# Sirui-Xu/InterDiff

Measured on AMD Instinct MI355X. Metric: denoising frame-steps/sec (denoising-steps/sec x B x T frames), higher is better.
Workload: dtype f32 (every contraction of the denoiser -- feed-forward block, QKV projection, self-attention, row-block contractions and the two token GEMMs: every fp32 operand as two f16 planes, 3 f16 MFMAs per product, fp32 accumulate; SMPL and everything else fp32 MFMA / VALU)

## Files before the change

include/interdiff_hip.h:

```cpp
#ifndef INTERDIFF_HIP_H
#define INTERDIFF_HIP_H

#include <stddef.h>
#include <stdint.h>

#ifdef __cplusplus
extern "C" {
#endif

#define IDF_OK            0
#define IDF_E_INVAL      -22
#define IDF_E_NOMEM      -12
#define IDF_E_LAUNCH     -5

int         interdiff_abi_version(void);
const char *interdiff_build_info(void);

int interdiff_rotation_6d_to_matrix   (const float *d6, float *m,  int64_t n, void *stream);
int interdiff_matrix_to_rotation_6d   (const float *m,  float *d6, int64_t n, void *stream);
int interdiff_matrix_to_axis_angle    (const float *m,  float *aa, int64_t n, void *stream);
int interdiff_axis_angle_to_matrix    (const float *aa, float *m,  int64_t n, void *stream);
int interdiff_axis_angle_to_quaternion(const float *aa, float *q,  int64_t n, void *stream);
int interdiff_rotation_6d_to_axis_angle(const float *d6, float *aa, int64_t n, void *stream);

typedef struct {
    int32_t V, J, n_betas, KB, S;
    const float   *blend;
    const float   *jt;
    const float   *js;
    const int32_t *parents;
    const int32_t *skin_idx;
    const float   *skin_w;
} idf_smpl_model;

size_t interdiff_smpl_workspace_bytes(const idf_smpl_model *m, int64_t N);
int interdiff_smpl_forward(const idf_smpl_model *m, const float *pose, const float *betas,
                           const float *trans, int64_t N, float *verts, float *jtr,
                           float *v_posed, void *ws, size_t ws_bytes, void *stream);

int interdiff_vertex_normals(const float *verts, int64_t N, int32_t V, const int32_t *faces,
                             const int32_t *adj_ptr, const int32_t *adj_face,
                             const int32_t *adj_corner, float *normals, void *stream);
int interdiff_nn_argmin(const float *q, int32_t Pq, const float *r, int32_t Pr, int64_t N,
                        int32_t *idx, void *stream);
int interdiff_point2point_signed(const float *x, int32_t P1, const float *y, int32_t P2, int64_t N,
                                 const float *x_normals, const float *y_normals,
                                 float *y2x_signed, float *x2y_signed, int32_t *yidx, int32_t *xidx,
                                 float *y2x, float *x2y, void *stream);

#define IDF_MDM_LAYERS 8
#define IDF_MDM_D      256
#define IDF_MDM_FF     1024
#define IDF_MDM_HEADS  4
#define IDF_MDM_NQ     10
#define IDF_MDM_MEM    10
#define IDF_MDM_MEM_MAX 16
#define IDF_FFN_SLICES 5

typedef struct {
    int64_t is_qan;
    int64_t sa_in_w, sa_in_b, sa_out_w, sa_out_b;
    int64_t qc, wk;
    int64_t ca_q_w, ca_q_b;
    int64_t ca_kv_w, ca_kv_b;
    int64_t ca_out_w, ca_out_b;
    int64_t ff1_w, ff1_b, ff2_w, ff2_b;
    int64_t ffn_pack;
    int64_t ffn_b1p;
    int64_t sa_in_pack;
    int64_t sa_out_frag;
    int64_t ln_w[3], ln_b[3];
    int64_t ffn_pack_h2;
    int64_t sa_in_pack_h2;
    int64_t qc_h2;
    int64_t rb_h2_ok;
    int64_t sa_out_frag_h2;
    int64_t qkv_bounds_ok;
} idf_mdm_layer;

typedef struct {
    int32_t C;
    int32_t n_steps;
    const float *arena;
    int64_t in_w, in_b;
    int64_t out_w, out_b;
    int64_t temb_table;
    int64_t pe;
    int32_t max_T, has_encoder;
    idf_mdm_layer layer[IDF_MDM_LAYERS];
    idf_mdm_layer enc_layer[IDF_MDM_LAYERS];
    int32_t tune[8];
    int64_t out_w_h2, in_w_h2;
    int64_t tail_h2_ok;
    int32_t mem_len;
    int32_t rb_tokens;
} idf_mdm_weights;

int interdiff_gemm_f32(const float *A, int32_t lda, const float *W, const float *bias, const float *resid, float *C,
                       int32_t ldc, int32_t M, int32_t N, int32_t K, int32_t epi, int32_t cfg, void *stream);

int interdiff_mdm_ffn(const idf_mdm_weights *w, int32_t layer, int32_t encoder, const float *x2, int32_t M, float *parts, void *stream);
size_t interdiff_mdm_memctx_floats_for(int32_t B, int32_t mem_len);

size_t interdiff_mdm_memctx_floats(int32_t B);
size_t interdiff_mdm_workspace_bytes(int32_t B, int32_t T);
int interdiff_mdm_prepare_memory(const idf_mdm_weights *w, const float *cond, int32_t B,
                                 float *memctx, void *ws, size_t ws_bytes, void *stream);
int interdiff_mdm_forward(const idf_mdm_weights *w, const float *memctx, const float *x,
                          const int64_t *ts, int32_t B, int32_t T, float *x0,
                          void *ws, size_t ws_bytes, void *stream);

typedef struct {
    int64_t w[3], b[3];
    int32_t c[4];
} idf_pn_mlp;

typedef struct {
    const float *arena;
    idf_pn_mlp sa1[2];
    idf_pn_mlp sa2[2];
    int64_t lin_w, lin_b;
} idf_pointnet2;

int interdiff_pointnet2_encode(const idf_pointnet2 *pn, const float *obj_points, int32_t B, int32_t P, float *out,
                               void *stream);
size_t interdiff_mdm_encode_workspace_bytes(int32_t B, int32_t Tp);
int interdiff_mdm_encode(const idf_mdm_weights *w, const float *pc, const float *x_past, int32_t B, int32_t Tp,
                         float *cond, void *ws, size_t ws_bytes, void *stream);

int interdiff_inpaint(float *x0, const float *gt, const uint8_t *mask, int64_t n, void *stream);
int interdiff_posterior_step(float *x, const float *x0, const float *noise, int64_t n,
                             float c1, float c2, float sigma, uint64_t seed, uint64_t step_index,
                             void *stream);
int interdiff_randn(float *out, int64_t n, uint64_t seed, uint64_t step_index, void *stream);
int interdiff_posterior_step_at(float *x, const float *x0, const float *noise, int64_t n,
                                float c1, float c2, float sigma, uint64_t seed, uint64_t step_index,
                                uint64_t elem0, void *stream);
int interdiff_randn_at(float *out, int64_t n, uint64_t seed, uint64_t step_index, uint64_t elem0, void *stream);
int interdiff_posterior_step_dev(float *x, const float *x0, const float *gt, const uint8_t *mask, int64_t n,
                                 const float *table, int64_t *state, int64_t *ts, int32_t B, void *stream);
int interdiff_sampler_advance(int64_t *state, int64_t *ts, int32_t B, void *stream);
int interdiff_posterior_step_dev_map(float *x, const float *x0, const float *gt, const uint8_t *mask, int64_t n,
                                     const float *table, const int64_t *tmap, int64_t *state, int64_t *ts, int32_t B, void *stream);
int interdiff_sampler_advance_map(int64_t *state, int64_t *ts, const int64_t *tmap, int32_t B, void *stream);
int interdiff_mdm_forward_step(const idf_mdm_weights *w, const float *memctx, float *x, int64_t *ts, int32_t B, int32_t T,
                               const float *gt, const uint8_t *mask, const float *table, int64_t *state,
                               void *ws, size_t ws_bytes, void *stream);
#define IDF_STEP_EMBED_READY 1
#define IDF_STEP_EMBED_NEXT 2
int interdiff_mdm_forward_step_ex(const idf_mdm_weights *w, const float *memctx, float *x, int64_t *ts, int32_t B, int32_t T,
                                  const float *gt, const uint8_t *mask, const float *table, int64_t *state, void *ws,
                                  size_t ws_bytes, int32_t flags, void *stream);
int interdiff_mdm_forward_step_map(const idf_mdm_weights *w, const float *memctx, float *x, int64_t *ts, int32_t B, int32_t T,
                                   const float *gt, const uint8_t *mask, const float *table, const int64_t *tmap, int64_t *state,
                                   void *ws, size_t ws_bytes, int32_t flags, void *stream);
int interdiff_mdm_step_chaining(const idf_mdm_weights *w);
int interdiff_exclusive_cu_report(char *buf, int32_t cap);
int interdiff_debug_deny_exclusive(const char *patterns);

typedef struct {
    int32_t T, past_len, P, n_pre;
    const float *arena;
    int64_t dct_pad;
    int64_t dct;
    int64_t idct;
    int64_t hand_bonus;
    int64_t layer[12];
    int32_t cin[12], cout[12];
} idf_objproj;

int interdiff_objprojector_sample(const idf_objproj *op, const float *obj_angles,
                                  const float *obj_trans, const float *markers,
                                  const int32_t *contact, int32_t B, float *out, void *stream);
size_t interdiff_objprojector_forward_workspace_bytes(int32_t B);
int interdiff_objprojector_forward(const idf_objproj *op, const float *obj_angles, const float *obj_trans, const float *markers,
                                   const int32_t *contact, int32_t B, int32_t initialize, float *out, void *ws, size_t ws_bytes, void *stream);

typedef struct {
    const idf_smpl_model *smpl;
    const idf_objproj    *objproj;
    const int32_t *faces;
    const int32_t *adj_ptr, *adj_face, *adj_corner;
    const int32_t *markers_idx;
    int32_t n_markers, n_points, past_len;
    int32_t tune;
    const int32_t *vorder, *faces_scan, *markers_scan, *adj_pair_scan;
    const int32_t *adj_pair;
    const int32_t *vrank;
} idf_correction_ctx;

size_t interdiff_correction_workspace_bytes(const idf_correction_ctx *c, int32_t B, int32_t T);
int interdiff_correction(const idf_correction_ctx *c, float *x0, const float *gt,
                         const float *hand_pose, const float *beta, const float *obj_points,
                         int32_t B, int32_t T, float blend_t ,
                         uint8_t *condition, int32_t *contact, float *distance, float *loss,
                         void *ws, size_t ws_bytes, void *stream);
int interdiff_correction_dev(const idf_correction_ctx *c, float *x0, const float *gt, const float *hand_pose,
                             const float *beta, const float *obj_points, int32_t B, int32_t T, const float *table,
                             const int64_t *state, void *ws, size_t ws_bytes, void *stream);

#define IDF_CONTACT_STATS 12
size_t interdiff_contact_nn_workspace_bytes(const idf_correction_ctx *c, int32_t B, int32_t T);
int interdiff_contact_nn(const idf_correction_ctx *c, const float *verts, const float *obj_points, const float *objR,
                         const float *objT, int32_t B, int32_t T, float *o2h, int32_t *idx, uint64_t *stats,
                         void *ws, size_t ws_bytes, void *stream);

size_t interdiff_metrics_workspace_bytes(const idf_correction_ctx *c, int32_t B, int32_t T);
int interdiff_metrics(const idf_correction_ctx *c, const float *obj_pred, const float *jtr,
                      const float *body_trans, const float *obj_gt, const float *jtr_gt,
                      const float *body_trans_gt, const float *verts, const float *obj_points,
                      int32_t B, int32_t T, int32_t J, float *out6 ,
                      void *ws, size_t ws_bytes, void *stream);

typedef struct {
    int32_t T, past_len, J, n_pre;
    const float *arena;
    int64_t dct_pad;
    int64_t dct;
    int64_t idct;
    int64_t layer[12];
    int32_t cin[12], cout[12];
} idf_skel_objproj;

int interdiff_skeleton_objprojector_sample(const idf_skel_objproj *op, const float *obj_angles,
                                           const float *obj_trans, const float *human_points, int32_t B,
                                           float *quat_out, float *trans_out, void *stream);
int interdiff_skeleton_correction(const idf_skel_objproj *op, const float *x, const float *gt,
                                  const float *zero_pose_obj, int32_t B, int32_t T, float blend_t,
                                  float *out, void *stream);
int interdiff_skeleton_metrics(const float *body_pred, const float *body_gt, const float *obj_pred,
                               const float *obj_gt, const float *pose_pred, const float *pose_gt,
                               int32_t T, int32_t B, int32_t from_frame, float *out4, void *stream);

int interdiff_skeleton_finetune_param_table(const idf_skel_objproj *op, int32_t *table, int32_t *n_param, int32_t *n_bn);
size_t interdiff_skeleton_finetune_workspace_bytes(const idf_skel_objproj *op, int32_t B);
int interdiff_skeleton_finetune_grads(const idf_skel_objproj *op, const float *params, const float *bn, const float *obj_angles,
                                      const float *obj_trans, const float *human_points, const float *pose_gt, int32_t B, int32_t T,
                                      const float *weights8, float *out9, float *grads, void *ws, size_t ws_bytes, void *stream);
int interdiff_skeleton_finetune_step(const idf_skel_objproj *op, float *arena, float *params, const float *bn, const float *grads,
                                     float *exp_avg, float *exp_avg_sq, int32_t step, double lr, double beta1, double beta2, double eps,
                                     double weight_decay, void *stream);

typedef struct idf_skel_head {
    int32_t n_body, n_points;
    int32_t n_tiles, reserved;
    int64_t out_w, out_b;
    int64_t shape_w, shape_b;
} idf_skel_head;
int interdiff_skeleton_mdm_forward(const idf_mdm_weights *w, const idf_skel_head *head, const float *memctx, const float *x,
                                   const int64_t *ts, const float *zero_pose_obj, int32_t B, int32_t T, float *x0,
                                   void *ws, size_t ws_bytes, void *stream);
int interdiff_skeleton_mdm_forward_step(const idf_mdm_weights *w, const idf_skel_head *head, const float *memctx, float *x,
                                        int64_t *ts, const float *zero_pose_obj, int32_t B, int32_t T, const float *gt,
                                        const uint8_t *mask, const float *table, int64_t *state, void *ws, size_t ws_bytes,
                                        void *stream);
int interdiff_skeleton_mdm_forward_step_map(const idf_mdm_weights *w, const idf_skel_head *head, const float *memctx, float *x,
                                            int64_t *ts, const float *zero_pose_obj, int32_t B, int32_t T, const float *gt,
                                            const uint8_t *mask, const float *table, const int64_t *tmap, int64_t *state, void *ws,
                                            size_t ws_bytes, void *stream);
size_t interdiff_skeleton_mdm_encode_workspace_bytes(int32_t B, int32_t Tp);
int interdiff_skeleton_mdm_encode(const idf_mdm_weights *w, const idf_skel_head *head, const float *zero_pose_obj,
                                  const float *x_past, int32_t B, int32_t Tp, float *cond, void *ws, size_t ws_bytes,
                                  void *stream);

#define IDF_OPT_NP 483
#define IDF_OPT_NLOSS 6
typedef struct {
    const idf_correction_ctx *geo;
    const float   *blendT;
    const int32_t *jv_ptr;
    const int32_t *jv_vtx;
    const float   *jv_w;
    int32_t K3P, _pad;
} idf_opt_ctx;

typedef struct {
    int32_t B, T, P, max_iters;
    const float *betas;
    const float *obj_points;
    float *param, *init, *grad, *m, *v, *best;
    float *pose, *tr;
    float *verts, *vposed, *verts_gt, *gv;
    float *jtr;
    float *pts, *y2x;
    float *y2x_signed;
    int32_t *yidx;
    int32_t *near;
    float *dvposed;
    float *dA;
    float *dfeat;
    float *gtr;
    float *lossf;
    float *loss;
    float *loss_hist;
    float *best_loss;
    int32_t *flag;
    uint8_t *foot_static;
    int32_t *foot_cnt;
    int32_t *ctl;
    void *smpl_ws; size_t smpl_ws_bytes;
    int32_t *porder; float *psort, *pbox;
} idf_opt_state;

int interdiff_optimize_init(const idf_opt_ctx *c, const idf_opt_state *st, const float *pose, const float *trans,
                            const float *obj_angles, const float *obj_trans, int32_t first_iter, void *stream);
int interdiff_optimize_loss_grad(const idf_opt_ctx *c, const idf_opt_state *st, void *stream);
int interdiff_optimize_step(const idf_opt_ctx *c, const idf_opt_state *st, void *stream);
int interdiff_optimize_finish(const idf_opt_ctx *c, const idf_opt_state *st, float *pose, float *trans, float *obj_angles,
                              float *obj_trans, void *stream);
int interdiff_debug_joint_map_vjp(const float *R, const float *g_out, float *g_in, int32_t n);
int interdiff_debug_lds_sentinel(uint32_t *out, int32_t n_wg, int32_t spin, void *stream);
int interdiff_debug_f16_aggressor(const float *src, size_t n_floats, float *sink, int32_t iters, int32_t grid, int32_t with_loads, void *stream);

enum { IDF_LOSS_VAL = 0, IDF_LOSS_TEST = 1 };
int interdiff_q_sample(float *x_t, const float *x0, const float *noise, const int64_t *ts, const float *sqrt_ac, const float *sqrt_1mac,
                       int32_t n_steps, const float *gt, const uint8_t *mask, int32_t B, int64_t per_clip, uint64_t seed, uint64_t elem0,
                       void *stream);
int interdiff_denoising_losses(const float *pred, const float *target, int32_t B, int32_t T, int32_t past_len, float *out, void *stream);
size_t interdiff_sample_losses_workspace_bytes(int32_t K, int32_t B);
int interdiff_sample_losses(const float *samples, const float *gt, const float *hand_pose, int32_t K, int32_t B, int32_t T, int32_t past_len,
                            int32_t variant, float *out_terms, float *out_per_clip, void *ws, size_t ws_bytes, void *stream);

size_t interdiff_skeleton_sample_losses_workspace_bytes(int32_t K, int32_t B);
int interdiff_skeleton_sample_losses(const float *pred, const float *gt, int32_t K, int32_t B, int32_t C, int32_t T, int32_t past_len,
                                     int32_t n_body, int32_t n_points, float *out_terms, float *out_per_clip, void *ws, size_t ws_bytes,
                                     void *stream);
int interdiff_skeleton_denoising_losses(const float *pred, const float *target, int32_t B, int32_t T, int32_t past_len, int32_t n_body,
                                        int32_t n_points, float *out, void *stream);

size_t interdiff_correction_losses_workspace_bytes(int32_t T, int32_t B, int32_t V, int32_t P);
int interdiff_correction_losses(const float *obj_pred, const float *obj_gt, const float *obj_points, int32_t point_stride, const float *human_verts,
                                int32_t T, int32_t B, int32_t V, int32_t P, int32_t rot_width, int32_t past_len, float *out_terms, float *out_frames,
                                void *ws, size_t ws_bytes, void *stream);

size_t interdiff_contact_labels_workspace_bytes(int64_t N, int32_t V, int32_t F, int32_t P);
int interdiff_contact_labels(const float *verts, int64_t N, int32_t V, const int32_t *faces, int32_t F, const float *points, int32_t P,
                             int64_t point_frame_stride, const float *objR, const float *objT, float thres, uint8_t *obj_label ,
                             uint8_t *human_label , float *signed_dist , void *ws, size_t ws_bytes, void *stream);
int interdiff_debug_point_triangle(const float *tri, const float *p, float *out, int32_t n);

#define IDF_RENDER_SUBPIX 16
#define IDF_RENDER_GUARD 32768
#define IDF_RENDER_MAX_DIM 2048
#define IDF_RENDER_ZONE (1 << 28)
#define IDF_RENDER_REC_INTS 20
#define IDF_RENDER_TILE 16
#define IDF_RENDER_MAX_MESHES 8
enum { IDF_RMESH_SCENE_SPACE = 1, IDF_RMESH_VERTEX_RGB = 2 };
typedef struct {
    float off[3], cam_t[3];
    float cam_cos, cam_sin, znear, focal;
    float light[9];
    float light_gain, ambient;
    float bg[3];
    float reserved;
} idf_render_scene;
typedef struct {
    const float *verts, *normals;
    const int32_t *faces;
    const float *rgb, *R, *t;
    int32_t V, F, frames, flags;
} idf_render_mesh;
size_t interdiff_render_frames_workspace_bytes(int64_t n_images, int64_t n_triangles, int32_t H, int32_t W);
int interdiff_render_frames(const idf_render_scene *scene, const idf_render_mesh *meshes, int32_t n_meshes, int64_t N, int32_t views, int32_t H,
                            int32_t W, uint8_t *out_rgb, int32_t *out_id, int32_t *out_depth, int32_t *out_setup, int64_t *dropped, float *stage_ms,
                            void *ws, size_t ws_bytes, void *stream);
int interdiff_debug_render_setup_vertex(const idf_render_scene *scene, int32_t view, int32_t scene_space, int32_t H, int32_t W, const float *pos,
                                        const float *nrm, const float *rgb, float *out_f, int32_t *out_i, int32_t n);
int interdiff_debug_render_pixel(const int32_t *rec, const int32_t *ij, int32_t *out, int32_t n);

enum {
    IDF_K_EMBED = 0, IDF_K_GEMM_QKV, IDF_K_SELF_ATTN, IDF_K_GEMM_OUTPROJ, IDF_K_ROWBLOCK_QAN,
    IDF_K_ROWBLOCK_STD, IDF_K_FFN_FUSED, IDF_K_RESERVED7, IDF_K_GEMM_HEADS, IDF_K_MEM_PREP,
    IDF_K_INPAINT, IDF_K_POSTERIOR, IDF_K_CORR_PREPARE, IDF_K_SMPL_POSE, IDF_K_SMPL_BLEND_SKIN,
    IDF_K_CORR_CONTACT, IDF_K_CORR_REDUCE, IDF_K_OBJPROJ, IDF_K_CORR_BLEND, IDF_K_OTHER,
    IDF_K_COUNT
};
int interdiff_profile_begin(int32_t capacity);
int interdiff_profile_end(double *ms_per_kind, int64_t *count_per_kind);

enum {
    IDF_TUNE_FFN = 3, IDF_TUNE_FFN_MATH = 4, IDF_TUNE_COUNT = 8
};

#ifdef __cplusplus
}
#endif
#endif
```

interdiff_amd/_lib.py:

```python
import ctypes as C
import os
import torch

_HERE = os.path.dirname(os.path.abspath(__file__))
LIB_PATH = os.environ.get('INTERDIFF_HIP_LIB') or os.path.join(_HERE, 'csrc', 'libinterdiff_hip.so')
ABI_VERSION = 17

vp, i32, i64, f32, u64, sz = C.c_void_p, C.c_int32, C.c_int64, C.c_float, C.c_uint64, C.c_size_t

MDM_LAYERS = 8
FFN_SLICES = 5
STEP_EMBED_READY, STEP_EMBED_NEXT = 1, 2
LOSS_VAL, LOSS_TEST = 0, 1
TUNE = dict(ffn=3, ffn_math=4)


class SmplModel(C.Structure):
    _fields_ = [('V', i32), ('J', i32), ('n_betas', i32), ('KB', i32), ('S', i32),
                ('blend', vp), ('jt', vp), ('js', vp), ('parents', vp), ('skin_idx', vp), ('skin_w', vp)]


class MdmLayer(C.Structure):
    _fields_ = [('is_qan', i64),
                ('sa_in_w', i64), ('sa_in_b', i64), ('sa_out_w', i64), ('sa_out_b', i64),
                ('qc', i64), ('wk', i64),
                ('ca_q_w', i64), ('ca_q_b', i64), ('ca_kv_w', i64), ('ca_kv_b', i64),
                ('ca_out_w', i64), ('ca_out_b', i64),
                ('ff1_w', i64), ('ff1_b', i64), ('ff2_w', i64), ('ff2_b', i64), ('ffn_pack', i64), ('ffn_b1p', i64), ('sa_in_pack', i64), ('sa_out_frag', i64),
                ('ln_w', i64 * 3), ('ln_b', i64 * 3), ('ffn_pack_h2', i64), ('sa_in_pack_h2', i64), ('qc_h2', i64), ('rb_h2_ok', i64), ('sa_out_frag_h2', i64), ('qkv_bounds_ok', i64)]


class MdmWeights(C.Structure):
    _fields_ = [('C', i32), ('n_steps', i32), ('arena', vp),
                ('in_w', i64), ('in_b', i64), ('out_w', i64), ('out_b', i64),
                ('temb_table', i64), ('pe', i64), ('max_T', i32), ('has_encoder', i32),
                ('layer', MdmLayer * MDM_LAYERS), ('enc_layer', MdmLayer * MDM_LAYERS), ('tune', i32 * 8), ('out_w_h2', i64), ('in_w_h2', i64), ('tail_h2_ok', i64), ('mem_len', i32), ('rb_tokens', i32)]


class PnMlp(C.Structure):
    _fields_ = [('w', i64 * 3), ('b', i64 * 3), ('c', i32 * 4)]


class PointNet2(C.Structure):
    _fields_ = [('arena', vp), ('sa1', PnMlp * 2), ('sa2', PnMlp * 2), ('lin_w', i64), ('lin_b', i64)]


class ObjProj(C.Structure):
    _fields_ = [('T', i32), ('past_len', i32), ('P', i32), ('n_pre', i32), ('arena', vp),
                ('dct_pad', i64), ('dct', i64), ('idct', i64), ('hand_bonus', i64),
                ('layer', i64 * 12), ('cin', i32 * 12), ('cout', i32 * 12)]


class SkelObjProj(C.Structure):
    _fields_ = [('T', i32), ('past_len', i32), ('J', i32), ('n_pre', i32), ('arena', vp),
                ('dct_pad', i64), ('dct', i64), ('idct', i64),
                ('layer', i64 * 12), ('cin', i32 * 12), ('cout', i32 * 12)]


class SkelHead(C.Structure):
    _fields_ = [('n_body', i32), ('n_points', i32), ('n_tiles', i32), ('reserved', i32),
                ('out_w', i64), ('out_b', i64), ('shape_w', i64), ('shape_b', i64)]


class CorrectionCtx(C.Structure):
    _fields_ = [('smpl', C.POINTER(SmplModel)), ('objproj', C.POINTER(ObjProj)),
                ('faces', vp), ('adj_ptr', vp), ('adj_face', vp), ('adj_corner', vp), ('markers_idx', vp),
                ('n_markers', i32), ('n_points', i32), ('past_len', i32), ('tune', i32),
                ('vorder', vp), ('faces_scan', vp), ('markers_scan', vp), ('adj_pair_scan', vp), ('adj_pair', vp), ('vrank', vp)]


class OptCtx(C.Structure):
    _fields_ = [('geo', C.POINTER(CorrectionCtx)), ('blendT', vp), ('jv_ptr', vp), ('jv_vtx', vp), ('jv_w', vp), ('K3P', i32), ('_pad', i32)]


OPT_NP, OPT_NLOSS = 483, 6
_OPT_PTRS = ('betas', 'obj_points', 'param', 'init', 'grad', 'm', 'v', 'best', 'pose', 'tr', 'verts', 'vposed', 'verts_gt', 'gv',
             'jtr', 'pts', 'y2x', 'y2x_signed', 'yidx', 'near', 'dvposed', 'dA', 'dfeat', 'gtr', 'lossf', 'loss', 'loss_hist',
             'best_loss', 'flag', 'foot_static', 'foot_cnt', 'ctl', 'smpl_ws')


class OptState(C.Structure):
    _fields_ = [('B', i32), ('T', i32), ('P', i32), ('max_iters', i32)] + [(k, vp) for k in _OPT_PTRS] + [('smpl_ws_bytes', sz), ('porder', vp), ('psort', vp), ('pbox', vp)]


class RenderScene(C.Structure):
    _fields_ = [('off', f32 * 3), ('cam_t', f32 * 3), ('cam_cos', f32), ('cam_sin', f32), ('znear', f32), ('focal', f32),
                ('light', f32 * 9), ('light_gain', f32), ('ambient', f32), ('bg', f32 * 3), ('reserved', f32)]


class RenderMesh(C.Structure):
    _fields_ = [('verts', vp), ('normals', vp), ('faces', vp), ('rgb', vp), ('R', vp), ('t', vp),
                ('V', i32), ('F', i32), ('frames', i32), ('flags', i32)]


RMESH_SCENE_SPACE, RMESH_VERTEX_RGB = 1, 2
RENDER_SUBPIX, RENDER_GUARD, RENDER_MAX_DIM, RENDER_ZONE, RENDER_REC_INTS, RENDER_TILE = 16, 32768, 2048, 1 << 28, 20, 16

_SIGS = {
    'interdiff_abi_version': (C.c_int, []),
    'interdiff_build_info': (C.c_char_p, []),
    'interdiff_rotation_6d_to_matrix': (C.c_int, [vp, vp, i64, vp]),
    'interdiff_matrix_to_rotation_6d': (C.c_int, [vp, vp, i64, vp]),
    'interdiff_matrix_to_axis_angle': (C.c_int, [vp, vp, i64, vp]),
    'interdiff_axis_angle_to_matrix': (C.c_int, [vp, vp, i64, vp]),
    'interdiff_axis_angle_to_quaternion': (C.c_int, [vp, vp, i64, vp]),
    'interdiff_rotation_6d_to_axis_angle': (C.c_int, [vp, vp, i64, vp]),
    'interdiff_smpl_workspace_bytes': (sz, [C.POINTER(SmplModel), i64]),
    'interdiff_smpl_forward': (C.c_int, [C.POINTER(SmplModel), vp, vp, vp, i64, vp, vp, vp, vp, sz, vp]),
    'interdiff_vertex_normals': (C.c_int, [vp, i64, i32, vp, vp, vp, vp, vp, vp]),
    'interdiff_nn_argmin': (C.c_int, [vp, i32, vp, i32, i64, vp, vp]),
    'interdiff_point2point_signed': (C.c_int, [vp, i32, vp, i32, i64, vp, vp, vp, vp, vp, vp, vp, vp, vp]),
    'interdiff_gemm_f32': (C.c_int, [vp, i32, vp, vp, vp, vp, i32, i32, i32, i32, i32, i32, vp]),
    'interdiff_pointnet2_encode': (C.c_int, [C.POINTER(PointNet2), vp, i32, i32, vp, vp]),
    'interdiff_mdm_encode_workspace_bytes': (sz, [i32, i32]),
    'interdiff_mdm_encode': (C.c_int, [C.POINTER(MdmWeights), vp, vp, i32, i32, vp, vp, sz, vp]),
    'interdiff_mdm_ffn': (C.c_int, [C.POINTER(MdmWeights), i32, i32, vp, i32, vp, vp]),
    'interdiff_mdm_memctx_floats': (sz, [i32]),
    'interdiff_mdm_memctx_floats_for': (sz, [i32, i32]),
    'interdiff_mdm_workspace_bytes': (sz, [i32, i32]),
    'interdiff_mdm_prepare_memory': (C.c_int, [C.POINTER(MdmWeights), vp, i32, vp, vp, sz, vp]),
    'interdiff_mdm_forward': (C.c_int, [C.POINTER(MdmWeights), vp, vp, vp, i32, i32, vp, vp, sz, vp]),
    'interdiff_mdm_forward_step': (C.c_int, [C.POINTER(MdmWeights), vp, vp, vp, i32, i32, vp, vp, vp, vp, vp, sz, vp]),
    'interdiff_mdm_forward_step_ex': (C.c_int, [C.POINTER(MdmWeights), vp, vp, vp, i32, i32, vp, vp, vp, vp, vp, sz, i32, vp]),
    'interdiff_mdm_forward_step_map': (C.c_int, [C.POINTER(MdmWeights), vp, vp, vp, i32, i32, vp, vp, vp, vp, vp, vp, sz, i32, vp]),
    'interdiff_mdm_step_chaining': (C.c_int, [C.POINTER(MdmWeights)]),
    'interdiff_inpaint': (C.c_int, [vp, vp, vp, i64, vp]),
    'interdiff_posterior_step': (C.c_int, [vp, vp, vp, i64, f32, f32, f32, u64, u64, vp]),
    'interdiff_randn': (C.c_int, [vp, i64, u64, u64, vp]),
    'interdiff_posterior_step_at': (C.c_int, [vp, vp, vp, i64, f32, f32, f32, u64, u64, u64, vp]),
    'interdiff_randn_at': (C.c_int, [vp, i64, u64, u64, u64, vp]),
    'interdiff_posterior_step_dev': (C.c_int, [vp, vp, vp, vp, i64, vp, vp, vp, i32, vp]),
    'interdiff_sampler_advance': (C.c_int, [vp, vp, i32, vp]),
    'interdiff_posterior_step_dev_map': (C.c_int, [vp, vp, vp, vp, i64, vp, vp, vp, vp, i32, vp]),
    'interdiff_sampler_advance_map': (C.c_int, [vp, vp, vp, i32, vp]),
    'interdiff_objprojector_sample': (C.c_int, [C.POINTER(ObjProj), vp, vp, vp, vp, i32, vp, vp]),
    'interdiff_objprojector_forward_workspace_bytes': (sz, [i32]),
    'interdiff_objprojector_forward': (C.c_int, [C.POINTER(ObjProj), vp, vp, vp, vp, i32, i32, vp, vp, sz, vp]),
    'interdiff_correction_workspace_bytes': (sz, [C.POINTER(CorrectionCtx), i32, i32]),
    'interdiff_correction': (C.c_int, [C.POINTER(CorrectionCtx), vp, vp, vp, vp, vp, i32, i32, f32,
                                       vp, vp, vp, vp, vp, sz, vp]),
    'interdiff_correction_dev': (C.c_int, [C.POINTER(CorrectionCtx), vp, vp, vp, vp, vp, i32, i32, vp, vp, vp, sz, vp]),
    'interdiff_metrics_workspace_bytes': (sz, [C.POINTER(CorrectionCtx), i32, i32]),
    'interdiff_metrics': (C.c_int, [C.POINTER(CorrectionCtx), vp, vp, vp, vp, vp, vp, vp, vp, i32, i32, i32,
                                    vp, vp, sz, vp]),
    'interdiff_contact_nn_workspace_bytes': (sz, [C.POINTER(CorrectionCtx), i32, i32]),
    'interdiff_contact_nn': (C.c_int, [C.POINTER(CorrectionCtx), vp, vp, vp, vp, i32, i32, vp, vp, vp, vp, sz, vp]),
    'interdiff_skeleton_objprojector_sample': (C.c_int, [C.POINTER(SkelObjProj), vp, vp, vp, i32, vp, vp, vp]),
    'interdiff_skeleton_correction': (C.c_int, [C.POINTER(SkelObjProj), vp, vp, vp, i32, i32, f32, vp, vp]),
    'interdiff_skeleton_metrics': (C.c_int, [vp, vp, vp, vp, vp, vp, i32, i32, i32, vp, vp]),
    'interdiff_skeleton_finetune_param_table': (C.c_int, [C.POINTER(SkelObjProj), vp, C.POINTER(i32), C.POINTER(i32)]),
    'interdiff_skeleton_finetune_workspace_bytes': (sz, [C.POINTER(SkelObjProj), i32]),
    'interdiff_skeleton_finetune_grads': (C.c_int, [C.POINTER(SkelObjProj), vp, vp, vp, vp, vp, vp, i32, i32, C.POINTER(f32), vp, vp, vp, sz, vp]),
    'interdiff_skeleton_finetune_step': (C.c_int, [C.POINTER(SkelObjProj), vp, vp, vp, vp, vp, vp, i32, C.c_double, C.c_double, C.c_double, C.c_double,
                                                   C.c_double, vp]),
    'interdiff_skeleton_mdm_forward': (C.c_int, [C.POINTER(MdmWeights), C.POINTER(SkelHead), vp, vp, vp, vp, i32, i32, vp, vp, sz, vp]),
    'interdiff_skeleton_mdm_forward_step': (C.c_int, [C.POINTER(MdmWeights), C.POINTER(SkelHead), vp, vp, vp, vp, i32, i32, vp, vp, vp, vp, vp, sz, vp]),
    'interdiff_skeleton_mdm_forward_step_map': (C.c_int, [C.POINTER(MdmWeights), C.POINTER(SkelHead), vp, vp, vp, vp, i32, i32, vp, vp, vp, vp, vp, vp, sz, vp]),
    'interdiff_skeleton_mdm_encode_workspace_bytes': (sz, [i32, i32]),
    'interdiff_skeleton_mdm_encode': (C.c_int, [C.POINTER(MdmWeights), C.POINTER(SkelHead), vp, vp, i32, i32, vp, vp, sz, vp]),
    'interdiff_q_sample': (C.c_int, [vp, vp, vp, vp, vp, vp, i32, vp, vp, i32, i64, u64, u64, vp]),
    'interdiff_denoising_losses': (C.c_int, [vp, vp, i32, i32, i32, vp, vp]),
    'interdiff_sample_losses_workspace_bytes': (sz, [i32, i32]),
    'interdiff_sample_losses': (C.c_int, [vp, vp, vp, i32, i32, i32, i32, i32, vp, vp, vp, sz, vp]),
    'interdiff_skeleton_sample_losses_workspace_bytes': (sz, [i32, i32]),
    'interdiff_skeleton_sample_losses': (C.c_int, [vp, vp, i32, i32, i32, i32, i32, i32, i32, vp, vp, vp, sz, vp]),
    'interdiff_skeleton_denoising_losses': (C.c_int, [vp, vp, i32, i32, i32, i32, i32, vp, vp]),
    'interdiff_correction_losses_workspace_bytes': (sz, [i32, i32, i32, i32]),
    'interdiff_correction_losses': (C.c_int, [vp, vp, vp, i32, vp, i32, i32, i32, i32, i32, i32, vp, vp, vp, sz, vp]),
    'interdiff_contact_labels_workspace_bytes': (sz, [i64, i32, i32, i32]),
    'interdiff_contact_labels': (C.c_int, [vp, i64, i32, vp, i32, vp, i32, i64, vp, vp, f32, vp, vp, vp, vp, sz, vp]),
    'interdiff_debug_point_triangle': (C.c_int, [vp, vp, vp, i32]),
    'interdiff_render_frames_workspace_bytes': (sz, [i64, i64, i32, i32]),
    'interdiff_render_frames': (C.c_int, [C.POINTER(RenderScene), C.POINTER(RenderMesh), i32, i64, i32, i32, i32, vp, vp, vp, vp, C.POINTER(i64), C.POINTER(f32),
                                          vp, sz, vp]),
    'interdiff_debug_render_setup_vertex': (C.c_int, [C.POINTER(RenderScene), i32, i32, i32, i32, vp, vp, vp, vp, vp, i32]),
    'interdiff_debug_render_pixel': (C.c_int, [vp, vp, vp, i32]),
    'interdiff_optimize_init': (C.c_int, [C.POINTER(OptCtx), C.POINTER(OptState), vp, vp, vp, vp, i32, vp]),
    'interdiff_optimize_loss_grad': (C.c_int, [C.POINTER(OptCtx), C.POINTER(OptState), vp]),
    'interdiff_optimize_step': (C.c_int, [C.POINTER(OptCtx), C.POINTER(OptState), vp]),
    'interdiff_optimize_finish': (C.c_int, [C.POINTER(OptCtx), C.POINTER(OptState), vp, vp, vp, vp, vp]),
    'interdiff_debug_joint_map_vjp': (C.c_int, [vp, vp, vp, i32]),
    'interdiff_debug_lds_sentinel': (C.c_int, [vp, i32, i32, vp]),
    'interdiff_exclusive_cu_report': (C.c_int, [C.c_char_p, i32]),
    'interdiff_debug_deny_exclusive': (C.c_int, [C.c_char_p]),
    'interdiff_debug_f16_aggressor': (C.c_int, [vp, sz, vp, i32, i32, i32, vp]),
    'interdiff_profile_begin': (C.c_int, [i32]),
    'interdiff_profile_end': (C.c_int, [C.POINTER(C.c_double), C.POINTER(C.c_int64)]),
}

KERNEL_KINDS = ('embed', 'gemm_qkv', 'self_attn', 'gemm_outproj', 'rowblock_qan', 'rowblock_std', 'ffn_fused', 'reserved7',
                'gemm_heads', 'mem_prep', 'inpaint', 'posterior', 'corr_prepare', 'smpl_pose', 'smpl_blend_skin',
                'corr_contact', 'corr_reduce', 'objproj', 'corr_blend', 'other')

_lib = None


class HipLibraryMissing(RuntimeError):
    pass


def load():
    global _lib
    if _lib is not None:
        return _lib
    if not os.path.exists(LIB_PATH):
        raise HipLibraryMissing('%s not found: build it with `python -m interdiff_amd.csrc.build` '
                                '(there is no CPU/torch fallback for the hot path)' % LIB_PATH)
    lib = C.CDLL(LIB_PATH)
    for name, (res, args) in _SIGS.items():
        fn = getattr(lib, name)
        fn.restype, fn.argtypes = res, args
    if lib.interdiff_abi_version() != ABI_VERSION:
        raise HipLibraryMissing('stale %s: abi %d != %d, rebuild' % (LIB_PATH, lib.interdiff_abi_version(), ABI_VERSION))
    _lib = lib
    return lib


def exclusive_cu_report():
    buf = C.create_string_buffer(8192)
    bad = load().interdiff_exclusive_cu_report(buf, len(buf))
    if bad < 0:
        check(bad, 'exclusive_cu_report')
    return buf.value.decode(), bad


def debug_deny_exclusive(patterns=''):
    check(load().interdiff_debug_deny_exclusive(patterns.encode() if patterns else None), 'debug_deny_exclusive')


def exported_symbols():
    return sorted(_SIGS)


_ERR = {-22: 'IDF_E_INVAL (bad shape / pointer / unsupported size)', -12: 'IDF_E_NOMEM (workspace too small)',
        -5: 'IDF_E_LAUNCH (kernel launch failed)'}


def check(rc, what=''):
    if rc != 0:
        raise RuntimeError('interdiff_hip %s failed: %s' % (what, _ERR.get(rc, rc)))


def dptr(t, dtype=None, allow_none=False):
    if t is None:
        if allow_none:
            return vp(None)
        raise ValueError('null tensor')
    if not t.is_cuda:
        raise ValueError('interdiff_amd ops need device tensors (got %s); the HIP path has no CPU fallback' % t.device)
    if not t.is_contiguous():
        raise ValueError('tensor must be contiguous')
    if dtype is not None and t.dtype != dtype:
        raise ValueError('expected %s, got %s' % (dtype, t.dtype))
    return vp(t.data_ptr())


def stream():
    return vp(torch.cuda.current_stream().cuda_stream)
```

interdiff_amd/correction.py:

```python
import ctypes as C
import os
import itertools
import numpy as np
import torch
from . import _lib
from .geometry import MeshTopology

MARKERS67 = [3470, 3171, 3327, 857, 1812, 628, 182, 3116, 3040, 239,
             1666, 1725, 0, 2174, 1568, 1368, 3387, 2112, 1053, 1058,
             3336, 3346, 1323, 2108, 3122, 3314, 1252, 1082, 1861, 1454,
             850, 2224, 3233, 1769, 6728, 4343, 5273, 4116, 3694, 6399,
             6540, 6488, 3749, 5135, 5194, 3512, 5635, 5210, 4360, 4841,
             6786, 5573, 4538, 4544, 6736, 6747, 4804, 5568, 6544, 6682,
             5322, 4927, 5686, 4598, 6633, 3506, 3508]


_UID = itertools.count(1)


def correction_gate(t0):
    return not (t0 > 500 or t0 % 50 != 0)


class HipCorrection:
    def __init__(self, smpl_layer, objprojector, n_points=2048, past_len=10, markers=MARKERS67, device='cuda', scan_order=True):
        self.lib = _lib.load()
        self.device = torch.device(device)
        self.smpl, self.objproj, self.past_len = smpl_layer, objprojector, past_len
        self.topo = MeshTopology(smpl_layer.th_faces, smpl_layer.cmodel.V, self.device, rest_vertices=getattr(smpl_layer, 'v_template', None) if scan_order else None)
        self.markers_idx = torch.tensor(list(markers), dtype=torch.int32, device=self.device)
        ctx = _lib.CorrectionCtx()
        ctx.smpl = C.pointer(smpl_layer.cmodel)
        ctx.objproj = C.pointer(objprojector.cop)
        ctx.faces, ctx.adj_ptr = self.topo.faces.data_ptr(), self.topo.adj_ptr.data_ptr()
        ctx.adj_face, ctx.adj_corner = self.topo.adj_face.data_ptr(), self.topo.adj_corner.data_ptr()
        ctx.markers_idx = self.markers_idx.data_ptr()
        ctx.n_markers, ctx.n_points, ctx.past_len = len(markers), n_points, past_len
        if self.topo.vorder is not None:
            self.markers_scan = self.topo.scan_positions(markers, self.device)
            ctx.vorder, ctx.faces_scan, ctx.markers_scan = self.topo.vorder.data_ptr(), self.topo.faces_scan.data_ptr(), self.markers_scan.data_ptr()
            ctx.adj_pair_scan = self.topo.adj_pair_scan.data_ptr()
            ctx.vrank = self.topo.vrank.data_ptr()
        ctx.tune = 0
        self.ctx = ctx
        self._ws = {}
        self.debug = None
        self._uid = next(_UID)

    graph_capturable = True

    def workspace_for(self, B, T):
        return torch.empty(self.lib.interdiff_correction_workspace_bytes(C.byref(self.ctx), B, T), dtype=torch.uint8, device=self.device)

    def apply_dev(self, x, table, state, y, ws):
        B, _, Cc, T = x.shape
        if y['obj_points'].shape[1] != self.ctx.n_points:
            raise ValueError('obj_points must have %d points' % self.ctx.n_points)
        _lib.check(self.lib.interdiff_correction_dev(C.byref(self.ctx), _lib.dptr(x, torch.float32), _lib.dptr(y['inpainted_motion'], torch.float32),
                                                     _lib.dptr(y['hand_pose'], torch.float32), _lib.dptr(y['beta'], torch.float32),
                                                     _lib.dptr(y['obj_points'], torch.float32), B, T, _lib.dptr(table), _lib.dptr(state),
                                                     _lib.dptr(ws), ws.numel(), _lib.stream()), 'correction_dev')
        return x

    def _workspace(self, B, T):
        need = self.lib.interdiff_correction_workspace_bytes(C.byref(self.ctx), B, T)
        key = torch.cuda.current_stream(self.device).cuda_stream
        ws = self._ws.pop(key, None)
        if ws is None or ws.numel() < need:
            ws = torch.empty(need, dtype=torch.uint8, device=self.device)
        self._ws[key] = ws
        if len(self._ws) > self.MAX_STREAM_WORKSPACES:
            torch.cuda.synchronize(self.device)
            self._ws.pop(next(iter(self._ws)))
        return ws

    MAX_STREAM_WORKSPACES = 4

    def apply(self, x, t0, y):
        B, _, Cc, T = x.shape
        if not x.is_contiguous():
            raise ValueError('x must be contiguous (it is updated in place)')
        if y['obj_points'].shape[1] != self.ctx.n_points:
            raise ValueError('obj_points must have %d points' % self.ctx.n_points)
        gt = y['inpainted_motion'].contiguous()
        hp, beta, pts = y['hand_pose'].contiguous().float(), y['beta'].contiguous().float(), y['obj_points'].contiguous().float()
        ws = self._workspace(B, T)
        dbg = [None] * 4
        if self.debug is not None:
            dbg = [torch.empty(B, dtype=torch.uint8, device=self.device), torch.empty(B, len(MARKERS67), dtype=torch.int32, device=self.device),
                   torch.empty(B, device=self.device), torch.empty(B, device=self.device)]
        blend_t = float(np.float32(t0) / np.float32(1000))
        _lib.check(self.lib.interdiff_correction(C.byref(self.ctx), _lib.dptr(x, torch.float32), _lib.dptr(gt, torch.float32),
                                                 _lib.dptr(hp), _lib.dptr(beta), _lib.dptr(pts), B, T, blend_t,
                                                 *[_lib.dptr(d, allow_none=True) for d in dbg], _lib.dptr(ws), ws.numel(),
                                                 _lib.stream()), 'correction')
        if self.debug is not None:
            self.debug.update(condition=dbg[0], contact=dbg[1], distance=dbg[2], loss=dbg[3])
        return x

    def contact_nn(self, verts, obj_points, objR, objT, want_stats=False):
        T, B = verts.shape[:2]
        P = self.ctx.n_points
        o2h = torch.empty(T, B, P, device=self.device)
        idx = torch.empty(T, B, P, dtype=torch.int32, device=self.device)
        stats = torch.zeros(12, dtype=torch.int64, device=self.device) if want_stats else None
        need = self.lib.interdiff_contact_nn_workspace_bytes(C.byref(self.ctx), B, T)
        ws = getattr(self, '_nn_ws', None)
        if ws is None or ws.numel() < need:
            ws = self._nn_ws = torch.empty(need, dtype=torch.uint8, device=self.device)
        v, pts, R_, t_ = (a.contiguous().float() for a in (verts, obj_points, objR, objT))
        _lib.check(self.lib.interdiff_contact_nn(C.byref(self.ctx), _lib.dptr(v), _lib.dptr(pts), _lib.dptr(R_), _lib.dptr(t_), B, T, _lib.dptr(o2h),
                                                 _lib.dptr(idx), _lib.dptr(stats, allow_none=True), _lib.dptr(ws), ws.numel(), _lib.stream()), 'contact_nn')
        return (o2h, idx, tuple(int(x) for x in stats.cpu())) if want_stats else (o2h, idx)

    def is_active(self, t0):
        return correction_gate(int(t0))

    def __call__(self, x, t, model_kwargs):
        t0 = getattr(t, 'host_value', None)
        if t0 is None:
            t0 = int(t[0])
        if not correction_gate(t0):
            return x
        return self.apply(x, t0, model_kwargs['y'])
```

interdiff_amd/csrc/common.h:

```cpp
#pragma once
#include <hip/hip_runtime.h>
#include <stdint.h>
#include <stdio.h>
#include <atomic>
#include <mutex>
#include <string>
#include <vector>
#include "../../include/interdiff_hip.h"

#define IDF_WAVE 64

#define IDF_CHECK_LAUNCH()                                                                        \
    do {                                                                                          \
        const hipError_t idf_e_ = hipGetLastError();                                              \
        if (idf_e_ != hipSuccess) {                                                               \
            fprintf(stderr, "interdiff_hip: %s (%s:%d)\n", hipGetErrorString(idf_e_), __FILE__, __LINE__); \
            return IDF_E_LAUNCH;                                                                  \
        }                                                                                         \
    } while (0)

static inline hipStream_t idf_stream(void *s) { return reinterpret_cast<hipStream_t>(s); }
static inline int64_t idf_cdiv(int64_t a, int64_t b) { return (a + b - 1) / b; }
static inline size_t idf_align(size_t x, size_t a = 256) { return (x + a - 1) / a * a; }

static inline int idf_opt_in_lds(const void *fn, int bytes, std::atomic<uint64_t> &done) {
    int dev = 0;
    if (hipGetDevice(&dev) != hipSuccess) return IDF_E_LAUNCH;
    const uint64_t bit = 1ull << (dev & 63);
    if (done.load(std::memory_order_acquire) & bit) return IDF_OK;
    if (hipFuncSetAttribute(fn, hipFuncAttributeMaxDynamicSharedMemorySize, bytes) != hipSuccess) return IDF_E_LAUNCH;
    done.fetch_or(bit, std::memory_order_release);
    return IDF_OK;
}

struct idf_excl_entry {
    const char *name;
    int threads, num_regs, static_lds, dyn_lds, blocks_per_cu, ok, dev, denied;
};
inline std::mutex g_idf_excl_mu;
inline std::vector<idf_excl_entry> g_idf_excl;
inline void idf_excl_record(const idf_excl_entry &e) {
    std::lock_guard<std::mutex> lk(g_idf_excl_mu);
    for (idf_excl_entry &o : g_idf_excl)
        if (o.dev == e.dev && std::string(o.name) == e.name) { o = e; return; }
    g_idf_excl.push_back(e);
}
inline int idf_excl_report(char *buf, int cap) {
    std::lock_guard<std::mutex> lk(g_idf_excl_mu);
    int bad = 0, n = 0;
    buf[0] = 0;
    for (const idf_excl_entry &e : g_idf_excl) {
        bad += e.ok ? 0 : 1;
        const int w = snprintf(buf + n, (size_t)(cap - n), "%-52s dev %d  threads %3d  regs %3d  lds %6d + %6d  workgroups_per_cu %d  %s\n", e.name, e.dev, e.threads, e.num_regs,
                               e.static_lds, e.dyn_lds, e.blocks_per_cu, e.ok ? "exclusive" : (e.denied ? "DENIED (debug deny list) -> fp32 kernel" : "NOT exclusive -> fp32 kernel"));
        if (w < 0 || w >= cap - n) break;
        n += w;
    }
    return bad;
}
inline std::string g_idf_excl_deny;
inline std::atomic<uint64_t> g_idf_excl_gen{1};
inline void idf_excl_set_deny(const char *patterns) {
    std::lock_guard<std::mutex> lk(g_idf_excl_mu);
    g_idf_excl_deny = patterns ? patterns : "";
    g_idf_excl.clear();
    g_idf_excl_gen.fetch_add(1, std::memory_order_acq_rel);
}
inline bool idf_excl_denied(const char *name) {
    std::lock_guard<std::mutex> lk(g_idf_excl_mu);
    if (g_idf_excl_deny.empty()) return false;
    const std::string nm(name);
    size_t a = 0;
    while (a <= g_idf_excl_deny.size()) {
        size_t b = g_idf_excl_deny.find(',', a);
        if (b == std::string::npos) b = g_idf_excl_deny.size();
        if (b > a && nm.find(g_idf_excl_deny.substr(a, b - a)) != std::string::npos) return true;
        a = b + 1;
    }
    return false;
}
struct idf_excl_cache {
    std::atomic<uint64_t> yes{0}, no{0}, gen{0};
    std::atomic<int> dyn{-1};
};
constexpr int IDF_CU_LDS_BYTES = 160 * 1024;
constexpr int IDF_NOT_EXCLUSIVE = 1;
static inline int idf_public_rc(int rc) { return rc == IDF_NOT_EXCLUSIVE ? IDF_E_LAUNCH : rc; }
static inline int idf_exclusive_cu(const void *fn, const char *name, int threads, idf_excl_cache &c) {
    int dev = 0;
    if (hipGetDevice(&dev) != hipSuccess) return -1;
    const uint64_t bit = 1ull << (dev & 63), gen = g_idf_excl_gen.load(std::memory_order_acquire);
    if (c.gen.load(std::memory_order_acquire) != gen) {
        c.yes.store(0, std::memory_order_release);
        c.no.store(0, std::memory_order_release);
        c.gen.store(gen, std::memory_order_release);
    }
    if (c.yes.load(std::memory_order_acquire) & bit) return c.dyn.load(std::memory_order_acquire);
    if (c.no.load(std::memory_order_acquire) & bit) return -1;
    idf_excl_entry e{name, threads, -1, -1, -1, -1, 0, dev, 0};
    hipFuncAttributes at;
    if (hipFuncGetAttributes(&at, fn) == hipSuccess) {
        e.num_regs = at.numRegs;
        e.static_lds = (int)at.sharedSizeBytes;
        e.dyn_lds = IDF_CU_LDS_BYTES - e.static_lds;
        if (e.dyn_lds >= 0 && hipFuncSetAttribute(fn, hipFuncAttributeMaxDynamicSharedMemorySize, e.dyn_lds) == hipSuccess &&
            hipOccupancyMaxActiveBlocksPerMultiprocessor(&e.blocks_per_cu, fn, threads, (size_t)e.dyn_lds) == hipSuccess)
            e.ok = e.blocks_per_cu == 1 && e.num_regs >= (threads > 512 ? 128 : 256) ? 1 : 0;
    }
    (void)hipGetLastError();
    if (e.ok && idf_excl_denied(name)) { e.ok = 0; e.denied = 1; }
    idf_excl_record(e);
    if (e.ok) {
        c.dyn.store(e.dyn_lds, std::memory_order_release);
        c.yes.fetch_or(bit, std::memory_order_release);
        return e.dyn_lds;
    }
    c.no.fetch_or(bit, std::memory_order_release);
    if (e.denied) fprintf(stderr, "interdiff_hip: %s is on the DEBUG deny list: the fp32-MFMA kernel runs instead\n", name);
    else fprintf(stderr, "interdiff_hip: %s does not get its CU to itself on device %d (regs %d, LDS %d + %d, %d workgroups per CU): the fp32-MFMA kernel runs instead\n",
                 name, dev, e.num_regs, e.static_lds, e.dyn_lds, e.blocks_per_cu);
    return -1;
}

static inline int idf_cu_count() {
    static std::atomic<int> cached[64];
    int dev = 0;
    if (hipGetDevice(&dev) != hipSuccess) return 256;
    int n = cached[dev & 63].load(std::memory_order_acquire);
    if (n <= 0) {
        if (hipDeviceGetAttribute(&n, hipDeviceAttributeMultiprocessorCount, dev) != hipSuccess || n <= 0) n = 256;
        cached[dev & 63].store(n, std::memory_order_release);
    }
    return n;
}

typedef float f32x4 __attribute__((ext_vector_type(4)));

typedef __attribute__((address_space(3))) float idf_lds_float;
__device__ __forceinline__ uint32_t idf_lds_addr(const float *p) {
    return __builtin_amdgcn_readfirstlane((uint32_t)(uintptr_t)(idf_lds_float *)p);
}
__device__ __forceinline__ const float *idf_uniform_ptr(const float *p) {
    const uint64_t v = (uint64_t)(uintptr_t)p;
    const uint32_t lo = __builtin_amdgcn_readfirstlane((uint32_t)v), hi = __builtin_amdgcn_readfirstlane((uint32_t)(v >> 32));
    return reinterpret_cast<const float *>(((uint64_t)hi << 32) | lo);
}
__device__ __forceinline__ void idf_dma16_s(const float *gbase, uint32_t voff_bytes, uint32_t lds_base) {
    gbase = idf_uniform_ptr(gbase);
    lds_base = __builtin_amdgcn_readfirstlane(lds_base);
    asm volatile("s_mov_b32 m0, %2\n\ts_nop 0\n\tglobal_load_lds_dwordx4 %0, %1" ::"v"(voff_bytes), "s"(gbase), "s"(lds_base) : "memory", "m0");
}
__device__ __forceinline__ void idf_dma16_v(const float *gptr, uint32_t lds_base) {
    lds_base = __builtin_amdgcn_readfirstlane(lds_base);
    asm volatile("s_mov_b32 m0, %1\n\ts_nop 0\n\tglobal_load_lds_dwordx4 %0, off" ::"v"(gptr), "s"(lds_base) : "memory", "m0");
}

__device__ __forceinline__ void idf_store4_wt(float *p, const float v) {
    asm volatile("global_store_dword %0, %1, off sc0 sc1" ::"v"(p), "v"(v) : "memory");
}
__device__ __forceinline__ void idf_store16_wt(float *p, const float4 v) {
    const f32x4 t = {v.x, v.y, v.z, v.w};
    asm volatile("global_store_dwordx4 %0, %1, off sc0 sc1\n\ts_nop 1" ::"v"(p), "v"(t) : "memory");
}

template <class T>
__device__ __forceinline__ void idf_arg_now(T a) { asm volatile("" ::"s"(a)); }
template <class... A>
__device__ __forceinline__ void idf_args_now(A... a) { (idf_arg_now(a), ...); }

int idf_point_order(hipStream_t s, const float *obj_points, int B, int P, int32_t *porder);
int idf_nn_scan_opt(hipStream_t s, int64_t N, int frames_per_clip, const float *verts, int V, const float *pts_frame, const float *obj_points, int P,
                    const int32_t *porder, const idf_correction_ctx *c, int32_t *yidx);
int idf_near_mask_opt(hipStream_t s, int64_t N, int frames_per_clip, const float *verts, int V, const float *pts_frame, int P, const int32_t *porder,
                      const int32_t *vorder, float *psort, float *pbox, int32_t *near);

size_t idf_objproj_keep_floats();
int idf_objproj_check(const idf_objproj *op);
int idf_objproj_pick(const idf_objproj *op, const float *keep, const int32_t *contact, int B, float *out, hipStream_t s);

extern bool g_idf_prof_on;
void idf_prof_mark_slow(int kind, hipStream_t s);
static inline void idf_prof_mark(int kind, hipStream_t s) { if (g_idf_prof_on) idf_prof_mark_slow(kind, s); }


typedef float f32x16 __attribute__((ext_vector_type(16)));

#define IDF_DPP_ROR(v, n) __builtin_bit_cast(float, __builtin_amdgcn_update_dpp(0, __builtin_bit_cast(int, v), 0x120 + (n), 0xf, 0xf, false))
__device__ __forceinline__ float row16_sum(float v) {
    v += IDF_DPP_ROR(v, 8);
    v += IDF_DPP_ROR(v, 4);
    v += IDF_DPP_ROR(v, 2);
    v += IDF_DPP_ROR(v, 1);
    return v;
}
__device__ __forceinline__ float row16_max(float v) {
    v = fmaxf(v, IDF_DPP_ROR(v, 8));
    v = fmaxf(v, IDF_DPP_ROR(v, 4));
    v = fmaxf(v, IDF_DPP_ROR(v, 2));
    v = fmaxf(v, IDF_DPP_ROR(v, 1));
    return v;
}
#define IDF_LANE(v, l) __builtin_bit_cast(float, __builtin_amdgcn_readlane(__builtin_bit_cast(int, v), l))
__device__ __forceinline__ float wave_sum(float v) {
    v = row16_sum(v);
    return (IDF_LANE(v, 0) + IDF_LANE(v, 16)) + (IDF_LANE(v, 32) + IDF_LANE(v, 48));
}
__device__ __forceinline__ float wave_max(float v) {
    v = row16_max(v);
    return fmaxf(fmaxf(IDF_LANE(v, 0), IDF_LANE(v, 16)), fmaxf(IDF_LANE(v, 32), IDF_LANE(v, 48)));
}

__device__ __forceinline__ float gelu_erf(float x) { return 0.5f * x * (1.0f + erff(x * 0.70710678118654752440f)); }

__device__ __forceinline__ float gelu_fast(float x) {
    const float z = fabsf(x) * 0.70710678118654752440f;
    const float t = __builtin_amdgcn_rcpf(1.0f + 0.3275911f * z);
    const float p = ((((1.061405429f * t - 1.453152027f) * t + 1.421413741f) * t - 0.284496736f) * t + 0.254829592f) * t;
    const float er = 1.0f - p * __expf(-(z * z));
    return 0.5f * x * (1.0f + copysignf(er, x));
}

__device__ __forceinline__ void ln_row_stats(const float4 v, float &mean, float &rstd) {
    mean = wave_sum(v.x + v.y + v.z + v.w) * (1.0f / 256.0f);
    const float a = v.x - mean, b = v.y - mean, c = v.z - mean, d = v.w - mean;
    const float var = wave_sum(a * a + b * b + c * c + d * d) * (1.0f / 256.0f);
    rstd = __builtin_amdgcn_rsqf(var + 1e-5f);
}

struct Row16 {
    float4 c[4];
};
__device__ __forceinline__ void ln_row16(Row16 &r, const float *__restrict__ w, const float *__restrict__ b, int l16) {
    float s = 0.f;
#pragma unroll
    for (int i = 0; i < 4; ++i) s += (r.c[i].x + r.c[i].y) + (r.c[i].z + r.c[i].w);
    const float mean = row16_sum(s) * (1.0f / 256.0f);
    float q = 0.f;
#pragma unroll
    for (int i = 0; i < 4; ++i) {
        const float a0 = r.c[i].x - mean, a1 = r.c[i].y - mean, a2 = r.c[i].z - mean, a3 = r.c[i].w - mean;
        q += (a0 * a0 + a1 * a1) + (a2 * a2 + a3 * a3);
    }
    const float rstd = __builtin_amdgcn_rsqf(row16_sum(q) * (1.0f / 256.0f) + 1e-5f);
#pragma unroll
    for (int i = 0; i < 4; ++i) {
        const float4 g = *reinterpret_cast<const float4 *>(w + (i * 16 + l16) * 4), be = *reinterpret_cast<const float4 *>(b + (i * 16 + l16) * 4);
        r.c[i].x = (r.c[i].x - mean) * rstd * g.x + be.x;
        r.c[i].y = (r.c[i].y - mean) * rstd * g.y + be.y;
        r.c[i].z = (r.c[i].z - mean) * rstd * g.z + be.z;
        r.c[i].w = (r.c[i].w - mean) * rstd * g.w + be.w;
    }
}
__device__ __forceinline__ void row16_load(Row16 &r, const float *__restrict__ row, int l16) {
#pragma unroll
    for (int i = 0; i < 4; ++i) r.c[i] = *reinterpret_cast<const float4 *>(row + (i * 16 + l16) * 4);
}
template <int NP>
__device__ __forceinline__ float4 ld4_sum(const float *__restrict__ p, size_t stride) {
    float4 t[NP];
#pragma unroll
    for (int s = 0; s < NP; ++s) t[s] = *reinterpret_cast<const float4 *>(p + s * stride);
    float4 v = t[0];
#pragma unroll
    for (int s = 1; s < NP; ++s) { v.x += t[s].x; v.y += t[s].y; v.z += t[s].z; v.w += t[s].w; }
    return v;
}
template <int NP>
struct Row16Raw {
    float4 t[4][NP];
    __device__ __forceinline__ void request(const float *__restrict__ row, int l16, size_t stride) {
#pragma unroll
        for (int i = 0; i < 4; ++i)
#pragma unroll
            for (int s = 0; s < NP; ++s) t[i][s] = *reinterpret_cast<const float4 *>(row + s * stride + (i * 16 + l16) * 4);
    }
    __device__ __forceinline__ void reduce(Row16 &r) const {
#pragma unroll
        for (int i = 0; i < 4; ++i) {
            float4 v = t[i][0];
#pragma unroll
            for (int s = 1; s < NP; ++s) { v.x += t[i][s].x; v.y += t[i][s].y; v.z += t[i][s].z; v.w += t[i][s].w; }
            r.c[i] = v;
        }
    }
};
template <int NP>
__device__ __forceinline__ void row16_load_sum(Row16 &r, const float *__restrict__ row, int l16, size_t stride) {
    Row16Raw<NP> raw;
    raw.request(row, l16, stride);
    raw.reduce(r);
}
__device__ __forceinline__ void row16_store(const Row16 &r, float *__restrict__ row, int l16) {
#pragma unroll
    for (int i = 0; i < 4; ++i) *reinterpret_cast<float4 *>(row + (i * 16 + l16) * 4) = r.c[i];
}
__device__ __forceinline__ void row16_store_wt(const Row16 &r, float *__restrict__ row, int l16) {
#pragma unroll
    for (int i = 0; i < 4; ++i) idf_store16_wt(row + (i * 16 + l16) * 4, r.c[i]);
}
__device__ __forceinline__ void row16_zero(Row16 &r) {
#pragma unroll
    for (int i = 0; i < 4; ++i) r.c[i] = make_float4(0.f, 0.f, 0.f, 0.f);
}
```

interdiff_amd/csrc/correction.hip:

```cpp
#include "common.h"
#include "objproj.h"
#include "rot_math.h"
#include <float.h>

namespace {

constexpr int NBODY = 22;
constexpr int CTOK = 144;

__global__ __launch_bounds__(256) void corr_prepare_kernel(const float *__restrict__ x0, const float *__restrict__ gt,
                                                           const float *__restrict__ hand_pose, int B, int T,
                                                           float *__restrict__ pose, float *__restrict__ trans,
                                                           float *__restrict__ objR, float *__restrict__ objT,
                                                           float *__restrict__ gt_angles, float *__restrict__ gt_trans) {
    const int64_t i = (int64_t)blockIdx.x * 256 + threadIdx.x;
    const int64_t N = (int64_t)B * T;
    if (i >= N * 24) return;
    const int64_t n = i / 24;
    const int slot = (int)(i - n * 24), t = (int)(n / B), b = (int)(n - (int64_t)t * B);
    const float *xb = x0 + (size_t)b * CTOK * T + t;
    if (slot < NBODY) {
        float d[6], m[9], a[3];
#pragma unroll
        for (int k = 0; k < 6; ++k) d[k] = xb[(size_t)(slot * 6 + k) * T];
        rot::rot6d_to_matrix(d, m);
        rot::matrix_to_axis_angle(m, a);
        float *p = pose + n * 156 + slot * 3;
        p[0] = a[0]; p[1] = a[1]; p[2] = a[2];
    } else if (slot == 22) {
        for (int k = 0; k < 90; ++k) pose[n * 156 + 66 + k] = hand_pose[n * 90 + k];
#pragma unroll
        for (int k = 0; k < 3; ++k) trans[n * 3 + k] = xb[(size_t)(132 + k) * T];
    } else {
        float d[6], m[9];
#pragma unroll
        for (int k = 0; k < 6; ++k) d[k] = xb[(size_t)(135 + k) * T];
        rot::rot6d_to_matrix(d, m);
#pragma unroll
        for (int k = 0; k < 9; ++k) objR[n * 9 + k] = m[k];
        const float *gb = gt + (size_t)b * CTOK * T + t;
#pragma unroll
        for (int k = 0; k < 3; ++k) {
            objT[n * 3 + k] = xb[(size_t)(141 + k) * T];
            gt_trans[n * 3 + k] = gb[(size_t)(141 + k) * T];
        }
#pragma unroll
        for (int k = 0; k < 6; ++k) gt_angles[n * 6 + k] = gb[(size_t)(135 + k) * T];
    }
}

__device__ __forceinline__ float dist2_exact(float qx, float qy, float qz, float rx, float ry, float rz) {
#pragma clang fp contract(off)
    const float dx = qx - rx, dy = qy - ry, dz = qz - rz;
    const float xx = dx * dx, yy = dy * dy, zz = dz * dz;
    return (xx + yy) + zz;
}

__device__ __forceinline__ float3 f3(const float4 v) { return make_float3(v.x, v.y, v.z); }
__device__ __forceinline__ float3 sub3(float3 a, float3 b) { return make_float3(a.x - b.x, a.y - b.y, a.z - b.z); }
__device__ __forceinline__ float3 cross3(float3 a, float3 b) {
    return make_float3(a.y * b.z - a.z * b.y, a.z * b.x - a.x * b.z, a.x * b.y - a.y * b.x);
}

constexpr int MAXP = 2048;
__global__ __launch_bounds__(1024) void corr_point_order_kernel(const float *__restrict__ obj_points, int P, int32_t *__restrict__ porder) {
    __shared__ unsigned long long keys[MAXP];
    __shared__ float red[6][1024];
    const int b = blockIdx.x, tid = threadIdx.x;
    const float *op = obj_points + (size_t)b * P * 3;
    float p[2][3];
    float lo[3] = {FLT_MAX, FLT_MAX, FLT_MAX}, hi[3] = {-FLT_MAX, -FLT_MAX, -FLT_MAX};
#pragma unroll
    for (int k = 0; k < 2; ++k) {
        const int i = tid + 1024 * k;
#pragma unroll
        for (int a = 0; a < 3; ++a) {
            p[k][a] = i < P ? op[3 * i + a] : 0.f;
            if (i < P) { lo[a] = fminf(lo[a], p[k][a]); hi[a] = fmaxf(hi[a], p[k][a]); }
        }
    }
#pragma unroll
    for (int a = 0; a < 3; ++a) { red[a][tid] = lo[a]; red[3 + a][tid] = hi[a]; }
    __syncthreads();
    for (int s = 512; s > 0; s >>= 1) {
        if (tid < s) {
#pragma unroll
            for (int a = 0; a < 3; ++a) {
                red[a][tid] = fminf(red[a][tid], red[a][tid + s]);
                red[3 + a][tid] = fmaxf(red[3 + a][tid], red[3 + a][tid + s]);
            }
        }
        __syncthreads();
    }
#pragma unroll
    for (int k = 0; k < 2; ++k) {
        const int i = tid + 1024 * k;
        unsigned long long key = ~0ull;
        if (i < P) {
            unsigned code = 0;
            unsigned q[3];
#pragma unroll
            for (int a = 0; a < 3; ++a) {
                const float ext = red[3 + a][0] - red[a][0];
                const float u = ext > 0.f ? (p[k][a] - red[a][0]) / ext : 0.f;
                q[a] = (unsigned)fminf(fmaxf(u * 1023.0f, 0.f), 1023.0f);
            }
#pragma unroll
            for (int bit = 0; bit < 10; ++bit)
#pragma unroll
                for (int a = 0; a < 3; ++a) code |= ((q[a] >> bit) & 1u) << (3 * bit + a);
            key = ((unsigned long long)code << 11) | (unsigned)i;
        }
        keys[i] = key;
    }
    __syncthreads();
    for (int k = 2; k <= MAXP; k <<= 1) {
        for (int j = k >> 1; j > 0; j >>= 1) {
            const int l = 2 * j * (tid / j) + (tid % j), r = l + j;
            const unsigned long long x = keys[l], y = keys[r];
            const bool up = (l & k) == 0;
            if ((x > y) == up) { keys[l] = y; keys[r] = x; }
            __syncthreads();
        }
    }
#pragma unroll
    for (int k = 0; k < 2; ++k) {
        const int i = tid + 1024 * k;
        if (i < P) porder[(size_t)b * P + i] = (int32_t)(keys[i] & 2047u);
    }
}

constexpr int MAXM = 128;
constexpr float MARK_D2 = 0.00039999996079131961f;
constexpr int CB = 16;
constexpr int SB = 8;
constexpr int SEED_STRIDE = 4;
constexpr int CT = 1024;
constexpr int TASK = 64;
typedef float v2f __attribute__((ext_vector_type(2)));

struct ContactLds {
    int V4, nCB, nSB, nSeed;
    int rec, mark, box, sbox, seed, flags, red, pl, total;
    __host__ __device__ explicit ContactLds(int V) {
        V4 = (V + CB - 1) / CB * CB; nCB = V4 / CB; nSB = (nCB + SB - 1) / SB; nSeed = (nCB + SEED_STRIDE - 1) / SEED_STRIDE;
        rec = 0;
        mark = rec + V4;
        box = mark + MAXM;
        sbox = box + 3 * (nSB * SB / 2);
        seed = sbox + 3 * ((nSB + 2) / 2);
        flags = seed + 2 * ((nSeed + 1) / 2);
        red = flags + MAXM / 4;
        pl = red + CT / 4;
        total = pl + MAXP / 4;
    }
};

__device__ __forceinline__ float3 lds_rec(const float4 *vs, int pos) {
    const float *f = reinterpret_cast<const float *>(vs + 2 * (pos >> 1));
    const int h = pos & 1;
    return make_float3(f[h], f[2 + h], f[4 + h]);
}
__device__ __forceinline__ void lds_rec_store(float4 *vs, int pos, float x, float y, float z) {
    float *f = reinterpret_cast<float *>(vs + 2 * (pos >> 1));
    const int h = pos & 1;
    f[h] = x; f[2 + h] = y; f[4 + h] = z;
}
__device__ __forceinline__ void lds_box_store(float4 *bx, int k, float3 lo, float3 hi) {
    float *f = reinterpret_cast<float *>(bx + 3 * (k >> 1));
    const int h = k & 1;
    f[h] = lo.x; f[2 + h] = lo.y; f[4 + h] = lo.z; f[6 + h] = hi.x; f[8 + h] = hi.y; f[10 + h] = hi.z;
}
__device__ __forceinline__ void lds_box_load(const float4 *bx, int k, float3 &lo, float3 &hi) {
    const float *f = reinterpret_cast<const float *>(bx + 3 * (k >> 1));
    const int h = k & 1;
    lo = make_float3(f[h], f[2 + h], f[4 + h]);
    hi = make_float3(f[6 + h], f[8 + h], f[10 + h]);
}

struct PredArgs {
    idf_objproj op;
    const float *obj_angles, *obj_trans;
    const int32_t *markers_idx;
    float *markers, *keep;
    int nclips;
};
template <bool OPT, bool WITH_PRED = false>
__global__ __launch_bounds__(CT) void corr_contact_kernel(const float *__restrict__ verts, int V,
                                                          const float *__restrict__ obj_points, int P,
                                                          const int32_t *__restrict__ porder ,
                                                          const float *__restrict__ objR, const float *__restrict__ objT,
                                                          const int32_t *__restrict__ faces ,
                                                          const int32_t *__restrict__ adj_ptr,
                                                          const int32_t *__restrict__ adj_face,
                                                          const int32_t *__restrict__ adj_corner,
                                                          const int32_t *__restrict__ adj_pair ,
                                                          const int32_t *__restrict__ vorder ,
                                                          const int32_t *__restrict__ vrank ,
                                                          const int32_t *__restrict__ markers_pos , int M, int B,
                                                          float *__restrict__ markers_out, float *__restrict__ loss_sum,
                                                          float *__restrict__ min_dist, int32_t *__restrict__ label,
                                                          float *__restrict__ o2h_out ,
                                                          int32_t *__restrict__ idx_out ,
                                                          unsigned long long *__restrict__ stats ,
                                                          int64_t nn_from ,
                                                          const float *__restrict__ pts_frame , int frames_per_clip ,
                                                          const PredArgs pred) {
    extern __shared__ __attribute__((aligned(16))) float4 vs[];
    if constexpr (WITH_PRED) {
        if ((int)blockIdx.x < pred.nclips) {
            const int b = blockIdx.x, Tn = pred.op.T;
            for (int i = threadIdx.x; i < Tn * M; i += CT) {
                const int t = i / M, m = i - t * M;
                const size_t nfr = (size_t)t * B + b;
                const float *v = verts + (nfr * V + pred.markers_idx[m]) * 3;
                float *o = pred.markers + (nfr * M + m) * 3;
                o[0] = v[0]; o[1] = v[1]; o[2] = v[2];
            }
            __threadfence();
            __syncthreads();
            idf_objproj_dev::objproj_body<1>(reinterpret_cast<float *>(vs), pred.op, pred.obj_angles, pred.obj_trans, pred.markers, nullptr, B, b, pred.keep, nullptr);
            return;
        }
    }
    const ContactLds L(V);
    const int nCB = L.nCB, nSB = L.nSB;
    float4 *ms = vs + L.mark, *bb = vs + L.box, *sbb = vs + L.sbox, *sd = vs + L.seed;
    int *flags = reinterpret_cast<int *>(vs + L.flags);
    float *red = reinterpret_cast<float *>(vs + L.red);
    float *pl = reinterpret_cast<float *>(vs + L.pl);
    __shared__ int next_task;
    const int64_t n = WITH_PRED ? (int64_t)blockIdx.x - pred.nclips : (int64_t)blockIdx.x;
    const int b = OPT ? (int)(n / frames_per_clip) : (int)(n % B), tid = threadIdx.x;
    const float *vf = verts + (size_t)n * V * 3;
    const bool do_nn = n >= nn_from;
    long long t_prev = 0;
    int n_phase = 0;
    auto phase_done = [&]() {
        if (stats && tid == 0 && do_nn) {
            const long long now = (long long)__builtin_readcyclecounter();
            if (n_phase > 0) atomicAdd(stats + 3 + n_phase, (unsigned long long)(now - t_prev));
            t_prev = now;
        }
        ++n_phase;
    };
    phase_done();
    float R[9] = {1.f, 0.f, 0.f, 0.f, 1.f, 0.f, 0.f, 0.f, 1.f}, tr[3] = {0.f, 0.f, 0.f};
    if constexpr (!OPT) {
#pragma unroll
        for (int k = 0; k < 9; ++k) R[k] = objR[n * 9 + k];
#pragma unroll
        for (int k = 0; k < 3; ++k) tr[k] = objT[n * 3 + k];
    }
    const int my_marker_pos = (!OPT && tid < M) ? markers_pos[tid] : 0;
    if (vorder && vrank) {
        for (int i0 = tid; i0 < V; i0 += 4 * CT) {
            typedef float f3v __attribute__((ext_vector_type(3), aligned(4)));
            int pos[4];
            f3v pv[4];
#pragma unroll
            for (int k = 0; k < 4; ++k) {
                const int i = min(i0 + k * CT, V - 1);
                pos[k] = vrank[i];
                pv[k] = *reinterpret_cast<const f3v *>(vf + 3 * i);
            }
#pragma unroll
            for (int k = 0; k < 4; ++k) {
                if (i0 + k * CT < V) {
                    lds_rec_store(vs, pos[k], pv[k].x, pv[k].y, pv[k].z);
                    reinterpret_cast<int *>(vs + 2 * (pos[k] >> 1) + 1)[2 + (pos[k] & 1)] = i0 + k * CT;
                }
            }
        }
        for (int v = V + tid; v < L.V4; v += CT) {
            lds_rec_store(vs, v, 3e18f, 3e18f, 3e18f);
            reinterpret_cast<int *>(vs + 2 * (v >> 1) + 1)[2 + (v & 1)] = 0x7fffffff;
        }
    } else
    for (int v0 = tid; v0 < L.V4; v0 += 4 * CT) {
        int o[4];
        float x[4], y[4], z[4];
#pragma unroll
        for (int k = 0; k < 4; ++k) {
            const int v = v0 + k * CT;
            o[k] = v < V ? (vorder ? vorder[v] : v) : -1;
        }
#pragma unroll
        for (int k = 0; k < 4; ++k) {
            x[k] = y[k] = z[k] = 3e18f;
            if (o[k] >= 0) {
                typedef float f3v __attribute__((ext_vector_type(3), aligned(4)));
                const f3v pv = *reinterpret_cast<const f3v *>(vf + 3 * o[k]);
                x[k] = pv.x; y[k] = pv.y; z[k] = pv.z;
            }
        }
#pragma unroll
        for (int k = 0; k < 4; ++k) {
            const int v = v0 + k * CT;
            if (v < L.V4) {
                lds_rec_store(vs, v, x[k], y[k], z[k]);
                reinterpret_cast<int *>(vs + 2 * (v >> 1) + 1)[2 + (v & 1)] = o[k] >= 0 ? o[k] : 0x7fffffff;
            }
        }
    }
    if (tid < MAXM) flags[tid] = 0;
    const int ntask_all = (P + TASK - 1) / TASK;
    const int task0 = (int)((long long)blockIdx.y * ntask_all / gridDim.y), task1 = (int)((long long)(blockIdx.y + 1) * ntask_all / gridDim.y);
    if (tid == 0) next_task = task0;
    for (int i = tid; i < MAXP; i += CT) pl[i] = 0.f;
    __syncthreads();
    phase_done();
    if (!OPT && tid < ((M + 1) & ~1)) {
        float3 mk = make_float3(3e18f, 3e18f, 3e18f);
        if (tid < M) {
            mk = lds_rec(vs, my_marker_pos);
            if (markers_out) {
                float *mo = markers_out + ((size_t)n * M + tid) * 3;
                mo[0] = mk.x; mo[1] = mk.y; mo[2] = mk.z;
            }
        }
        lds_rec_store(ms, tid, mk.x, mk.y, mk.z);
    }
    if (do_nn) {
#define IDF_DPP8(v, op, ctrl) v = op(v, __builtin_bit_cast(float, __builtin_amdgcn_update_dpp(__builtin_bit_cast(int, v), __builtin_bit_cast(int, v), ctrl, 0xf, 0xf, false)))
        const int lane_ = tid & 63, wave_ = tid >> 6, nsw = 2 * ((nSB + 2) / 2);
        for (int sb = wave_; sb < nsw; sb += CT / 64) {
            const int pr = sb * 64 + lane_;
            float lx = FLT_MAX, ly = FLT_MAX, lz = FLT_MAX, hx = -FLT_MAX, hy = -FLT_MAX, hz = -FLT_MAX;
            if (2 * pr < V) {
                const float4 xy = vs[2 * pr], zz = vs[2 * pr + 1];
                const bool two = 2 * pr + 1 < V;
                lx = two ? fminf(xy.x, xy.y) : xy.x; hx = two ? fmaxf(xy.x, xy.y) : xy.x;
                ly = two ? fminf(xy.z, xy.w) : xy.z; hy = two ? fmaxf(xy.z, xy.w) : xy.z;
                lz = two ? fminf(zz.x, zz.y) : zz.x; hz = two ? fmaxf(zz.x, zz.y) : zz.x;
            }
            IDF_DPP8(lx, fminf, 0xB1); IDF_DPP8(lx, fminf, 0x4E); IDF_DPP8(lx, fminf, 0x141);
            IDF_DPP8(ly, fminf, 0xB1); IDF_DPP8(ly, fminf, 0x4E); IDF_DPP8(ly, fminf, 0x141);
            IDF_DPP8(lz, fminf, 0xB1); IDF_DPP8(lz, fminf, 0x4E); IDF_DPP8(lz, fminf, 0x141);
            IDF_DPP8(hx, fmaxf, 0xB1); IDF_DPP8(hx, fmaxf, 0x4E); IDF_DPP8(hx, fmaxf, 0x141);
            IDF_DPP8(hy, fmaxf, 0xB1); IDF_DPP8(hy, fmaxf, 0x4E); IDF_DPP8(hy, fmaxf, 0x141);
            IDF_DPP8(hz, fmaxf, 0xB1); IDF_DPP8(hz, fmaxf, 0x4E); IDF_DPP8(hz, fmaxf, 0x141);
            const int cb = sb * SB + (lane_ >> 3);
            if ((lane_ & 7) == 0 && cb < nSB * SB) lds_box_store(bb, cb, make_float3(lx, ly, lz), make_float3(hx, hy, hz));
            const float slx = -wave_max(-lx), sly = -wave_max(-ly), slz = -wave_max(-lz), shx = wave_max(hx), shy = wave_max(hy), shz = wave_max(hz);
            if (lane_ == 0) lds_box_store(sbb, sb, make_float3(slx, sly, slz), make_float3(shx, shy, shz));
        }
#undef IDF_DPP8
        for (int k = tid; k < 2 * ((L.nSeed + 1) / 2); k += CT) {
            const float3 p = lds_rec(vs, min(k * SEED_STRIDE, nCB - 1) * CB);
            lds_rec_store(sd, k, p.x, p.y, p.z);
        }
    }
    const float *op = OPT ? pts_frame + (size_t)n * P * 3 : obj_points + (size_t)b * P * 3;
    const int ln = tid & 63, ntask = task1;
    __syncthreads();
    phase_done();
    float mind2 = FLT_MAX;
    unsigned n_exec = 0, n_test = 0, n_tasks = 0;
    for (;;) {
        int task = 0;
        if (ln == 0) task = atomicAdd(&next_task, 1);
        task = __builtin_amdgcn_readfirstlane(task);
        if (task >= ntask) break;
        ++n_tasks;
        const int sp = task * TASK + ln;
        const int i = sp < P ? (porder ? porder[(size_t)b * P + sp] : sp) : -1;
        const bool valid = i >= 0;
        float px = 0.f, py = 0.f, pz = 0.f;
        if (valid) { px = op[3 * i]; py = op[3 * i + 1]; pz = op[3 * i + 2]; }
        const float qx = OPT ? px : (px * R[0] + py * R[1] + pz * R[2]) + tr[0];
        const float qy = OPT ? py : (px * R[3] + py * R[4] + pz * R[5]) + tr[1];
        const float qz = OPT ? pz : (px * R[6] + py * R[7] + pz * R[8]) + tr[2];
        if (do_nn) {
#pragma clang fp contract(off)
            const v2f QX = v2f{qx, qx}, QY = v2f{qy, qy}, QZ = v2f{qz, qz};
            auto pair_d2 = [&](const float4 xy, const float4 zz) {
#pragma clang fp contract(off)
                const v2f dx = QX - v2f{xy.x, xy.y}, dy = QY - v2f{xy.z, xy.w}, dz = QZ - v2f{zz.x, zz.y};
                return (dx * dx + dy * dy) + dz * dz;
            };
            auto pair_a2 = [&](const float4 xy, const float2 zz) {
                const v2f dx = QX - v2f{xy.x, xy.y}, dy = QY - v2f{xy.z, xy.w}, dz = QZ - v2f{zz.x, zz.y};
                return __builtin_elementwise_fma(dz, dz, __builtin_elementwise_fma(dy, dy, dx * dx));
            };
            constexpr float SCAN_M = 1.000003814697265625f, SCAN_ABS = 1e-37f;
            float seed = FLT_MAX;
            for (int k = 0; k < (L.nSeed + 1) / 2; k += 4) {
                float4 xy[4]; float2 zz[4];
#pragma unroll
                for (int u = 0; u < 4; ++u) { xy[u] = sd[2 * min(k + u, (L.nSeed + 1) / 2 - 1)]; zz[u] = *reinterpret_cast<const float2 *>(&sd[2 * min(k + u, (L.nSeed + 1) / 2 - 1) + 1]); }
#pragma unroll
                for (int u = 0; u < 4; ++u) {
                    const v2f a2 = pair_a2(xy[u], zz[u]);
                    seed = fminf(fminf(seed, a2.x), a2.y);
                }
            }
            float thr = __builtin_fmaf(seed, SCAN_M, SCAN_ABS);
            float best = FLT_MAX, bthr = FLT_MAX;
            int tie = 0;
            int bblk = 0, bblk2 = 0;
            auto pair_lb = [&](const float4 a, const float4 bq, const float4 c) {
#pragma clang fp contract(off)
                const v2f ax = v2f{a.x, a.y} - QX, bx = QX - v2f{bq.z, bq.w};
                const v2f ay = v2f{a.z, a.w} - QY, by = QY - v2f{c.x, c.y};
                const v2f az = v2f{bq.x, bq.y} - QZ, bz = QZ - v2f{c.z, c.w};
                const v2f ex = v2f{fmaxf(fmaxf(ax.x, bx.x), 0.f), fmaxf(fmaxf(ax.y, bx.y), 0.f)};
                const v2f ey = v2f{fmaxf(fmaxf(ay.x, by.x), 0.f), fmaxf(fmaxf(ay.y, by.y), 0.f)};
                const v2f ez = v2f{fmaxf(fmaxf(az.x, bz.x), 0.f), fmaxf(fmaxf(az.y, bz.y), 0.f)};
                return __builtin_elementwise_fma(ez, ez, __builtin_elementwise_fma(ey, ey, ex * ex));
            };
            auto score_block = [&](int cb) {
                ++n_exec;
                const int v0 = cb * CB;
                float4 xy[CB / 2]; float2 zz[CB / 2];
#pragma unroll
                for (int u = 0; u < CB / 2; ++u) { xy[u] = vs[v0 + 2 * u]; zz[u] = *reinterpret_cast<const float2 *>(&vs[v0 + 2 * u + 1]); }
                float bm = FLT_MAX;
#pragma unroll
                for (int u = 0; u < CB / 2; ++u) {
                    const v2f a2 = pair_a2(xy[u], zz[u]);
                    bm = fminf(fminf(bm, a2.x), a2.y);
                }
                if (bm < best) {
                    const float w = __builtin_fmaf(bm, SCAN_M, SCAN_ABS);
                    if (best <= w) { tie = tie ? 2 : 1; bblk2 = bblk; } else tie = 0;
                    best = bm; bblk = v0; bthr = w; thr = fminf(thr, w);
                } else if (bm <= bthr) { tie = tie ? 2 : 1; bblk2 = v0; }
            };
            auto scan_super = [&](int sb) {
                const int cb0 = sb * SB;
#pragma unroll
                for (int j = 0; j < SB / 2; ++j) {
                    const int cb = cb0 + 2 * j;
                    const float4 *bx = bb + 3 * (cb >> 1);
                    const v2f lb = pair_lb(bx[0], bx[1], bx[2]);
                    n_test += 2;
                    if (__builtin_amdgcn_ballot_w64(valid && lb.x <= thr) != 0ull) score_block(cb);
                    if (__builtin_amdgcn_ballot_w64(valid && lb.y <= thr) != 0ull) score_block(cb + 1);
                }
            };
            if (!vorder) {
                for (int cb = 0; cb < nCB; ++cb) score_block(cb);
            } else
            for (int sb = 0; sb < nSB; sb += 2) {
                const float4 *bx = sbb + 3 * (sb >> 1);
                const v2f lb = pair_lb(bx[0], bx[1], bx[2]);
                n_test += 2;
                if (__builtin_amdgcn_ballot_w64(valid && lb.x <= thr) != 0ull) scan_super(sb);
                if (__builtin_amdgcn_ballot_w64(valid && lb.y <= thr) != 0ull) scan_super(sb + 1);
            }
            int pos = bblk, org = 0x7fffffff;
            float ebest = FLT_MAX;
            auto resolve_pair = [&](int pr) {
                const float4 xy = vs[2 * pr], zz = vs[2 * pr + 1];
                const v2f d2 = pair_d2(xy, zz);
                const int o0 = __builtin_bit_cast(int, zz.z), o1 = __builtin_bit_cast(int, zz.w);
                if (d2.x < ebest || (d2.x == ebest && o0 < org)) { ebest = d2.x; org = o0; pos = 2 * pr; }
                if (d2.y < ebest || (d2.y == ebest && o1 < org)) { ebest = d2.y; org = o1; pos = 2 * pr + 1; }
            };
            if (tie < 2) {
#pragma unroll
                for (int u = 0; u < CB / 2; ++u) resolve_pair((bblk >> 1) + u);
                if (tie) {
#pragma unroll
                    for (int u = 0; u < CB / 2; ++u) resolve_pair((bblk2 >> 1) + u);
                }
            } else {
                for (int pr = 0; pr < (V + 1) / 2; ++pr) resolve_pair(pr);
            }
            pos = min(pos, V - 1);
            if (org == 0x7fffffff) org = vorder ? vorder[pos] : pos;
            if constexpr (OPT) {
                if (valid) idx_out[(size_t)n * P + i] = org;
            } else if (valid) {
                const float3 v3 = lds_rec(vs, pos);
                float3 acc = make_float3(0.f, 0.f, 0.f);
                const int e0 = adj_ptr[org], e1 = adj_ptr[org + 1];
                if (adj_pair) {
                    for (int e = e0; e < e1; e += 4) {
                        int2 ab[4];
#pragma unroll
                        for (int u = 0; u < 4; ++u) ab[u] = *reinterpret_cast<const int2 *>(adj_pair + 2 * (size_t)min(e + u, e1 - 1));
#pragma unroll
                        for (int u = 0; u < 4; ++u) {
                            if (e + u < e1) {
                                const float3 nn = cross3(sub3(lds_rec(vs, ab[u].x), v3), sub3(lds_rec(vs, ab[u].y), v3));
                                acc.x += nn.x; acc.y += nn.y; acc.z += nn.z;
                            }
                        }
                    }
                } else {
                    for (int e = e0; e < e1; ++e) {
                        const int f = adj_face[e], c = adj_corner[e];
                        const float3 p0 = lds_rec(vs, faces[3 * f]), p1 = lds_rec(vs, faces[3 * f + 1]), p2 = lds_rec(vs, faces[3 * f + 2]);
                        float3 nn;
                        if (c == 1) nn = cross3(sub3(p2, p1), sub3(p0, p1));
                        else if (c == 2) nn = cross3(sub3(p0, p2), sub3(p1, p2));
                        else nn = cross3(sub3(p1, p0), sub3(p2, p0));
                        acc.x += nn.x; acc.y += nn.y; acc.z += nn.z;
                    }
                }
                const float nl = fmaxf(sqrtf(acc.x * acc.x + acc.y * acc.y + acc.z * acc.z), 1e-6f);
                const float vx = qx - v3.x, vy = qy - v3.y, vz = qz - v3.z;
                const float dt = (acc.x / nl) * vx + (acc.y / nl) * vy + (acc.z / nl) * vz;
                const float d = sqrtf(vx * vx + vy * vy + vz * vz);
                const float o2h = d * (dt > 0.f ? 1.f : (dt < 0.f ? -1.f : 0.f));
                if (o2h_out) o2h_out[(size_t)n * P + i] = o2h;
                if (idx_out) idx_out[(size_t)n * P + i] = org;
                pl[sp] = o2h < 0.f ? fabsf(o2h) * 20.0f : 0.f;
            }
        }
        if (!OPT && valid) {
#pragma clang fp contract(off)
            const v2f QX = v2f{qx, qx}, QY = v2f{qy, qy}, QZ = v2f{qz, qz};
            for (int p2 = 0; p2 < (M + 1) / 2; ++p2) {
                const float4 xy = ms[2 * p2], zz = ms[2 * p2 + 1];
                const v2f dx = v2f{xy.x, xy.y} - QX, dy = v2f{xy.z, xy.w} - QY, dz = v2f{zz.x, zz.y} - QZ;
                const v2f d2 = __builtin_elementwise_fma(dy, dy, dx * dx) + dz * dz;
                mind2 = fminf(fminf(mind2, d2.x), d2.y);
                if (__builtin_amdgcn_ballot_w64(fminf(d2.x, d2.y) < MARK_D2) != 0ull) {
                    if (d2.x < MARK_D2) flags[2 * p2] = 1;
                    if (d2.y < MARK_D2) flags[2 * p2 + 1] = 1;
                }
            }
        }
    }
    if (stats && ln == 0 && do_nn) {
        atomicAdd(stats, (unsigned long long)n_exec);
        atomicAdd(stats + 1, (unsigned long long)nCB * n_tasks);
        atomicAdd(stats + 2, (unsigned long long)n_test);
    }
    phase_done();
    if constexpr (OPT) return;
    __syncthreads();
    phase_done();
    float loss = 0.f;
#pragma unroll
    for (int k = 0; k < MAXP / CT; ++k) loss += pl[tid + CT * k];
    red[tid] = loss;
    __syncthreads();
    for (int s = CT / 2; s > 0; s >>= 1) {
        if (tid < s) red[tid] += red[tid + s];
        __syncthreads();
    }
    const float loss_total = red[0];
    __syncthreads();
    red[tid] = mind2;
    __syncthreads();
    for (int s = CT / 2; s > 0; s >>= 1) {
        if (tid < s) red[tid] = fminf(red[tid], red[tid + s]);
        __syncthreads();
    }
    if (tid == 0) { loss_sum[n] = loss_total; min_dist[n] = red[0] == FLT_MAX ? FLT_MAX : sqrtf(red[0]); }
    if (tid < M) label[(size_t)n * M + tid] = flags[tid];
    phase_done();
    if (stats && tid == 0 && do_nn) atomicAdd(stats + 3, 1ull);
}

size_t contact_lds_bytes(int V) { return (size_t)ContactLds(V).total * sizeof(float4); }

int launch_contact(hipStream_t s, int64_t N, const float *verts, int V, const float *obj_points, int P, int32_t *porder,
                   const float *objR, const float *objT, const idf_correction_ctx *c, int B, float *markers, float *loss_sum,
                   float *min_dist, int32_t *label, float *o2h, int32_t *idx, unsigned long long *stats, int64_t nn_from, const PredArgs *pred = nullptr) {
    const int M = c->n_markers;
    const size_t lds = contact_lds_bytes(V);
    if (lds > 160 * 1024 - 16384 || P > MAXP) return IDF_E_INVAL;
    const bool ordered = c->vorder != nullptr;
    if (ordered != (c->faces_scan != nullptr) || ordered != (c->markers_scan != nullptr) || ordered != (c->adj_pair_scan != nullptr)) return IDF_E_INVAL;
    const int32_t *faces = ordered ? c->faces_scan : c->faces, *mpos = ordered ? c->markers_scan : c->markers_idx;
    if (porder) hipLaunchKernelGGL(corr_point_order_kernel, dim3((unsigned)B), dim3(1024), 0, s, obj_points, P, porder);
    if (pred) {
        const size_t lds2 = (pred->nclips > 0 && lds < idf_objproj_dev::OBJPROJ_LDS) ? idf_objproj_dev::OBJPROJ_LDS : lds;
        static std::atomic<uint64_t> lds_ok2{0};
        if (lds2 > 160 * 1024 - 2048) return IDF_E_INVAL;
        if (idf_opt_in_lds(reinterpret_cast<const void *>(corr_contact_kernel<false, true>), 160 * 1024 - 2048, lds_ok2) != IDF_OK) return IDF_E_LAUNCH;
        hipLaunchKernelGGL((corr_contact_kernel<false, true>), dim3((unsigned)(N + pred->nclips)), dim3(CT), lds2, s, verts, V, obj_points, P, porder, objR, objT, faces,
                           c->adj_ptr, c->adj_face, c->adj_corner, c->adj_pair_scan, c->vorder, c->vrank, mpos, M, B, markers, loss_sum, min_dist, label, o2h, idx,
                           stats, nn_from, nullptr, 0, *pred);
        return IDF_OK;
    }
    static std::atomic<uint64_t> lds_ok{0};
    if (idf_opt_in_lds(reinterpret_cast<const void *>(corr_contact_kernel<false>), 160 * 1024 - 16384, lds_ok) != IDF_OK) return IDF_E_LAUNCH;
    hipLaunchKernelGGL(corr_contact_kernel<false>, dim3((unsigned)N), dim3(CT), lds, s, verts, V, obj_points, P, porder, objR, objT, faces,
                       c->adj_ptr, c->adj_face, c->adj_corner, c->adj_pair_scan, c->vorder, c->vrank, mpos, M, B, markers, loss_sum, min_dist, label, o2h, idx,
                       stats, nn_from, nullptr, 0, PredArgs{});
    return IDF_OK;
}

__global__ __launch_bounds__(128) void corr_reduce_kernel(const float *__restrict__ loss_sum, const float *__restrict__ min_dist,
                                                          const int32_t *__restrict__ label, int B, int T, int past, int P, int M,
                                                          uint8_t *__restrict__ condition, int32_t *__restrict__ contact,
                                                          float *__restrict__ distance_out, float *__restrict__ loss_out) {
    extern __shared__ float fr[];
    const int b = blockIdx.x, tid = threadIdx.x;
    for (int t = tid; t < T; t += 128) {
        fr[t] = loss_sum[(size_t)t * B + b];
        fr[T + t] = min_dist[(size_t)t * B + b];
    }
    if (tid < M) {
        int c = 0;
#pragma unroll 16
        for (int t = past; t < T; ++t) c += label[((size_t)t * B + b) * M + tid];
        contact[(size_t)b * M + tid] = c;
    }
    __syncthreads();
    if (tid == 0) {
        float ls = 0.f, ds = 0.f;
        for (int t = past; t < T; ++t) ls += fr[t] / (float)P;
        for (int t = 0; t < T; ++t) ds += fr[T + t];
        const float loss = ls / (float)(T - past), dist = ds / (float)T;
        condition[b] = !((loss < 0.002f) && (dist < 0.02f));
        if (distance_out) distance_out[b] = dist;
        if (loss_out) loss_out[b] = loss;
    }
}

__global__ __launch_bounds__(256) void corr_blend_kernel(float *__restrict__ x0, const float *__restrict__ proj,
                                                         const uint8_t *__restrict__ condition, int B, int T, float a,
                                                         const float *__restrict__ a_table, const int64_t *__restrict__ a_state) {
    if (a_table) a = a_table[a_state[0] * 4 + 3];
    const int64_t i = (int64_t)blockIdx.x * 256 + threadIdx.x;
    if (i >= (int64_t)B * CTOK * T) return;
    const int b = (int)(i / (CTOK * T)), r = (int)(i - (int64_t)b * CTOK * T), c = r / T, t = r - c * T;
    if (!condition[b]) return;
    const float x = x0[i];
    const float other = c < 135 ? x : proj[((size_t)t * B + b) * 9 + (c - 135)];
    x0[i] = a * x + (1.0f - a) * other;
}

struct CorrWs {
    float *pose, *trans, *objR, *objT, *gt_angles, *gt_trans, *verts, *jtr, *markers, *loss_sum, *min_dist, *proj, *proj_keep;
    int32_t *label, *contact, *porder;
    uint8_t *condition;
    void *smpl_ws;
    size_t smpl_ws_bytes, total;
};

CorrWs carve(const idf_correction_ctx *c, int B, int T, void *ws) {
    const int64_t N = (int64_t)B * T;
    const int V = c->smpl->V, J = c->smpl->J, M = c->n_markers;
    char *p = reinterpret_cast<char *>(ws);
    size_t off = 0;
    auto take = [&](size_t bytes) { char *r = p ? p + off : nullptr; off += idf_align(bytes); return r; };
    CorrWs w;
    w.pose = (float *)take(N * 156 * 4);
    w.trans = (float *)take(N * 3 * 4);
    w.objR = (float *)take(N * 9 * 4);
    w.objT = (float *)take(N * 3 * 4);
    w.gt_angles = (float *)take(N * 6 * 4);
    w.gt_trans = (float *)take(N * 3 * 4);
    w.verts = (float *)take((size_t)N * V * 3 * 4);
    w.jtr = (float *)take((size_t)N * J * 3 * 4);
    w.markers = (float *)take((size_t)N * M * 3 * 4);
    w.loss_sum = (float *)take(N * 4);
    w.min_dist = (float *)take(N * 4);
    w.proj = (float *)take(N * 9 * 4);
    w.label = (int32_t *)take((size_t)N * M * 4);
    w.contact = (int32_t *)take((size_t)B * M * 4);
    w.condition = (uint8_t *)take(B);
    w.porder = (int32_t *)take((size_t)B * c->n_points * 4);
    w.proj_keep = (float *)take((size_t)B * idf_objproj_keep_floats() * 4);
    w.smpl_ws_bytes = interdiff_smpl_workspace_bytes(c->smpl, N);
    w.smpl_ws = take(w.smpl_ws_bytes);
    w.total = off;
    return w;
}


constexpr int NPATCH = MAXP / 64;
__global__ __launch_bounds__(256) void opt_patch_kernel(const float *__restrict__ pts, int P, const int32_t *__restrict__ porder, int frames_per_clip,
                                                        float4 *__restrict__ psort , float4 *__restrict__ pbox ) {
    const int64_t n = blockIdx.x;
    const int b = (int)(n / frames_per_clip), tid = threadIdx.x, lane = tid & 63, wave = tid >> 6;
    const float *pn = pts + (size_t)n * P * 3;
    for (int k = wave; k < NPATCH; k += 4) {
        const int sp = 64 * k + lane;
        float x = 3e18f, y = 3e18f, z = 3e18f;
        float lx = FLT_MAX, ly = FLT_MAX, lz = FLT_MAX, hx = -FLT_MAX, hy = -FLT_MAX, hz = -FLT_MAX;
        if (sp < P) {
            const int i = porder[(size_t)b * P + sp];
            x = pn[3 * i]; y = pn[3 * i + 1]; z = pn[3 * i + 2];
            lx = hx = x; ly = hy = y; lz = hz = z;
        }
        psort[(size_t)n * MAXP + sp] = make_float4(x, y, z, 0.f);
        lx = -wave_max(-lx); ly = -wave_max(-ly); lz = -wave_max(-lz);
        hx = wave_max(hx); hy = wave_max(hy); hz = wave_max(hz);
        if (lane == 0) {
            pbox[((size_t)n * NPATCH + k) * 2] = make_float4(lx, ly, lz, 0.f);
            pbox[((size_t)n * NPATCH + k) * 2 + 1] = make_float4(hx, hy, hz, 0.f);
        }
    }
}

__global__ __launch_bounds__(256) void opt_near_kernel(const float *__restrict__ verts, int V, int P, const float4 *__restrict__ psort,
                                                       const float4 *__restrict__ pbox, const int32_t *__restrict__ vorder,
                                                       int32_t *__restrict__ near) {
    __shared__ float4 ps[MAXP];
    __shared__ float4 bx[NPATCH * 2];
    const int64_t n = blockIdx.y;
    const int tid = threadIdx.x, pos = blockIdx.x * 256 + tid, vid = vorder[min(pos, V - 1)];
    for (int i = tid; i < MAXP; i += 256) ps[i] = psort[(size_t)n * MAXP + i];
    if (tid < NPATCH * 2) bx[tid] = pbox[(size_t)n * NPATCH * 2 + tid];
    const bool valid = pos < V;
    const float *vp = verts + ((size_t)n * V + vid) * 3;
    const float vx = vp[0], vy = vp[1], vz = vp[2];
    __syncthreads();
    const int npatch = (P + 63) / 64;
    bool hit = false;
    {
#pragma clang fp contract(off)
        const v2f VX = v2f{vx, vx}, VY = v2f{vy, vy}, VZ = v2f{vz, vz};
        for (int k = 0; k < npatch; ++k) {
            if (__builtin_amdgcn_ballot_w64(valid && !hit) == 0ull) break;
            const float4 lo = bx[2 * k], hi = bx[2 * k + 1];
            const float ex = fmaxf(fmaxf(lo.x - vx, vx - hi.x), 0.f), ey = fmaxf(fmaxf(lo.y - vy, vy - hi.y), 0.f), ez = fmaxf(fmaxf(lo.z - vz, vz - hi.z), 0.f);
            const float xx = ex * ex, yy = ey * ey, zz = ez * ez;
            if (__builtin_amdgcn_ballot_w64(valid && !hit && (xx + yy) + zz < 0.25f) == 0ull) continue;
            const float4 *pp = ps + 64 * k;
            for (int j0 = 0; j0 < 64; j0 += 16) {
#pragma unroll
                for (int j = j0; j < j0 + 16; j += 2) {
                    const float4 p = pp[j], q = pp[j + 1];
                    const v2f dx = v2f{p.x, q.x} - VX, dy = v2f{p.y, q.y} - VY, dz = v2f{p.z, q.z} - VZ;
                    const v2f d2 = (dx * dx + dy * dy) + dz * dz;
                    hit = hit || d2.x < 0.25f || d2.y < 0.25f;
                }
                if (__builtin_amdgcn_ballot_w64(valid && !hit) == 0ull) break;
            }
        }
    }
    if (valid) near[(size_t)n * V + vid] = hit ? 1 : 0;
}

}

int idf_point_order(hipStream_t s, const float *obj_points, int B, int P, int32_t *porder) {
    if (P > MAXP) return IDF_E_INVAL;
    hipLaunchKernelGGL(corr_point_order_kernel, dim3((unsigned)B), dim3(1024), 0, s, obj_points, P, porder);
    return IDF_OK;
}

int idf_nn_scan_opt(hipStream_t s, int64_t N, int frames_per_clip, const float *verts, int V, const float *pts_frame, const float *obj_points, int P,
                    const int32_t *porder, const idf_correction_ctx *c, int32_t *yidx) {
    const size_t lds = contact_lds_bytes(V);
    if (lds > 160 * 1024 - 16384 || P > MAXP || !c->vorder) return IDF_E_INVAL;
    const int B = (int)(N / frames_per_clip);
    static std::atomic<uint64_t> lds_ok{0};
    if (idf_opt_in_lds(reinterpret_cast<const void *>(corr_contact_kernel<true>), 160 * 1024 - 16384, lds_ok) != IDF_OK) return IDF_E_LAUNCH;
    hipLaunchKernelGGL(corr_contact_kernel<true>, dim3((unsigned)N, 2), dim3(CT), lds, s, verts, V, obj_points, P, porder, nullptr, nullptr, nullptr,
                       nullptr, nullptr, nullptr, nullptr, c->vorder, c->vrank, nullptr, 0, B, nullptr, nullptr, nullptr, nullptr, nullptr, yidx, nullptr, (int64_t)0,
                       pts_frame, frames_per_clip, PredArgs{});
    return IDF_OK;
}

int idf_near_mask_opt(hipStream_t s, int64_t N, int frames_per_clip, const float *verts, int V, const float *pts_frame, int P, const int32_t *porder,
                      const int32_t *vorder, float *psort, float *pbox, int32_t *near) {
    if (P > MAXP || !vorder) return IDF_E_INVAL;
    hipLaunchKernelGGL(opt_patch_kernel, dim3((unsigned)N), dim3(256), 0, s, pts_frame, P, porder, frames_per_clip, reinterpret_cast<float4 *>(psort),
                       reinterpret_cast<float4 *>(pbox));
    hipLaunchKernelGGL(opt_near_kernel, dim3((unsigned)idf_cdiv(V, 256), (unsigned)N), dim3(256), 0, s, verts, V, P, reinterpret_cast<const float4 *>(psort),
                       reinterpret_cast<const float4 *>(pbox), vorder, near);
    return IDF_OK;
}

namespace {

}

extern "C" size_t interdiff_correction_workspace_bytes(const idf_correction_ctx *c, int32_t B, int32_t T) {
    if (!c || !c->smpl || B <= 0 || T <= 0) return 0;
    return carve(c, B, T, nullptr).total;
}

static int correction_impl(const idf_correction_ctx *c, float *x0, const float *gt, const float *hand_pose,
                           const float *beta, const float *obj_points, int32_t B, int32_t T, float blend_t, const float *blend_table,
                           const int64_t *blend_state, uint8_t *condition, int32_t *contact, float *distance, float *loss, void *ws,
                           size_t ws_bytes, void *stream) {
    if (!c || !c->smpl || !c->objproj || !x0 || !gt || !hand_pose || !beta || !obj_points || !ws || B <= 0 || T <= 0) return IDF_E_INVAL;
    const int V = c->smpl->V, M = c->n_markers, P = c->n_points;
    if (c->smpl->J != 52 || c->smpl->n_betas != 10 || M > MAXM || M != c->objproj->P || P > MAXP || T != c->objproj->T ||
        c->past_len != c->objproj->past_len || c->past_len >= T)
        return IDF_E_INVAL;
    CorrWs w = carve(c, B, T, ws);
    if (ws_bytes < w.total) return IDF_E_NOMEM;
    hipStream_t s = idf_stream(stream);
    const int64_t N = (int64_t)B * T;
    const bool fused = (c->tune & 2) == 0 && idf_objproj_check(c->objproj) == IDF_OK;
    idf_prof_mark(IDF_K_CORR_PREPARE, s);
    hipLaunchKernelGGL(corr_prepare_kernel, dim3((unsigned)idf_cdiv(N * 24, 256)), dim3(256), 0, s, x0, gt, hand_pose, B, T, w.pose,
                       w.trans, w.objR, w.objT, w.gt_angles, w.gt_trans);
    int rc = interdiff_smpl_forward(c->smpl, w.pose, beta, w.trans, N, w.verts, w.jtr, nullptr, w.smpl_ws, w.smpl_ws_bytes, stream);
    if (rc) return rc;
    idf_prof_mark(IDF_K_CORR_CONTACT, s);
    PredArgs pred{};
    if (fused) {
        pred.op = *c->objproj;
        pred.obj_angles = w.gt_angles; pred.obj_trans = w.gt_trans;
        pred.markers_idx = c->markers_idx; pred.markers = w.markers; pred.keep = w.proj_keep;
        pred.nclips = B;
    }
    rc = launch_contact(s, N, w.verts, V, obj_points, P, w.porder, w.objR, w.objT, c, B, fused ? nullptr : w.markers, w.loss_sum, w.min_dist, w.label, nullptr,
                        nullptr, nullptr, (int64_t)c->past_len * B, &pred);
    if (rc) return rc;
    uint8_t *cond = condition ? condition : w.condition;
    int32_t *cont = contact ? contact : w.contact;
    idf_prof_mark(IDF_K_CORR_REDUCE, s);
    hipLaunchKernelGGL(corr_reduce_kernel, dim3(B), dim3(128), 2 * (size_t)T * sizeof(float), s, w.loss_sum, w.min_dist, w.label, B, T, c->past_len, P, M, cond,
                       cont, distance, loss);
    if (fused) {
        idf_prof_mark(IDF_K_OBJPROJ, s);
        rc = idf_objproj_pick(c->objproj, w.proj_keep, cont, B, w.proj, s);
    } else {
        rc = interdiff_objprojector_sample(c->objproj, w.gt_angles, w.gt_trans, w.markers, cont, B, w.proj, stream);
    }
    if (rc) return rc;
    idf_prof_mark(IDF_K_CORR_BLEND, s);
    hipLaunchKernelGGL(corr_blend_kernel, dim3((unsigned)idf_cdiv((int64_t)B * CTOK * T, 256)), dim3(256), 0, s, x0, w.proj, cond, B, T,
                       blend_t, blend_table, blend_state);
    idf_prof_mark(-1, s);
    IDF_CHECK_LAUNCH();
    return IDF_OK;
}

extern "C" int interdiff_correction(const idf_correction_ctx *c, float *x0, const float *gt, const float *hand_pose,
                                    const float *beta, const float *obj_points, int32_t B, int32_t T, float blend_t,
                                    uint8_t *condition, int32_t *contact, float *distance, float *loss, void *ws,
                                    size_t ws_bytes, void *stream) {
    return correction_impl(c, x0, gt, hand_pose, beta, obj_points, B, T, blend_t, nullptr, nullptr, condition, contact, distance, loss, ws, ws_bytes, stream);
}

extern "C" int interdiff_correction_dev(const idf_correction_ctx *c, float *x0, const float *gt, const float *hand_pose,
                                        const float *beta, const float *obj_points, int32_t B, int32_t T, const float *table,
                                        const int64_t *state, void *ws, size_t ws_bytes, void *stream) {
    if (!table || !state) return IDF_E_INVAL;
    return correction_impl(c, x0, gt, hand_pose, beta, obj_points, B, T, 0.f, table, state, nullptr, nullptr, nullptr, nullptr, ws, ws_bytes, stream);
}

namespace {

__global__ __launch_bounds__(256) void metrics_prepare_kernel(const float *__restrict__ obj_pred, int64_t N,
                                                              float *__restrict__ objR, float *__restrict__ objT) {
    const int64_t n = (int64_t)blockIdx.x * 256 + threadIdx.x;
    if (n >= N) return;
    float q[4], m[9];
    rot::axis_angle_to_quaternion(obj_pred + n * 6, q);
    rot::quaternion_to_matrix(q, m);
#pragma unroll
    for (int k = 0; k < 9; ++k) objR[n * 9 + k] = m[k];
#pragma unroll
    for (int k = 0; k < 3; ++k) objT[n * 3 + k] = obj_pred[n * 6 + 3 + k];
}

__device__ __forceinline__ float block_sum(float v, float *red) {
    red[threadIdx.x] = v;
    __syncthreads();
    for (int s = 128; s > 0; s >>= 1) {
        if (threadIdx.x < s) red[threadIdx.x] += red[threadIdx.x + s];
        __syncthreads();
    }
    const float r = red[0];
    __syncthreads();
    return r;
}

__global__ __launch_bounds__(256) void metrics_reduce_kernel(const float *__restrict__ obj_pred, const float *__restrict__ jtr,
                                                             const float *__restrict__ body_trans, const float *__restrict__ obj_gt,
                                                             const float *__restrict__ jtr_gt, const float *__restrict__ body_trans_gt,
                                                             const float *__restrict__ o2h, int B, int T, int J, int P,
                                                             float *__restrict__ out6) {
    __shared__ float red[256];
    const int b = blockIdx.x, tid = threadIdx.x;
    float g = 0.f, l = 0.f;
    for (int i = tid; i < T * J; i += 256) {
        const int t = i / J, j = i - t * J;
        const float *a = jtr + (((size_t)t * B + b) * J + j) * 3, *c = jtr_gt + (((size_t)t * B + b) * J + j) * 3;
        const float *a0 = jtr + ((size_t)t * B + b) * J * 3, *c0 = jtr_gt + ((size_t)t * B + b) * J * 3;
        const float dx = a[0] - c[0], dy = a[1] - c[1], dz = a[2] - c[2];
        g += sqrtf(dx * dx + dy * dy + dz * dz);
        const float ex = (a[0] - a0[0]) - (c[0] - c0[0]), ey = (a[1] - a0[1]) - (c[1] - c0[1]), ez = (a[2] - a0[2]) - (c[2] - c0[2]);
        l += sqrtf(ex * ex + ey * ey + ez * ez);
    }
    float bt = 0.f, ot = 0.f, rq = 0.f;
    for (int t = tid; t < T; t += 256) {
        const size_t n = (size_t)t * B + b;
        const float *x = body_trans + n * 3, *y = body_trans_gt + n * 3;
        bt += sqrtf((x[0] - y[0]) * (x[0] - y[0]) + (x[1] - y[1]) * (x[1] - y[1]) + (x[2] - y[2]) * (x[2] - y[2]));
        const float *p = obj_pred + n * 6, *q = obj_gt + n * 6;
        ot += sqrtf((p[3] - q[3]) * (p[3] - q[3]) + (p[4] - q[4]) * (p[4] - q[4]) + (p[5] - q[5]) * (p[5] - q[5]));
        float qa[4], qb[4];
        rot::axis_angle_to_quaternion(p, qa);
        rot::axis_angle_to_quaternion(q, qb);
        float e1 = 0.f, e2 = 0.f;
#pragma unroll
        for (int k = 0; k < 4; ++k) { e1 += fabsf(qa[k] - qb[k]); e2 += fabsf(qa[k] + qb[k]); }
        rq += fminf(e1, e2);
    }
    const float gs = block_sum(g, red), ls = block_sum(l, red), bs = block_sum(bt, red), os = block_sum(ot, red), rs = block_sum(rq, red);
    float pen = 0.f;
    for (int t = 0; t < T; ++t) {
        const float *row = o2h + ((size_t)t * B + b) * P;
        float c = 0.f;
        for (int i = tid; i < P; i += 256) c += row[i] < 0.f ? 1.f : 0.f;
        const float cs = block_sum(c, red);
        pen += cs / (float)P;
    }
    if (tid == 0) {
        out6[0 * B + b] = gs / (float)J / (float)T;
        out6[1 * B + b] = ls / (float)J / (float)T;
        out6[2 * B + b] = bs / (float)T;
        out6[3 * B + b] = os / (float)T;
        out6[4 * B + b] = rs / (float)T;
        out6[5 * B + b] = pen / (float)T;
    }
}

struct MetWs {
    float *objR, *objT, *o2h, *markers, *loss_sum, *min_dist;
    int32_t *label, *porder;
    size_t total;
};
MetWs carve_metrics(const idf_correction_ctx *c, int B, int T, void *ws) {
    const int64_t N = (int64_t)B * T;
    char *p = reinterpret_cast<char *>(ws);
    size_t off = 0;
    auto take = [&](size_t bytes) { char *r = p ? p + off : nullptr; off += idf_align(bytes); return r; };
    MetWs w;
    w.objR = (float *)take(N * 9 * 4);
    w.objT = (float *)take(N * 3 * 4);
    w.o2h = (float *)take((size_t)N * c->n_points * 4);
    w.markers = (float *)take((size_t)N * c->n_markers * 3 * 4);
    w.loss_sum = (float *)take(N * 4);
    w.min_dist = (float *)take(N * 4);
    w.label = (int32_t *)take((size_t)N * c->n_markers * 4);
    w.porder = (int32_t *)take((size_t)B * c->n_points * 4);
    w.total = off;
    return w;
}

}

extern "C" size_t interdiff_contact_nn_workspace_bytes(const idf_correction_ctx *c, int32_t B, int32_t T) {
    if (!c || B <= 0 || T <= 0) return 0;
    return carve_metrics(c, B, T, nullptr).total;
}

extern "C" int interdiff_contact_nn(const idf_correction_ctx *c, const float *verts, const float *obj_points, const float *objR,
                                    const float *objT, int32_t B, int32_t T, float *o2h, int32_t *idx, uint64_t *stats, void *ws,
                                    size_t ws_bytes, void *stream) {
    if (!c || !c->smpl || !verts || !obj_points || !objR || !objT || !ws || B <= 0 || T <= 0 || (!o2h && !idx)) return IDF_E_INVAL;
    if (c->n_markers > MAXM || c->n_points > MAXP) return IDF_E_INVAL;
    MetWs w = carve_metrics(c, B, T, ws);
    if (ws_bytes < w.total) return IDF_E_NOMEM;
    hipStream_t s = idf_stream(stream);
    if (stats && hipMemsetAsync(stats, 0, IDF_CONTACT_STATS * sizeof(uint64_t), s) != hipSuccess) return IDF_E_LAUNCH;
    const int rc = launch_contact(s, (int64_t)B * T, verts, c->smpl->V, obj_points, c->n_points, w.porder, objR, objT, c, B, w.markers, w.loss_sum,
                                  w.min_dist, w.label, o2h ? o2h : w.o2h, idx, reinterpret_cast<unsigned long long *>(stats), 0);
    if (rc) return rc;
    IDF_CHECK_LAUNCH();
    return IDF_OK;
}

extern "C" size_t interdiff_metrics_workspace_bytes(const idf_correction_ctx *c, int32_t B, int32_t T) {
    if (!c || B <= 0 || T <= 0) return 0;
    return carve_metrics(c, B, T, nullptr).total;
}

extern "C" int interdiff_metrics(const idf_correction_ctx *c, const float *obj_pred, const float *jtr, const float *body_trans,
                                 const float *obj_gt, const float *jtr_gt, const float *body_trans_gt, const float *verts,
                                 const float *obj_points, int32_t B, int32_t T, int32_t J, float *out6, void *ws, size_t ws_bytes,
                                 void *stream) {
    if (!c || !c->smpl || !obj_pred || !jtr || !body_trans || !obj_gt || !jtr_gt || !body_trans_gt || !verts || !obj_points || !out6 ||
        !ws || B <= 0 || T <= 0 || J <= 0)
        return IDF_E_INVAL;
    const int V = c->smpl->V, M = c->n_markers, P = c->n_points;
    if (M > MAXM || P > MAXP) return IDF_E_INVAL;
    MetWs w = carve_metrics(c, B, T, ws);
    if (ws_bytes < w.total) return IDF_E_NOMEM;
    hipStream_t s = idf_stream(stream);
    const int64_t N = (int64_t)B * T;
    idf_prof_mark(IDF_K_OTHER, s);
    hipLaunchKernelGGL(metrics_prepare_kernel, dim3((unsigned)idf_cdiv(N, 256)), dim3(256), 0, s, obj_pred, N, w.objR, w.objT);
    const int rc = launch_contact(s, N, verts, V, obj_points, P, w.porder, w.objR, w.objT, c, B, w.markers, w.loss_sum, w.min_dist, w.label, w.o2h,
                                  nullptr, nullptr, 0);
    if (rc) return rc;
    hipLaunchKernelGGL(metrics_reduce_kernel, dim3(B), dim3(256), 0, s, obj_pred, jtr, body_trans, obj_gt, jtr_gt, body_trans_gt, w.o2h, B,
                       T, J, P, out6);
    idf_prof_mark(-1, s);
    IDF_CHECK_LAUNCH();
    return IDF_OK;
}
```

interdiff_amd/csrc/smpl.hip:

```cpp
#include "common.h"
#include "rot_math.h"
#include <algorithm>

#ifndef IDF_SMPL_STAMP
#define IDF_SMPL_STAMP(i) do { } while (0)
#endif

namespace {

constexpr int MAXJ = 64;

__global__ __launch_bounds__(64) void smpl_pose_kernel(const idf_smpl_model m, const float *__restrict__ pose,
                                                       const float *__restrict__ betas, const float *__restrict__ trans,
                                                       float *__restrict__ feat, float *__restrict__ A,
                                                       float *__restrict__ jtr) {
    __shared__ float Rs[MAXJ * 9], Js[MAXJ * 3], Gs[MAXJ * 12];
    const int64_t n = blockIdx.x;
    const int j = threadIdx.x, J = m.J, nb = m.n_betas, KB = m.KB;
    const float *beta = betas + n * nb;
    if (j < J) {
        rot::rodrigues_smpl(pose + n * 3 * J + 3 * j, Rs + j * 9);
#pragma unroll
        for (int c = 0; c < 3; ++c) {
            float s = m.jt[j * 3 + c];
            const float *jsr = m.js + (size_t)(j * 3 + c) * nb;
            for (int k = 0; k < nb; ++k) s += jsr[k] * beta[k];
            Js[j * 3 + c] = s;
        }
    }
    float *f = feat + n * KB;
    if (j >= 1 && j < J) {
#pragma unroll
        for (int e = 0; e < 9; ++e) f[(j - 1) * 9 + e] = Rs[j * 9 + e] - ((e == 0 || e == 4 || e == 8) ? 1.0f : 0.0f);
    }
    const int base = 9 * (J - 1);
    for (int k = j; k < KB - base; k += 64) f[base + k] = k < nb ? beta[k] : (k == nb ? 1.0f : 0.0f);
    __syncthreads();
    if (j < 12) {
        const int r = j >> 2, c = j & 3;
        Gs[j] = c < 3 ? Rs[r * 3 + c] : Js[r];
    }
    __syncthreads();
    for (int i = 1; i < J; ++i) {
        const int p = m.parents[i];
        if (j < 12) {
            const int r = j >> 2, c = j & 3;
            const float *gp = Gs + p * 12 + r * 4;
            float v;
            if (c < 3)
                v = gp[0] * Rs[i * 9 + c] + gp[1] * Rs[i * 9 + 3 + c] + gp[2] * Rs[i * 9 + 6 + c];
            else
                v = gp[0] * (Js[i * 3] - Js[p * 3]) + gp[1] * (Js[i * 3 + 1] - Js[p * 3 + 1]) +
                    gp[2] * (Js[i * 3 + 2] - Js[p * 3 + 2]) + gp[3];
            Gs[i * 12 + j] = v;
        }
        __syncthreads();
    }
    if (j < J) {
        const float *g = Gs + j * 12;
        const float jx = Js[j * 3], jy = Js[j * 3 + 1], jz = Js[j * 3 + 2];
        float *a = A + ((size_t)n * J + j) * 12;
#pragma unroll
        for (int r = 0; r < 3; ++r) {
            a[r * 4 + 0] = g[r * 4 + 0];
            a[r * 4 + 1] = g[r * 4 + 1];
            a[r * 4 + 2] = g[r * 4 + 2];
            a[r * 4 + 3] = g[r * 4 + 3] - (g[r * 4] * jx + g[r * 4 + 1] * jy + g[r * 4 + 2] * jz);
            jtr[((size_t)n * J + j) * 3 + r] = g[r * 4 + 3] + trans[n * 3 + r];
        }
    }
}

constexpr int FT = 32, VT = 64, NTC = 3 * VT;
constexpr int BT = 256;
constexpr int FM = FT / 16;
constexpr int STS = NTC + 1;
constexpr int SF = 16;
constexpr int TBF = 10, TBV = 4;

template <int NG>
__global__ __launch_bounds__(BT) void smpl_blend_skin_kernel(const idf_smpl_model m, const float *__restrict__ feat,
                                                              const float *__restrict__ A, const float *__restrict__ trans,
                                                              int64_t N, float *__restrict__ verts,
                                                              float *__restrict__ v_posed) {
    extern __shared__ __attribute__((aligned(16))) float sm[];
    idf_args_now(m.V, m.J, m.S, m.blend, m.skin_idx, m.skin_w, feat, A, trans, N, verts, v_posed, gridDim.x);
    constexpr int KB = 16 * NG, nq = KB / 4;
    const int V = m.V, J = m.J, S = m.S;
    float *As = sm, *stage = sm;
    const int tid = threadIdx.x, lane = tid & 63, wave = (tid >> 6) & 3, fh = tid >> 8, li = lane & 15, kq = lane >> 4;
    const int nft = (int)((N + FT - 1) / FT), nvt = (V + VT - 1) / VT;
    const int nwg = gridDim.x, id = blockIdx.x;
    const int xq = nwg >> 3, xr = nwg & 7, xcd = id & 7;
    const int lid = (xcd < xr ? xcd * (xq + 1) : xr * (xq + 1) + (xcd - xr) * xq) + (id >> 3);
    const int blk = lid / (TBF * TBV), wi = lid - blk * (TBF * TBV);
    const int nvb = (nvt + TBV - 1) / TBV;
    const int ftile = blk / nvb * TBF + wi % TBF, vtile = blk % nvb * TBV + wi / TBF;
    if (ftile >= nft || vtile >= nvt) return;
    const int64_t f0 = (int64_t)ftile * FT;
    const int v0 = vtile * VT;
    IDF_SMPL_STAMP(0);

    {
        const uint32_t as_lds = idf_lds_addr(As);
        const int ncell = FT * nq;
        for (int i = wave; i * 64 < ncell; i += BT / 64) {
            const int p = min(i * 64 + lane, ncell - 1), row = p / nq, pos = p - row * nq;
            idf_dma16_v(feat + (size_t)min(f0 + row, N - 1) * KB + ((pos ^ ((row >> 1) & 7)) << 2), as_lds + (uint32_t)(i * 1024));
        }
    }
    const int vl = tid & 63, vme = v0 + vl;
    float sw[4];
    int so[4];
#pragma unroll
    for (int k = 0; k < 4; ++k) {
        const size_t e = (size_t)min(vme, V - 1) * S + min(k, S - 1);
        sw[k] = m.skin_w[e];
        so[k] = m.skin_idx[e] * 12;
    }
#pragma unroll
    for (int k = 0; k < 4; ++k) {
        const bool ok = k < S && vme < V;
        sw[k] = ok ? sw[k] : 0.f;
        so[k] = ok ? so[k] : 0;
    }
    asm volatile("s_waitcnt vmcnt(0)" ::: "memory");
    __syncthreads();
    IDF_SMPL_STAMP(1);

    const float *brow[3];
#pragma unroll
    for (int t = 0; t < 3; ++t) brow[t] = m.blend + ((size_t)((vtile * 4 + wave) * 3 + t) * NG * 64 + lane) * 4;
    f32x4 acc[FM][3];
#pragma unroll
    for (int i = 0; i < FM; ++i)
#pragma unroll
        for (int t = 0; t < 3; ++t) acc[i][t] = f32x4{0.f, 0.f, 0.f, 0.f};
    constexpr int PD = 3;
    float4 bq[PD + 1][3];
    auto ldg = [&](float4 (&dst)[3], int gi) {
#pragma unroll
        for (int t = 0; t < 3; ++t) dst[t] = *reinterpret_cast<const float4 *>(brow[t] + gi * 256);
    };
    auto mac = [&](const float4 (&bc)[3], int gi) {
#pragma unroll
        for (int i = 0; i < FM; ++i) {
            const int row = (fh * FM + i) * 16 + li;
            const float4 a = *reinterpret_cast<const float4 *>(As + row * KB + (((gi * 4 + kq) ^ ((row >> 1) & 7)) << 2));
#pragma unroll
            for (int t = 0; t < 3; ++t) acc[i][t] = __builtin_amdgcn_mfma_f32_16x16x4f32(a.x, bc[t].x, acc[i][t], 0, 0, 0);
#pragma unroll
            for (int t = 0; t < 3; ++t) acc[i][t] = __builtin_amdgcn_mfma_f32_16x16x4f32(a.y, bc[t].y, acc[i][t], 0, 0, 0);
#pragma unroll
            for (int t = 0; t < 3; ++t) acc[i][t] = __builtin_amdgcn_mfma_f32_16x16x4f32(a.z, bc[t].z, acc[i][t], 0, 0, 0);
#pragma unroll
            for (int t = 0; t < 3; ++t) acc[i][t] = __builtin_amdgcn_mfma_f32_16x16x4f32(a.w, bc[t].w, acc[i][t], 0, 0, 0);
        }
    };
#pragma unroll
    for (int g = 0; g < PD && g < NG; ++g) ldg(bq[g], g);
#pragma unroll
    for (int g = 0; g < NG; ++g) {
        if (g + PD < NG) ldg(bq[(g + PD) % (PD + 1)], g + PD);
        __builtin_amdgcn_sched_barrier(0);
        mac(bq[g % (PD + 1)], g);
        __builtin_amdgcn_sched_barrier(0);
    }
    __syncthreads();
    IDF_SMPL_STAMP(2);
#pragma unroll
    for (int i = 0; i < FM; ++i)
#pragma unroll
        for (int t = 0; t < 3; ++t)
#pragma unroll
            for (int r = 0; r < 4; ++r) stage[((fh * FM + i) * 16 + kq * 4 + r) * STS + (wave * 3 + t) * 16 + li] = acc[i][t][r];

    float *Asub = sm + ((FT * STS + 255) & ~255);
    float *ost = Asub + ((SF * J * 12 + 255) & ~255);
    float *trs = ost + SF * NTC;
    const int arow = J * 12;
    if (tid < FT * 3) trs[tid] = trans[min(f0 + tid / 3, N - 1) * 3 + tid % 3];
    for (int sub = 0; sub < FT / SF; ++sub) {
        const int64_t fs = f0 + sub * SF;
        if (fs >= N) break;
        __syncthreads();
        {
            const uint32_t asub_lds = idf_lds_addr(Asub);
            const float *src = idf_uniform_ptr(A + (size_t)fs * arow);
            for (int i = wave; i * 256 < SF * arow; i += BT / 64) idf_dma16_s(src + (size_t)i * 256, (uint32_t)(lane << 4), asub_lds + (uint32_t)(i * 1024));
            asm volatile("s_waitcnt vmcnt(0)" ::: "memory");
        }
        __syncthreads();
        IDF_SMPL_STAMP(3 + 3 * sub);
#pragma unroll
        for (int k = 0; k < SF * VT / BT; ++k) {
            const int f = (tid >> 6) + (BT / 64) * k, fr = sub * SF + f;
            const float px = stage[fr * STS + 3 * vl], py = stage[fr * STS + 3 * vl + 1], pz = stage[fr * STS + 3 * vl + 2];
            float4 t0 = make_float4(0.f, 0.f, 0.f, 0.f), t1 = t0, t2 = t0;
            const float *Af = Asub + f * arow;
#pragma unroll
            for (int b = 0; b < 4; ++b) {
                if (b < S) {
                    const float w = sw[b];
                    const float4 *a = reinterpret_cast<const float4 *>(Af + so[b]);
                    const float4 a0 = a[0], a1 = a[1], a2 = a[2];
                    t0.x = fmaf(w, a0.x, t0.x); t0.y = fmaf(w, a0.y, t0.y); t0.z = fmaf(w, a0.z, t0.z); t0.w = fmaf(w, a0.w, t0.w);
                    t1.x = fmaf(w, a1.x, t1.x); t1.y = fmaf(w, a1.y, t1.y); t1.z = fmaf(w, a1.z, t1.z); t1.w = fmaf(w, a1.w, t1.w);
                    t2.x = fmaf(w, a2.x, t2.x); t2.y = fmaf(w, a2.y, t2.y); t2.z = fmaf(w, a2.z, t2.z); t2.w = fmaf(w, a2.w, t2.w);
                }
            }
            float *o = ost + f * NTC + 3 * vl;
            o[0] = fmaf(t0.x, px, fmaf(t0.y, py, fmaf(t0.z, pz, t0.w))) + trs[fr * 3 + 0];
            o[1] = fmaf(t1.x, px, fmaf(t1.y, py, fmaf(t1.z, pz, t1.w))) + trs[fr * 3 + 1];
            o[2] = fmaf(t2.x, px, fmaf(t2.y, py, fmaf(t2.z, pz, t2.w))) + trs[fr * 3 + 2];
        }
        __syncthreads();
        IDF_SMPL_STAMP(4 + 3 * sub);
        const int nvalid = min(VT, V - v0) * 3;
        for (int idx = tid; idx < SF * (NTC / 2); idx += BT) {
            const int f = idx / (NTC / 2), c2 = (idx - f * (NTC / 2)) * 2;
            if (fs + f >= N || c2 >= nvalid) continue;
            const size_t go = ((size_t)(fs + f) * V + v0) * 3 + c2;
            *reinterpret_cast<float2 *>(verts + go) = *reinterpret_cast<const float2 *>(ost + f * NTC + c2);
            if (v_posed) *reinterpret_cast<float2 *>(v_posed + go) = make_float2(stage[(sub * SF + f) * STS + c2], stage[(sub * SF + f) * STS + c2 + 1]);
        }
        IDF_SMPL_STAMP(5 + 3 * sub);
    }
}

}

extern "C" size_t interdiff_smpl_workspace_bytes(const idf_smpl_model *m, int64_t N) {
    if (!m || N < 0) return 0;
    return idf_align((size_t)N * m->KB * sizeof(float)) + idf_align(((size_t)N + SF) * m->J * 12 * sizeof(float));
}

extern "C" int interdiff_smpl_forward(const idf_smpl_model *m, const float *pose, const float *betas, const float *trans,
                                      int64_t N, float *verts, float *jtr, float *v_posed, void *ws, size_t ws_bytes,
                                      void *stream) {
    if (!m || !pose || !betas || !trans || !verts || !jtr || !ws || N < 0) return IDF_E_INVAL;
    if (m->J < 1 || m->J > MAXJ || m->KB % 16 != 0 || m->KB < 9 * (m->J - 1) + m->n_betas + 1 || m->S < 1) return IDF_E_INVAL;
    if (ws_bytes < interdiff_smpl_workspace_bytes(m, N)) return IDF_E_NOMEM;
    if (N == 0) return IDF_OK;
    hipStream_t s = idf_stream(stream);
    float *feat = reinterpret_cast<float *>(ws);
    float *A = reinterpret_cast<float *>(reinterpret_cast<char *>(ws) + idf_align((size_t)N * m->KB * sizeof(float)));
    idf_prof_mark(IDF_K_SMPL_POSE, s);
    hipLaunchKernelGGL(smpl_pose_kernel, dim3((unsigned)N), dim3(64), 0, s, *m, pose, betas, trans, feat, A, jtr);
    const size_t lds = std::max((size_t)FT * m->KB, (size_t)((FT * STS + 255) & ~255) + ((SF * m->J * 12 + 255) & ~255) + (size_t)SF * NTC + FT * 3) * sizeof(float);
    if (lds > 150 * 1024 || m->KB % 32 != 0 || (m->V * 3) % 2 != 0 || m->S > 4) return IDF_E_INVAL;
    if (m->KB != 480) return IDF_E_INVAL;
    static std::atomic<uint64_t> lds_ok{0};
    if (lds > 64 * 1024 && idf_opt_in_lds(reinterpret_cast<const void *>(smpl_blend_skin_kernel<30>), 150 * 1024, lds_ok) != IDF_OK) return IDF_E_LAUNCH;
    idf_prof_mark(IDF_K_SMPL_BLEND_SKIN, s);
    const unsigned nwg_launch = (unsigned)(idf_cdiv(idf_cdiv(N, FT), TBF) * idf_cdiv(idf_cdiv(m->V, VT), TBV) * TBF * TBV);
    hipLaunchKernelGGL(smpl_blend_skin_kernel<30>, dim3(nwg_launch), dim3(BT), lds, s, *m,
                       feat, A, trans, N, verts, v_posed);
    idf_prof_mark(-1, s);
    IDF_CHECK_LAUNCH();
    return IDF_OK;
}
```

interdiff_amd/diffusion.py:

```python
import itertools
import math
import os
import numpy as np
import torch
from . import _lib
from . import graph_sampler


def get_named_beta_schedule(schedule_name, num_diffusion_timesteps, scale_betas=1.):
    n = num_diffusion_timesteps
    if schedule_name == 'linear':
        scale = scale_betas * 1000 / n
        return np.linspace(scale * 0.0001, scale * 0.02, n, dtype=np.float64)
    if schedule_name == 'cosine':
        abar = lambda t: math.cos((t + 0.008) / 1.008 * math.pi / 2) ** 2
        return np.array([min(1 - abar((i + 1) / n) / abar(i / n), 0.999) for i in range(n)], dtype=np.float64)
    raise NotImplementedError('unknown beta schedule: %s' % schedule_name)


GRAPH_BLOCKS = (49, 7, 1)
SPLIT_MAX_BATCH = int(os.environ.get('INTERDIFF_SPLIT_MAX_BATCH', 128))
N_CHAINS = int(os.environ.get('INTERDIFF_CHAINS', 2))
MAX_GRAPH_SHAPES = 8
_UID = itertools.count(1)


def fresh_seed():
    return int(torch.randint(0, 2 ** 62, (1,), dtype=torch.int64).item())


def mask_operands(mask, gt, like):
    if mask is None or gt is None:
        return None, None
    assert like.shape == mask.shape == gt.shape
    return (mask if mask.dtype == torch.uint8 else mask.view(torch.uint8)).contiguous(), gt.contiguous()


def inpaint(x, gt, mask_u8):
    _lib.check(_lib.load().interdiff_inpaint(_lib.dptr(x, torch.float32), _lib.dptr(gt, torch.float32), _lib.dptr(mask_u8), x.numel(), _lib.stream()), 'inpaint')


def seeded_state(t_start, seed, elem0):
    return torch.tensor([t_start, 0, int(seed) & 0x7FFFFFFFFFFFFFFF, 0, 0, 0, elem0, 0], dtype=torch.int64)


def space_timesteps(num_timesteps, section_counts):
    if isinstance(section_counts, str):
        if section_counts.startswith('ddim'):
            want = int(section_counts[len('ddim'):])
            for stride in range(1, num_timesteps):
                if len(range(0, num_timesteps, stride)) == want:
                    return set(range(0, num_timesteps, stride))
            raise ValueError('cannot create exactly %d steps with an integer stride' % num_timesteps)
        section_counts = [int(c) for c in section_counts.split(',')]
    size_per, extra = divmod(num_timesteps, len(section_counts))
    start, kept = 0, []
    for k, count in enumerate(section_counts):
        size = size_per + (1 if k < extra else 0)
        if size < count:
            raise ValueError('cannot divide section of %d steps into %d' % (size, count))
        stride = 1 if count <= 1 else (size - 1) / (count - 1)
        kept += [start + round(cur) for cur in _strided(stride, count)]
        start += size
    return set(kept)


def _strided(stride, count):
    cur = 0.0
    for _ in range(count):
        yield cur
        cur += stride


def ddim_coefficients(alphas_cumprod, alphas_cumprod_prev, eta):
    ab, abp = np.asarray(alphas_cumprod, np.float64), np.asarray(alphas_cumprod_prev, np.float64)
    sigma = float(eta) * np.sqrt((1.0 - abp) / (1.0 - ab)) * np.sqrt(1.0 - ab / abp)
    k = np.sqrt(np.maximum(1.0 - abp - sigma ** 2, 0.0)) / np.sqrt(1.0 / ab - 1.0)
    return np.sqrt(abp) - k, k * np.sqrt(1.0 / ab), sigma


class GaussianDiffusion:

    def __init__(self, betas):
        betas = np.array(betas, dtype=np.float64)
        assert betas.ndim == 1 and (betas > 0).all() and (betas <= 1).all()
        self.betas = betas
        self.num_timesteps = int(betas.shape[0])
        alphas = 1.0 - betas
        self.alphas_cumprod = np.cumprod(alphas, axis=0)
        self.alphas_cumprod_prev = np.append(1.0, self.alphas_cumprod[:-1])
        self.posterior_variance = betas * (1.0 - self.alphas_cumprod_prev) / (1.0 - self.alphas_cumprod)
        self.posterior_log_variance_clipped = np.log(np.append(self.posterior_variance[1], self.posterior_variance[1:]))
        self.posterior_mean_coef1 = betas * np.sqrt(self.alphas_cumprod_prev) / (1.0 - self.alphas_cumprod)
        self.posterior_mean_coef2 = (1.0 - self.alphas_cumprod_prev) * np.sqrt(alphas) / (1.0 - self.alphas_cumprod)
        self._c1 = self.posterior_mean_coef1.astype(np.float32)
        self._c2 = self.posterior_mean_coef2.astype(np.float32)
        self._sigma = np.exp(np.float32(0.5) * self.posterior_log_variance_clipped.astype(np.float32)).astype(np.float32)
        self.sqrt_alphas_cumprod = np.sqrt(self.alphas_cumprod)
        self.sqrt_one_minus_alphas_cumprod = np.sqrt(1.0 - self.alphas_cumprod)
        self.timestep_map = list(range(self.num_timesteps))
        self.original_num_steps = self.num_timesteps
        self.identity_tmap_is_null = True
        self._t_cache = {}
        self._tables = {}
        self._rows_cache = {}
        self._tmaps = {}
        self._q_tables = {}
        self.fuse_plain_step = True
        self.chain_plain_steps = os.environ.get('INTERDIFF_CHAIN_STEPS', '1') != '0'
        self.split_chains = True
        self.split_min_rows = None
        self._uid = next(_UID)

    @property
    def is_respaced(self):
        return self.timestep_map != list(range(self.num_timesteps))

    def _timesteps(self, B, device, loop_side=False):
        key = (B, str(device), bool(loop_side) and self.is_respaced)
        if key not in self._t_cache:
            vals = torch.tensor(self.timestep_map, dtype=torch.int64) if not key[2] and self.is_respaced else torch.arange(self.num_timesteps, dtype=torch.int64)
            self._t_cache[key] = vals.to(device)[:, None].repeat(1, B).contiguous()
        return self._t_cache[key]

    def _tmap(self, device):
        if not self.is_respaced and self.identity_tmap_is_null:
            return None
        key = str(device)
        if key not in self._tmaps:
            self._tmaps[key] = torch.tensor(self.timestep_map, dtype=torch.int64).to(device)
        return self._tmaps[key]

    def _rows(self, sampler=('ddpm',)):
        if sampler not in self._rows_cache:
            if sampler[0] == 'ddpm':
                c1, c2, sig = self._c1, self._c2, self._sigma.copy()
            else:
                c1, c2, sig = (v.astype(np.float32) for v in ddim_coefficients(self.alphas_cumprod, self.alphas_cumprod_prev, sampler[1]))
            sig[0] = 0.0
            blend = (np.arange(self.num_timesteps, dtype=np.float32) / np.float32(1000)).astype(np.float32)
            self._rows_cache[sampler] = np.ascontiguousarray(np.stack([c1, c2, sig, blend], axis=1).astype(np.float32))
        return self._rows_cache[sampler]

    def _table(self, device, sampler=('ddpm',)):
        key = (str(device), sampler)
        if key not in self._tables:
            self._tables[key] = torch.from_numpy(self._rows(sampler)).to(device)
        return self._tables[key]

    def _step(self, model, img, x0_buf, i, it, t, model_kwargs, denoised_fn, noise_i, seed, elem0=0, rows_kw={}, t_hook=None, rows=None):
        lib = _lib.load()
        y = model_kwargs.get('y', {})
        x0 = model(img, t, **model_kwargs, **rows_kw)
        mu8, gc = mask_operands(y.get('inpainting_mask'), y.get('inpainted_motion'), x0)
        if mu8 is not None:
            inpaint(x0, gc, mu8)
        if denoised_fn is not None:
            x0 = denoised_fn(x0, t if t_hook is None else t_hook, model_kwargs)
        c1, c2, sigma = (float(v) for v in (self._rows() if rows is None else rows)[i, :3])
        _lib.check(lib.interdiff_posterior_step_at(_lib.dptr(img, torch.float32), _lib.dptr(x0, torch.float32),
                                                   _lib.dptr(noise_i, torch.float32, allow_none=True), img.numel(),
                                                   c1, c2, sigma, seed, it, elem0, _lib.stream()),
                   'posterior_step')
        return x0

    def p_sample_loop(self, model, shape, noise=None, clip_denoised=True, denoised_fn=None, cond_fn=None, model_kwargs=None,
                      device=None, progress=False, skip_timesteps=0, init_image=None, randomize_class=False,
                      cond_fn_with_grad=False, dump_steps=None, const_noise=False, step_noise=None, seed=None, n_steps=None,
                      use_graph=True, first_t=None, shard=None):
        return self._sample_loop(('ddpm',), model, shape, noise, clip_denoised, denoised_fn, cond_fn, model_kwargs, device, skip_timesteps,
                                 init_image, randomize_class, cond_fn_with_grad, dump_steps, const_noise, step_noise, seed, n_steps, use_graph,
                                 first_t, shard)

    def ddim_sample_loop(self, model, shape, noise=None, clip_denoised=True, denoised_fn=None, cond_fn=None, model_kwargs=None,
                         device=None, progress=False, eta=0.0, skip_timesteps=0, init_image=None, randomize_class=False,
                         cond_fn_with_grad=False, dump_steps=None, const_noise=False, step_noise=None, seed=None, n_steps=None,
                         use_graph=True, first_t=None, shard=None):
        return self._sample_loop(('ddim', float(eta)), model, shape, noise, clip_denoised, denoised_fn, cond_fn, model_kwargs, device,
                                 skip_timesteps, init_image, randomize_class, cond_fn_with_grad, dump_steps, const_noise, step_noise, seed,
                                 n_steps, use_graph, first_t, shard)

    def _sample_loop(self, sampler, model, shape, noise, clip_denoised, denoised_fn, cond_fn, model_kwargs, device, skip_timesteps, init_image,
                     randomize_class, cond_fn_with_grad, dump_steps, const_noise, step_noise, seed, n_steps, use_graph, first_t, shard):
        if clip_denoised:
            raise NotImplementedError('clip_denoised=True is not used on the eval path (eval_smpl_short.py:153)')
        if cond_fn is not None or skip_timesteps or init_image is not None or randomize_class or cond_fn_with_grad or const_noise:
            raise NotImplementedError('only noise=, denoised_fn=, model_kwargs=, dump_steps= are live (SURVEY.md §8(b))')
        if model_kwargs is None:
            model_kwargs = {}
        if seed is None:
            seed = fresh_seed()
        if device is None:
            device = next(model.parameters()).device
        assert isinstance(shape, (tuple, list))
        if shard is not None:
            shard = (int(shard[0]), int(shard[1]))
            if not 0 <= shard[0] <= shard[0] + shape[0] <= shard[1]:
                raise ValueError('shard=(first_clip, total_clips) must contain this batch of %d clips' % shape[0])
        first, total = (0, shape[0]) if shard is None else shard
        per_clip = int(np.prod(shape[1:]))
        elem0 = first * per_clip
        if shard is not None and elem0 % 4:
            raise ValueError('a shard must start at a multiple of 4 elements (C * T = %d per clip)' % per_clip)
        if noise is not None:
            img = noise.clone().contiguous().float()
        else:
            img = torch.empty(*shape, dtype=torch.float32, device=device)
            _lib.check(_lib.load().interdiff_randn_at(_lib.dptr(img), img.numel(), seed, 0xFFFFFFFF, elem0, _lib.stream()), 'randn')
            y = model_kwargs.get('y', {})
            mu8, gc = mask_operands(y.get('inpainting_mask'), y.get('inpainted_motion'), img) if sampler[0] == 'ddpm' else (None, None)
            if mu8 is not None:
                inpaint(img, gc, mu8)
        t_first = self.num_timesteps - 1 if first_t is None else int(first_t)
        if not 0 <= t_first < self.num_timesteps:
            raise ValueError('first_t outside the schedule')
        todo = t_first + 1 if n_steps is None else min(int(n_steps), t_first + 1)
        if (step_noise is None and use_graph and getattr(model, 'graph_safe', False) and img.is_cuda
                and 'cond' in model_kwargs.get('y', {}) and os.environ.get('INTERDIFF_NO_GRAPH') != '1'):
            return graph_sampler.sample(self, model, img, model_kwargs, denoised_fn, seed, todo, dump_steps, t_first, shard, sampler)
        rows_kw = {'batch_rows': total * shape[-1]} if shard is not None and getattr(model, 'accepts_batch_rows', False) else {}
        ts, ts_hook, rows = self._timesteps(shape[0], device), self._timesteps(shape[0], device, loop_side=True), self._rows(sampler)
        dump = []
        cond = model_kwargs.get('y', {}).get('cond') if isinstance(model_kwargs.get('y', None), dict) else None
        if cond is not None and hasattr(model, 'prepare_memory'):
            model.prepare_memory(cond)
        for it, i in enumerate(range(t_first, t_first - todo, -1)):
            t, th = ts[i], ts_hook[i]
            t.host_value = th.host_value = i
            if step_noise is None:
                nz = None
            elif callable(step_noise):
                nz = step_noise(it, img).contiguous()
            else:
                nz = step_noise[it]
            self._step(model, img, None, i, it, t, model_kwargs, denoised_fn, nz, seed, elem0, rows_kw, th, rows)
            if dump_steps is not None and it in dump_steps:
                dump.append(img.clone())
        return dump if dump_steps is not None else img

    def sample_timesteps(self, B, device, generator=None):
        gdev = generator.device if generator is not None else device
        t = torch.randint(0, self.num_timesteps, (B,), dtype=torch.int64, device=gdev, generator=generator).to(device)
        return t, torch.ones(B, dtype=torch.float32, device=device)

    def q_sample(self, x_start, t, noise=None, seed=None, inpainted_motion=None, inpainting_mask=None, elem0=0):
        lib = _lib.load()
        x0 = x_start.contiguous()
        if x0.dtype != torch.float32:
            raise ValueError('x_start must be float32')
        B = x0.shape[0]
        if tuple(t.shape) != (B,):
            raise ValueError('t must be [B]')
        if not t.is_cuda:
            if int(t.min()) < 0 or int(t.max()) >= self.num_timesteps:
                raise ValueError('t outside the schedule')
            t = t.to(x0.device)
        key = str(x0.device)
        if key not in self._q_tables:
            self._q_tables[key] = tuple(torch.from_numpy(v.astype(np.float32)).to(x0.device) for v in (self.sqrt_alphas_cumprod, self.sqrt_one_minus_alphas_cumprod))
        sa, s1 = self._q_tables[key]
        if (inpainted_motion is None) != (inpainting_mask is None):
            raise ValueError('inpainted_motion and inpainting_mask go together')
        mu8, gc = mask_operands(inpainting_mask, inpainted_motion, x0)
        if noise is not None:
            assert noise.shape == x0.shape
            noise = noise.contiguous()
        elif seed is None:
            seed = fresh_seed()
        x_t = torch.empty_like(x0)
        _lib.check(lib.interdiff_q_sample(_lib.dptr(x_t), _lib.dptr(x0), _lib.dptr(noise, torch.float32, allow_none=True),
                                          _lib.dptr(t.contiguous(), torch.int64), _lib.dptr(sa), _lib.dptr(s1), self.num_timesteps,
                                          _lib.dptr(gc, torch.float32, allow_none=True), _lib.dptr(mu8, allow_none=True), B, x0.numel() // B,
                                          int(seed or 0) & 0xFFFFFFFFFFFFFFFF, int(elem0), _lib.stream()), 'q_sample')
        return x_t

    def training_losses(self, model, x_start, t, model_kwargs=None, noise=None, seed=None):
        if model_kwargs is None:
            model_kwargs = {}
        y = model_kwargs.get('y', {})
        both = 'inpainting_mask' in y and 'inpainted_motion' in y
        x_t = self.q_sample(x_start, t, noise=noise, seed=seed, inpainted_motion=y['inpainted_motion'] if both else None,
                            inpainting_mask=y['inpainting_mask'] if both else None)
        t = t.to(x_t.device)
        if self.is_respaced:
            t = torch.tensor(self.timestep_map, dtype=torch.int64, device=x_t.device)[t]
        model_output = model(x_t, t, **model_kwargs)
        assert model_output.shape == x_start.shape
        return model_output, x_start


def sample_loop(diffusion, model, shape, sampler='ddpm', eta=0.0, **kw):
    if sampler == 'ddpm':
        return diffusion.p_sample_loop(model, shape, **kw)
    if sampler == 'ddim':
        return diffusion.ddim_sample_loop(model, shape, eta=eta, **kw)
    raise ValueError("sampler must be 'ddpm' or 'ddim'")


class SpacedDiffusion(GaussianDiffusion):

    def __init__(self, use_timesteps, betas, rescale_timesteps=False):
        if rescale_timesteps:
            raise NotImplementedError('rescale_timesteps=True is not built (the reference configuration is False: model/diffusion_smpl.py:258)')
        base = GaussianDiffusion(betas)
        self.use_timesteps = set(use_timesteps)
        last, new_betas, tmap = 1.0, [], []
        for i, ac in enumerate(base.alphas_cumprod):
            if i in self.use_timesteps:
                new_betas.append(1 - ac / last)
                last = ac
                tmap.append(i)
        super().__init__(np.array(new_betas))
        self.timestep_map, self.original_num_steps, self.rescale_timesteps = tmap, len(base.betas), False


def create_gaussian_diffusion(noise_schedule='cosine', diffusion_steps=1000, timestep_respacing=''):
    betas = get_named_beta_schedule(noise_schedule, diffusion_steps, 1.)
    if not timestep_respacing:
        timestep_respacing = [diffusion_steps]
    return SpacedDiffusion(space_timesteps(diffusion_steps, timestep_respacing), betas)
```

interdiff_amd/graph_sampler.py:

```python
import os
import torch
from . import _lib, diffusion

HOOK_KEYS = ('hand_pose', 'beta', 'obj_points')


def plan_steps(t_start, todo, active, dump_steps, fuse_hook):
    blocks = diffusion.GRAPH_BLOCKS
    dumps = () if dump_steps is None else dump_steps
    ops, i, it, end = [], t_start, 0, t_start - todo
    while i > end:
        if active(i):
            ops.append(('hook', 0) if fuse_hook else ('eager_hook',))
            k = 1
        else:
            run = 1
            while i - run > end and not active(i - run) and (it + run - 1) not in dumps:
                run += 1
            k = next(b for b in blocks if b <= run)
            if fuse_hook and k == run and i - run > end and active(i - run) and (it + k - 1) not in dumps:
                ops.append(('hook', k))
                k += 1
            else:
                ops.append(('plain', k))
        i -= k
        it += k
        if (it - 1) in dumps:
            ops.append(('dump', it - 1))
    return ops


def capture(enqueue, *args):
    g = torch.cuda.CUDAGraph()
    with torch.cuda.graph(g):
        enqueue(*args)
    return g


def posterior_update(x, x0, gt, mask, table, state, ts, tmap=None):
    _lib.check(_lib.load().interdiff_posterior_step_dev_map(_lib.dptr(x), _lib.dptr(x0), _lib.dptr(gt, allow_none=True), _lib.dptr(mask, allow_none=True),
                                                            x.numel(), _lib.dptr(table), _lib.dptr(tmap, torch.int64, allow_none=True), _lib.dptr(state),
                                                            _lib.dptr(ts), ts.numel(), _lib.stream()),
               'posterior_step_dev')


class Chain:

    def __init__(self, model, entry, sl, own_state):
        dev, h, mem_len = entry.x.device, sl.stop - sl.start, entry.cond.shape[0]
        self.sl = sl
        self.x, self.ts = entry.x[sl], entry.ts[sl]
        self.gt = None if entry.gt is None else entry.gt[sl]
        self.mask = None if entry.mask is None else entry.mask[sl]
        self.kwargs = {} if entry.zpo is None else {'zero_pose_obj': entry.zpo[sl]}
        self.state = torch.zeros(8, dtype=torch.int64, device=dev) if own_state else entry.state
        self.cond = torch.empty(mem_len, h, entry.cond.shape[2], device=dev)
        self.memctx = torch.empty(model.memctx_floats(h, mem_len), dtype=torch.float32, device=dev)
        self.ws = torch.empty(model.workspace_bytes(h, entry.x.shape[-1]), dtype=torch.uint8, device=dev)
        self.stream = torch.cuda.Stream(dev)


class HookBuffers:

    def __init__(self, hook, entry, y, shapes):
        B, T = entry.x.shape[0], entry.x.shape[-1]
        self.shapes = shapes
        self.ws = hook.workspace_for(B, T)
        self.y = {k: torch.empty(y[k].shape, dtype=torch.float32, device=entry.x.device) for k in HOOK_KEYS}
        self.y['inpainted_motion'] = entry.gt if entry.gt is not None else torch.empty_like(entry.x)
        self.fresh = True


class Entry:

    def __init__(self, img, cond, has_mask, zpo):
        dev = img.device
        self.x, self.x0 = torch.zeros_like(img), torch.empty_like(img)
        self.ts = torch.zeros(img.shape[0], dtype=torch.int64, device=dev)
        self.state = torch.zeros(8, dtype=torch.int64, device=dev)
        self.cond = torch.empty_like(cond, memory_format=torch.contiguous_format)
        self.gt = torch.empty_like(img) if has_mask else None
        self.mask = torch.empty(img.shape, dtype=torch.uint8, device=dev) if has_mask else None
        self.zpo = None if zpo is None else torch.empty(zpo.shape, dtype=torch.float32, device=dev)
        self.kwargs = {'y': {'cond': self.cond}}
        if zpo is not None:
            self.kwargs['zero_pose_obj'] = self.zpo
        self.graphs = {}
        self.chains = []
        self.hooks = {}
        self.chain_steps = None
        self.pool_keys = ()

    @staticmethod
    def of(model, key, img, cond, has_mask, zpo):
        cache = model.__dict__.setdefault('_graph_cache', {})
        entry = cache.get(key)
        if entry is not None:
            return entry, False
        entry = Entry(img, cond, has_mask, zpo)
        if len(cache) >= diffusion.MAX_GRAPH_SHAPES:
            evicted = list(cache.values())
            cache.clear()
            for old in evicted:
                model.forget_shape_buffers(old.pool_keys)
        cache[key] = entry
        return entry, True

    def load(self, cond, zpo, gt, mask):
        self.cond.copy_(cond)
        if zpo is not None:
            self.zpo.copy_(zpo)
        if mask is not None:
            self.gt.copy_(gt)
            self.mask.copy_(mask)

    def warm_up(self, model, table, rows, tmap=None):
        model(self.x, self.ts, out=self.x0, **self.kwargs, batch_rows=rows)
        if model.supports_forward_step:
            t0 = min(2, table.shape[0] - 1)
            x, ts, state = self.x.clone(), self.ts.clone(), diffusion.seeded_state(t0, 1, 0).to(self.x.device)
            model.forward_step(x, ts, table, state, gt=self.gt, mask=self.mask, tmap=tmap, **self.kwargs, batch_rows=rows)
            if model.step_chaining:
                state.copy_(diffusion.seeded_state(t0, 1, 0))
                ts.copy_(self.ts)
                model.forward_step(x, ts, table, state, gt=self.gt, mask=self.mask, tmap=tmap, embed_next=True, **self.kwargs, batch_rows=rows)
                model.forward_step(x, ts, table, state, gt=self.gt, mask=self.mask, tmap=tmap, embed_ready=True, **self.kwargs, batch_rows=rows)
        torch.cuda.synchronize(self.x.device)

    def split_into_chains(self, model, n):
        B = self.x.shape[0]
        for c in range(n):
            start = c * (B // n) + min(c, B % n)
            self.chains.append(Chain(model, self, slice(start, start + B // n + (1 if c < B % n else 0)), own_state=c > 0))

    def hook_buffers(self, hook, y, table):
        shapes = tuple(tuple(y[k].shape) for k in HOOK_KEYS)
        hk = self.hooks.get(hook._uid)
        if hk is None or hk.shapes != shapes:
            hk = self.hooks[hook._uid] = HookBuffers(hook, self, y, shapes)
            for stale in [gk for gk in self.graphs if isinstance(gk, tuple) and gk[0] == 'hook' and gk[1] == hook._uid]:
                del self.graphs[stale]
        for k in HOOK_KEYS + (() if self.gt is not None else ('inpainted_motion',)):
            hk.y[k].copy_(y[k])
        if hk.fresh:
            hook.apply_dev(hk.y['inpainted_motion'].clone(), table, torch.zeros(8, dtype=torch.int64, device=self.x.device), hk.y, hk.ws)
            torch.cuda.synchronize(self.x.device)
            hk.fresh = False
        return hk


def hook_capturable(hook, y):
    return (hook is not None and getattr(hook, 'graph_capturable', False) and getattr(hook, 'debug', None) is None
            and getattr(hook, 'is_active', None) is not None and all(k in y for k in ('inpainted_motion',) + HOOK_KEYS)
            and os.environ.get('INTERDIFF_EAGER_HOOK') != '1')


def hook_gate(hook):
    if hook is None:
        return lambda t: False
    return getattr(hook, 'is_active', None) or (lambda t: True)


class Run:

    def __init__(self, model, entry, table, rows, fused, split, hook, hk, tmap=None):
        self.model, self.entry, self.table, self.rows, self.tmap = model, entry, table, rows, tmap
        self.fused, self.split, self.hook, self.hk = fused, split, hook, hk

    def enqueue_forward(self):
        st = self.entry
        self.model(st.x, st.ts, out=st.x0, **st.kwargs, batch_rows=self.rows)

    def enqueue_plain(self, k):
        st, model = self.entry, self.model
        links = [dict(embed_ready=i > 0, embed_next=i + 1 < k) if st.chain_steps else {} for i in range(k)]
        if self.split:
            cur = torch.cuda.current_stream()
            for ch in st.chains:
                ch.stream.wait_stream(cur)
                with torch.cuda.stream(ch.stream):
                    for link in links:
                        model.forward_step(ch.x, ch.ts, self.table, ch.state, gt=ch.gt, mask=ch.mask, tmap=self.tmap, memctx=ch.memctx, ws=ch.ws, batch_rows=self.rows, **link, **ch.kwargs)
            for ch in st.chains:
                cur.wait_stream(ch.stream)
        elif self.fused:
            for link in links:
                model.forward_step(st.x, st.ts, self.table, st.state, gt=st.gt, mask=st.mask, tmap=self.tmap, **link, **st.kwargs, batch_rows=self.rows)
        else:
            for _ in links:
                self.enqueue_forward()
                posterior_update(st.x, st.x0, st.gt, st.mask, self.table, st.state, st.ts, self.tmap)

    def finish_hook_step(self, x0):
        st = self.entry
        posterior_update(st.x, x0, None, None, self.table, st.state, st.ts, self.tmap)
        if self.split:
            for ch in st.chains[1:]:
                ch.state[:6].copy_(st.state[:6])

    def enqueue_hook_block(self, k):
        st = self.entry
        if k:
            self.enqueue_plain(k)
        self.enqueue_forward()
        if st.mask is not None:
            diffusion.inpaint(st.x0, st.gt, st.mask)
        self.hook.apply_dev(st.x0, self.table, st.state, self.hk.y, self.hk.ws)
        self.finish_hook_step(st.x0)

    def graph(self, key, enqueue, *args):
        graphs = self.entry.graphs
        if key not in graphs:
            graphs[key] = capture(enqueue, *args)
        return graphs[key]

    def plain_block(self, k):
        return self.graph((k, self.fused, self.split), self.enqueue_plain, k)

    def hook_block(self, k):
        return self.graph(('hook', self.hook._uid, k, self.fused, self.split), self.enqueue_hook_block, k)

    def eager_hook_step(self, t, model_kwargs):
        st = self.entry
        self.graph('fwd', self.enqueue_forward).replay()
        if st.mask is not None:
            diffusion.inpaint(st.x0, st.gt, st.mask)
        self.finish_hook_step(self.hook(st.x0, t, model_kwargs).contiguous())

    def play(self, plan, t_start, ts_all, model_kwargs):
        st, dump, i = self.entry, [], t_start
        for op in plan:
            if op[0] == 'plain':
                self.plain_block(op[1]).replay()
                i -= op[1]
            elif op[0] == 'hook':
                self.hook_block(op[1]).replay()
                i -= op[1] + 1
            elif op[0] == 'eager_hook':
                t = ts_all[i]
                t.host_value = i
                self.eager_hook_step(t, model_kwargs)
                i -= 1
            else:
                dump.append(st.x.clone())
        return dump


def sample(diff, model, img, model_kwargs, hook, seed, todo, dump_steps, t_start, shard=None, sampler=('ddpm',)):
    y = model_kwargs.get('y', {})
    B, T, dev = img.shape[0], img.shape[-1], img.device
    first, total = (0, B) if shard is None else shard
    per_clip = img.numel() // B
    elem0 = first * per_clip
    rows = total * T
    table, tmap = diff._table(dev, sampler), diff._tmap(dev)
    mask, gt = diffusion.mask_operands(y.get('inpainting_mask'), y.get('inpainted_motion'), img)
    cond, zpo = y['cond'], model_kwargs.get('zero_pose_obj')
    key = (diff._uid, tuple(img.shape), mask is not None, tuple(cond.shape), model.ffn_graph_key(rows)) + (() if sampler == ('ddpm',) and tmap is None else (sampler, tmap is not None))
    if zpo is not None:
        key += (tuple(zpo.shape),)
    st, fresh = Entry.of(model, key, img, cond, mask is not None, zpo)
    st.load(cond, zpo, gt, mask)
    pools_before = model.shape_buffer_keys() if fresh else None
    model.prepare_memory(st.cond)
    if fresh:
        st.warm_up(model, table, rows, tmap)
        st.pool_keys = model.shape_buffer_keys() - pools_before

    fused = diff.fuse_plain_step and model.supports_forward_step
    nch = diffusion.N_CHAINS
    split = (fused and diff.split_chains and nch > 1 and 2 * nch <= B <= diffusion.SPLIT_MAX_BATCH
             and B * T > (model.one_chain_max_rows() if diff.split_min_rows is None else diff.split_min_rows))
    if split:
        if not st.chains:
            st.split_into_chains(model, nch)
        for ch in st.chains:
            ch.cond.copy_(st.cond[:, ch.sl])
            model.prepare_memory(ch.cond, into=ch.memctx)
    chain_steps = diff.chain_plain_steps and fused and model.step_chaining
    if st.chain_steps != chain_steps:
        st.graphs.clear()
        st.chain_steps = chain_steps
    fuse_hook = hook_capturable(hook, y)
    run = Run(model, st, table, rows, fused, split, hook, st.hook_buffers(hook, y, table) if fuse_hook else None, tmap)

    st.x.copy_(img)
    st.state.copy_(diffusion.seeded_state(t_start, seed, elem0))
    if split:
        for ch in st.chains[1:]:
            ch.state.copy_(diffusion.seeded_state(t_start, seed, elem0 + ch.sl.start * per_clip))
    st.ts.fill_(diff.timestep_map[t_start])
    dump = run.play(plan_steps(t_start, todo, hook_gate(hook), dump_steps, fuse_hook), t_start, diff._timesteps(B, dev, loop_side=True), model_kwargs)
    return dump if dump_steps is not None else st.x.clone()
```

interdiff_amd/smpl.py:

```python
import ctypes as C
import numpy as np
import torch
from . import _lib


def _np(a):
    return a.detach().cpu().numpy() if isinstance(a, torch.Tensor) else np.asarray(a)


def pack_smpl_model(model, device):
    vt = _np(model['v_template']).astype(np.float64).reshape(-1, 3)
    sdirs = _np(model['shapedirs']).astype(np.float64)
    pdirs = _np(model['posedirs']).astype(np.float64)
    jreg = _np(model['J_regressor']).astype(np.float64)
    wts = _np(model['weights']).astype(np.float32)
    parents = _np(model['parents']).astype(np.int64).copy()
    V, J, nb = vt.shape[0], wts.shape[1], sdirs.shape[2]
    kp = 9 * (J - 1)
    if pdirs.shape != (V, 3, kp) or jreg.shape != (J, V):
        raise ValueError('inconsistent SMPL buffers')
    KB = (kp + nb + 1 + 15) // 16 * 16
    blend = np.zeros((3 * V, KB), np.float32)
    blend[:, :kp] = pdirs.reshape(3 * V, kp)
    blend[:, kp:kp + nb] = sdirs.reshape(3 * V, nb)
    blend[:, kp + nb] = vt.reshape(3 * V)
    jt = (jreg @ vt).astype(np.float32)
    js = np.einsum('jv,vck->jck', jreg, sdirs).astype(np.float32)
    nnz = (wts != 0)
    S = max(1, int(nnz.sum(1).max()))
    skin_idx = np.zeros((V, S), np.int32)
    skin_w = np.zeros((V, S), np.float32)
    for v in range(V):
        js_ = np.nonzero(nnz[v])[0]
        skin_idx[v, :len(js_)] = js_
        skin_w[v, :len(js_)] = wts[v, js_]
    parents[0] = 0
    t = lambda a: torch.from_numpy(np.ascontiguousarray(a)).to(device)
    nvt = -(-V // 64)
    rows = np.zeros((nvt * 192, KB), np.float32)
    rows[:3 * V] = blend
    frag = rows.reshape(nvt, 4, 3, 16, KB // 16, 4, 4).transpose(0, 1, 2, 4, 5, 3, 6)
    bufs = dict(blend=t(frag), blend_rows=t(blend), jt=t(jt), js=t(js), parents=t(parents.astype(np.int32)), skin_idx=t(skin_idx), skin_w=t(skin_w))
    m = _lib.SmplModel()
    m.V, m.J, m.n_betas, m.KB, m.S = V, J, nb, KB, S
    for k, v in bufs.items():
        if k != 'blend_rows':
            setattr(m, k, v.data_ptr())
    return m, bufs


class SMPL_Layer:
    def __init__(self, model, device='cuda'):
        self.lib = _lib.load()
        self.device = torch.device(device)
        self.cmodel, self._bufs = pack_smpl_model(model, self.device)
        self.th_faces = torch.from_numpy(_np(model['faces']).astype(np.int64)).to(self.device)
        self.v_template = _np(model['v_template']).astype(np.float32).reshape(-1, 3)
        self.num_joints = self.cmodel.J
        self.kintree_parents = [int(p) for p in _np(model['parents'])]
        self._ws = None

    def _workspace(self, N):
        need = self.lib.interdiff_smpl_workspace_bytes(C.byref(self.cmodel), N)
        if self._ws is None or self._ws.numel() < need:
            self._ws = torch.empty(max(need, 256), dtype=torch.uint8, device=self.device)
        return self._ws

    def forward(self, th_pose_axisang, th_betas=None, th_trans=None, th_offsets=None, scale=1., want_v_posed=True):
        if th_offsets is not None or scale != 1.:
            raise NotImplementedError('th_offsets / scale are not used on the eval_smpl_short path')
        N = th_pose_axisang.shape[0]
        J, V, nb = self.cmodel.J, self.cmodel.V, self.cmodel.n_betas
        if th_pose_axisang.shape[1] != 3 * J:
            raise ValueError('pose must be [N,%d]' % (3 * J))
        if th_betas is None:
            th_betas = torch.zeros(N, nb, device=self.device)
        if th_trans is None:
            th_trans = torch.zeros(N, 3, device=self.device)
        pose, betas, trans = (a.contiguous().float() for a in (th_pose_axisang, th_betas, th_trans))
        verts = torch.empty(N, V, 3, dtype=torch.float32, device=self.device)
        jtr = torch.empty(N, J, 3, dtype=torch.float32, device=self.device)
        v_posed = torch.empty(N, V, 3, dtype=torch.float32, device=self.device) if want_v_posed else None
        ws = self._workspace(N)
        _lib.check(self.lib.interdiff_smpl_forward(C.byref(self.cmodel), _lib.dptr(pose, torch.float32), _lib.dptr(betas, torch.float32),
                                                   _lib.dptr(trans, torch.float32), N, _lib.dptr(verts), _lib.dptr(jtr),
                                                   _lib.dptr(v_posed, allow_none=True), _lib.dptr(ws), ws.numel(), _lib.stream()),
                   'smpl_forward')
        return verts, jtr, v_posed, v_posed

    __call__ = forward
```

Measured before the change: 7.128 million.

## Precompute constant hand-joint and shape blend contribution once per sample in SMPL correction

```diff
diff --git a/include/interdiff_hip.h b/include/interdiff_hip.h
--- a/include/interdiff_hip.h
+++ b/include/interdiff_hip.h
@@ -25,6 +25,7 @@
 
 typedef struct {
     int32_t V, J, n_betas, KB, S;
+    int32_t n_const_joints;
     const float   *blend;
     const float   *jt;
     const float   *js;
@@ -37,6 +38,12 @@
 int interdiff_smpl_forward(const idf_smpl_model *m, const float *pose, const float *betas,
                            const float *trans, int64_t N, float *verts, float *jtr,
                            float *v_posed, void *ws, size_t ws_bytes, void *stream);
+size_t interdiff_smpl_base_bytes(const idf_smpl_model *m, int64_t N);
+int interdiff_smpl_blend_base(const idf_smpl_model *m, const float *pose, const float *betas, int64_t N, float *base,
+                              void *ws, size_t ws_bytes, void *stream);
+int interdiff_smpl_forward_based(const idf_smpl_model *m, const float *pose, const float *betas, const float *trans,
+                                 int64_t N, const float *base, float *verts, float *jtr, float *v_posed,
+                                 void *ws, size_t ws_bytes, void *stream);
 
 int interdiff_vertex_normals(const float *verts, int64_t N, int32_t V, const int32_t *faces,
                              const int32_t *adj_ptr, const int32_t *adj_face,
@@ -198,6 +205,9 @@
 int interdiff_correction_dev(const idf_correction_ctx *c, float *x0, const float *gt, const float *hand_pose,
                              const float *beta, const float *obj_points, int32_t B, int32_t T, const float *table,
                              const int64_t *state, void *ws, size_t ws_bytes, void *stream);
+int interdiff_correction_begin_sample(const idf_correction_ctx *c, const float *hand_pose, const float *beta, int32_t B, int32_t T,
+                                      void *ws, size_t ws_bytes, void *stream);
+int interdiff_correction_end_sample(void *ws);
 
 #define IDF_CONTACT_STATS 12
 size_t interdiff_contact_nn_workspace_bytes(const idf_correction_ctx *c, int32_t B, int32_t T);
diff --git a/interdiff_amd/_lib.py b/interdiff_amd/_lib.py
--- a/interdiff_amd/_lib.py
+++ b/interdiff_amd/_lib.py
@@ -16,7 +16,7 @@
 
 
 class SmplModel(C.Structure):
-    _fields_ = [('V', i32), ('J', i32), ('n_betas', i32), ('KB', i32), ('S', i32),
+    _fields_ = [('V', i32), ('J', i32), ('n_betas', i32), ('KB', i32), ('S', i32), ('n_const_joints', i32),
                 ('blend', vp), ('jt', vp), ('js', vp), ('parents', vp), ('skin_idx', vp), ('skin_w', vp)]
 
 
@@ -107,6 +107,9 @@
     'interdiff_rotation_6d_to_axis_angle': (C.c_int, [vp, vp, i64, vp]),
     'interdiff_smpl_workspace_bytes': (sz, [C.POINTER(SmplModel), i64]),
     'interdiff_smpl_forward': (C.c_int, [C.POINTER(SmplModel), vp, vp, vp, i64, vp, vp, vp, vp, sz, vp]),
+    'interdiff_smpl_base_bytes': (sz, [C.POINTER(SmplModel), i64]),
+    'interdiff_smpl_blend_base': (C.c_int, [C.POINTER(SmplModel), vp, vp, i64, vp, vp, sz, vp]),
+    'interdiff_smpl_forward_based': (C.c_int, [C.POINTER(SmplModel), vp, vp, vp, i64, vp, vp, vp, vp, vp, sz, vp]),
     'interdiff_vertex_normals': (C.c_int, [vp, i64, i32, vp, vp, vp, vp, vp, vp]),
     'interdiff_nn_argmin': (C.c_int, [vp, i32, vp, i32, i64, vp, vp]),
     'interdiff_point2point_signed': (C.c_int, [vp, i32, vp, i32, i64, vp, vp, vp, vp, vp, vp, vp, vp, vp]),
@@ -140,6 +143,8 @@
     'interdiff_correction': (C.c_int, [C.POINTER(CorrectionCtx), vp, vp, vp, vp, vp, i32, i32, f32,
                                        vp, vp, vp, vp, vp, sz, vp]),
     'interdiff_correction_dev': (C.c_int, [C.POINTER(CorrectionCtx), vp, vp, vp, vp, vp, i32, i32, vp, vp, vp, sz, vp]),
+    'interdiff_correction_begin_sample': (C.c_int, [C.POINTER(CorrectionCtx), vp, vp, i32, i32, vp, sz, vp]),
+    'interdiff_correction_end_sample': (C.c_int, [vp]),
     'interdiff_metrics_workspace_bytes': (sz, [C.POINTER(CorrectionCtx), i32, i32]),
     'interdiff_metrics': (C.c_int, [C.POINTER(CorrectionCtx), vp, vp, vp, vp, vp, vp, vp, vp, i32, i32, i32,
                                     vp, vp, sz, vp]),
diff --git a/interdiff_amd/correction.py b/interdiff_amd/correction.py
--- a/interdiff_amd/correction.py
+++ b/interdiff_amd/correction.py
@@ -1,6 +1,7 @@
 import ctypes as C
 import os
 import itertools
+import weakref
 import numpy as np
 import torch
 from . import _lib
@@ -20,6 +21,11 @@
 
 def correction_gate(t0):
     return not (t0 > 500 or t0 % 50 != 0)
+
+
+def _forget_base(lib, keys, ptr):
+    keys.pop(ptr, None)
+    lib.interdiff_correction_end_sample(ptr)
 
 
 class HipCorrection:
@@ -44,18 +50,51 @@
         ctx.tune = 0
         self.ctx = ctx
         self._ws = {}
+        self._base = {}
         self.debug = None
         self._uid = next(_UID)
 
     graph_capturable = True
 
     def workspace_for(self, B, T):
-        return torch.empty(self.lib.interdiff_correction_workspace_bytes(C.byref(self.ctx), B, T), dtype=torch.uint8, device=self.device)
+        return self._track(torch.empty(self.lib.interdiff_correction_workspace_bytes(C.byref(self.ctx), B, T), dtype=torch.uint8, device=self.device))
+
+    def _track(self, ws):
+        weakref.finalize(ws, _forget_base, self.lib, self._base, ws.data_ptr())
+        return ws
+
+    @staticmethod
+    def _base_key(hp, beta):
+        return tuple((a.data_ptr(), a._version, tuple(a.shape)) for a in (hp, beta))
+
+    def begin_sample(self, y, ws=None):
+        hp, beta = y['hand_pose'].contiguous().float(), y['beta'].contiguous().float()
+        T, B = hp.shape[:2]
+        if ws is None:
+            ws = self._workspace(B, T)
+        _forget_base(self.lib, self._base, ws.data_ptr())
+        if hp is not y['hand_pose'] or beta is not y['beta']:
+            return
+        _lib.check(self.lib.interdiff_correction_begin_sample(C.byref(self.ctx), _lib.dptr(hp, torch.float32), _lib.dptr(beta, torch.float32), B, T,
+                                                              _lib.dptr(ws), ws.numel(), _lib.stream()), 'correction_begin_sample')
+        self._base[ws.data_ptr()] = self._base_key(hp, beta)
+
+    def end_sample(self, ws=None):
+        if ws is None:
+            ws = self._ws.get(torch.cuda.current_stream(self.device).cuda_stream)
+        if ws is not None:
+            _forget_base(self.lib, self._base, ws.data_ptr())
+
+    def _check_base(self, ws, y, hp, beta):
+        key = self._base.get(ws.data_ptr())
+        if key is not None and (hp is not y['hand_pose'] or beta is not y['beta'] or key != self._base_key(hp, beta)):
+            _forget_base(self.lib, self._base, ws.data_ptr())
 
     def apply_dev(self, x, table, state, y, ws):
         B, _, Cc, T = x.shape
         if y['obj_points'].shape[1] != self.ctx.n_points:
             raise ValueError('obj_points must have %d points' % self.ctx.n_points)
+        self._check_base(ws, y, y['hand_pose'], y['beta'])
         _lib.check(self.lib.interdiff_correction_dev(C.byref(self.ctx), _lib.dptr(x, torch.float32), _lib.dptr(y['inpainted_motion'], torch.float32),
                                                      _lib.dptr(y['hand_pose'], torch.float32), _lib.dptr(y['beta'], torch.float32),
                                                      _lib.dptr(y['obj_points'], torch.float32), B, T, _lib.dptr(table), _lib.dptr(state),
@@ -67,7 +106,7 @@
         key = torch.cuda.current_stream(self.device).cuda_stream
         ws = self._ws.pop(key, None)
         if ws is None or ws.numel() < need:
-            ws = torch.empty(need, dtype=torch.uint8, device=self.device)
+            ws = self._track(torch.empty(need, dtype=torch.uint8, device=self.device))
         self._ws[key] = ws
         if len(self._ws) > self.MAX_STREAM_WORKSPACES:
             torch.cuda.synchronize(self.device)
@@ -85,6 +124,7 @@
         gt = y['inpainted_motion'].contiguous()
         hp, beta, pts = y['hand_pose'].contiguous().float(), y['beta'].contiguous().float(), y['obj_points'].contiguous().float()
         ws = self._workspace(B, T)
+        self._check_base(ws, y, hp, beta)
         dbg = [None] * 4
         if self.debug is not None:
             dbg = [torch.empty(B, dtype=torch.uint8, device=self.device), torch.empty(B, len(MARKERS67), dtype=torch.int32, device=self.device),
diff --git a/interdiff_amd/csrc/common.h b/interdiff_amd/csrc/common.h
--- a/interdiff_amd/csrc/common.h
+++ b/interdiff_amd/csrc/common.h
@@ -22,6 +22,12 @@
 static inline hipStream_t idf_stream(void *s) { return reinterpret_cast<hipStream_t>(s); }
 static inline int64_t idf_cdiv(int64_t a, int64_t b) { return (a + b - 1) / b; }
 static inline size_t idf_align(size_t x, size_t a = 256) { return (x + a - 1) / a * a; }
+
+__host__ __device__ static inline int idf_smpl_kconst(const idf_smpl_model &m) { return (9 * m.n_const_joints + m.n_betas + 15) / 16 * 16; }
+__host__ __device__ static inline int idf_smpl_feat_col(const idf_smpl_model &m, int j) {
+    const int nvar = m.J - 1 - m.n_const_joints;
+    return j > nvar ? 9 * (j - 1 - nvar) : idf_smpl_kconst(m) + 9 * (j - 1);
+}
 
 static inline int idf_opt_in_lds(const void *fn, int bytes, std::atomic<uint64_t> &done) {
     int dev = 0;
diff --git a/interdiff_amd/csrc/correction.hip b/interdiff_amd/csrc/correction.hip
--- a/interdiff_amd/csrc/correction.hip
+++ b/interdiff_amd/csrc/correction.hip
@@ -633,6 +633,7 @@
     int32_t *label, *contact, *porder;
     uint8_t *condition;
     void *smpl_ws;
+    float *base;
     size_t smpl_ws_bytes, total;
 };
 
@@ -662,8 +663,38 @@
     w.proj_keep = (float *)take((size_t)B * idf_objproj_keep_floats() * 4);
     w.smpl_ws_bytes = interdiff_smpl_workspace_bytes(c->smpl, N);
     w.smpl_ws = take(w.smpl_ws_bytes);
+    w.base = (float *)take(interdiff_smpl_base_bytes(c->smpl, N));
     w.total = off;
     return w;
+}
+
+struct BaseRecord {
+    const void *ws, *smpl, *blend, *hand_pose, *beta;
+    int32_t B, T;
+};
+std::mutex g_base_mu;
+std::vector<BaseRecord> g_base;
+
+void base_drop(const void *ws) {
+    std::lock_guard<std::mutex> lk(g_base_mu);
+    for (size_t i = 0; i < g_base.size(); ++i)
+        if (g_base[i].ws == ws) { g_base[i] = g_base.back(); g_base.pop_back(); return; }
+}
+
+bool base_valid(const BaseRecord &want) {
+    std::lock_guard<std::mutex> lk(g_base_mu);
+    for (const BaseRecord &r : g_base)
+        if (r.ws == want.ws)
+            return r.smpl == want.smpl && r.blend == want.blend && r.hand_pose == want.hand_pose && r.beta == want.beta && r.B == want.B && r.T == want.T;
+    return false;
+}
+
+__global__ __launch_bounds__(256) void corr_base_pose_kernel(const float *__restrict__ hand_pose, int64_t N, float *__restrict__ pose) {
+    const int64_t i = (int64_t)blockIdx.x * 256 + threadIdx.x;
+    if (i >= N * 156) return;
+    const int64_t n = i / 156;
+    const int k = (int)(i - n * 156);
+    pose[i] = k < 66 ? 0.f : hand_pose[n * 90 + (k - 66)];
 }
 
 
@@ -789,7 +820,8 @@
     idf_prof_mark(IDF_K_CORR_PREPARE, s);
     hipLaunchKernelGGL(corr_prepare_kernel, dim3((unsigned)idf_cdiv(N * 24, 256)), dim3(256), 0, s, x0, gt, hand_pose, B, T, w.pose,
                        w.trans, w.objR, w.objT, w.gt_angles, w.gt_trans);
-    int rc = interdiff_smpl_forward(c->smpl, w.pose, beta, w.trans, N, w.verts, w.jtr, nullptr, w.smpl_ws, w.smpl_ws_bytes, stream);
+    const bool based = base_valid(BaseRecord{ws, c->smpl, c->smpl->blend, hand_pose, beta, B, T});
+    int rc = interdiff_smpl_forward_based(c->smpl, w.pose, beta, w.trans, N, based ? w.base : nullptr, w.verts, w.jtr, nullptr, w.smpl_ws, w.smpl_ws_bytes, stream);
     if (rc) return rc;
     idf_prof_mark(IDF_K_CORR_CONTACT, s);
     PredArgs pred{};
@@ -819,6 +851,28 @@
                        blend_t, blend_table, blend_state);
     idf_prof_mark(-1, s);
     IDF_CHECK_LAUNCH();
+    return IDF_OK;
+}
+
+extern "C" int interdiff_correction_begin_sample(const idf_correction_ctx *c, const float *hand_pose, const float *beta, int32_t B, int32_t T,
+                                                 void *ws, size_t ws_bytes, void *stream) {
+    if (!c || !c->smpl || !hand_pose || !beta || !ws || B <= 0 || T <= 0) return IDF_E_INVAL;
+    if (c->smpl->J != 52 || c->smpl->n_betas != 10 || c->smpl->n_const_joints != 52 - NBODY) return IDF_E_INVAL;
+    CorrWs w = carve(c, B, T, ws);
+    if (ws_bytes < w.total) return IDF_E_NOMEM;
+    base_drop(ws);
+    hipStream_t s = idf_stream(stream);
+    const int64_t N = (int64_t)B * T;
+    idf_prof_mark(IDF_K_CORR_PREPARE, s);
+    hipLaunchKernelGGL(corr_base_pose_kernel, dim3((unsigned)idf_cdiv(N * 156, 256)), dim3(256), 0, s, hand_pose, N, w.pose);
+    if (int rc = interdiff_smpl_blend_base(c->smpl, w.pose, beta, N, w.base, w.smpl_ws, w.smpl_ws_bytes, stream)) return rc;
+    std::lock_guard<std::mutex> lk(g_base_mu);
+    g_base.push_back(BaseRecord{ws, c->smpl, c->smpl->blend, hand_pose, beta, B, T});
+    return IDF_OK;
+}
+
+extern "C" int interdiff_correction_end_sample(void *ws) {
+    base_drop(ws);
     return IDF_OK;
 }
 
diff --git a/interdiff_amd/csrc/smpl.hip b/interdiff_amd/csrc/smpl.hip
--- a/interdiff_amd/csrc/smpl.hip
+++ b/interdiff_amd/csrc/smpl.hip
@@ -13,7 +13,7 @@
 __global__ __launch_bounds__(64) void smpl_pose_kernel(const idf_smpl_model m, const float *__restrict__ pose,
                                                        const float *__restrict__ betas, const float *__restrict__ trans,
                                                        float *__restrict__ feat, float *__restrict__ A,
-                                                       float *__restrict__ jtr) {
+                                                       float *__restrict__ jtr, int split) {
     __shared__ float Rs[MAXJ * 9], Js[MAXJ * 3], Gs[MAXJ * 12];
     const int64_t n = blockIdx.x;
     const int j = threadIdx.x, J = m.J, nb = m.n_betas, KB = m.KB;
@@ -30,11 +30,18 @@
     }
     float *f = feat + n * KB;
     if (j >= 1 && j < J) {
-#pragma unroll
-        for (int e = 0; e < 9; ++e) f[(j - 1) * 9 + e] = Rs[j * 9 + e] - ((e == 0 || e == 4 || e == 8) ? 1.0f : 0.0f);
-    }
-    const int base = 9 * (J - 1);
-    for (int k = j; k < KB - base; k += 64) f[base + k] = k < nb ? beta[k] : (k == nb ? 1.0f : 0.0f);
+        const int col = split ? idf_smpl_feat_col(m, j) : 9 * (j - 1);
+#pragma unroll
+        for (int e = 0; e < 9; ++e) f[col + e] = Rs[j * 9 + e] - ((e == 0 || e == 4 || e == 8) ? 1.0f : 0.0f);
+    }
+    if (split) {
+        const int cb = 9 * m.n_const_joints, kc = idf_smpl_kconst(m), vb = kc + 9 * (J - 1 - m.n_const_joints);
+        for (int k = j; k < kc - cb; k += 64) f[cb + k] = k < nb ? beta[k] : 0.0f;
+        for (int k = vb + j; k < KB; k += 64) f[k] = k == vb ? 1.0f : 0.0f;
+    } else {
+        const int base = 9 * (J - 1);
+        for (int k = j; k < KB - base; k += 64) f[base + k] = k < nb ? beta[k] : (k == nb ? 1.0f : 0.0f);
+    }
     __syncthreads();
     if (j < 12) {
         const int r = j >> 2, c = j & 3;
@@ -66,7 +73,7 @@
             a[r * 4 + 1] = g[r * 4 + 1];
             a[r * 4 + 2] = g[r * 4 + 2];
             a[r * 4 + 3] = g[r * 4 + 3] - (g[r * 4] * jx + g[r * 4 + 1] * jy + g[r * 4 + 2] * jz);
-            jtr[((size_t)n * J + j) * 3 + r] = g[r * 4 + 3] + trans[n * 3 + r];
+            if (jtr) jtr[((size_t)n * J + j) * 3 + r] = g[r * 4 + 3] + trans[n * 3 + r];
         }
     }
 }
@@ -78,13 +85,14 @@
 constexpr int SF = 16;
 constexpr int TBF = 10, TBV = 4;
 
-template <int NG>
+enum { SMPL_FULL = 0, SMPL_BASED = 1, SMPL_SNAP = 2 };
+template <int NG, int K0, int MODE>
 __global__ __launch_bounds__(BT) void smpl_blend_skin_kernel(const idf_smpl_model m, const float *__restrict__ feat,
                                                               const float *__restrict__ A, const float *__restrict__ trans,
                                                               int64_t N, float *__restrict__ verts,
-                                                              float *__restrict__ v_posed) {
+                                                              float *__restrict__ v_posed, float *__restrict__ base) {
     extern __shared__ __attribute__((aligned(16))) float sm[];
-    idf_args_now(m.V, m.J, m.S, m.blend, m.skin_idx, m.skin_w, feat, A, trans, N, verts, v_posed, gridDim.x);
+    idf_args_now(m.V, m.J, m.S, m.blend, m.skin_idx, m.skin_w, feat, A, trans, N, verts, v_posed, base, gridDim.x);
     constexpr int KB = 16 * NG, nq = KB / 4;
     const int V = m.V, J = m.J, S = m.S;
     float *As = sm, *stage = sm;
@@ -100,6 +108,17 @@
     const int64_t f0 = (int64_t)ftile * FT;
     const int v0 = vtile * VT;
     IDF_SMPL_STAMP(0);
+    constexpr bool SNAP = MODE == SMPL_SNAP;
+    constexpr int G0 = MODE == SMPL_BASED ? K0 : 0, G1 = SNAP ? K0 : NG;
+    f32x4 acc[FM][3];
+    f32x4 *snap = reinterpret_cast<f32x4 *>(base) + ((size_t)(ftile * nvt + vtile) * (BT / 64) + wave) * (FM * 3 * 64) + lane;
+#pragma unroll
+    for (int i = 0; i < FM; ++i)
+#pragma unroll
+        for (int t = 0; t < 3; ++t) {
+            if constexpr (MODE == SMPL_BASED) acc[i][t] = snap[(i * 3 + t) * 64];
+            else acc[i][t] = f32x4{0.f, 0.f, 0.f, 0.f};
+        }
 
     {
         const uint32_t as_lds = idf_lds_addr(As);
@@ -131,11 +150,6 @@
     const float *brow[3];
 #pragma unroll
     for (int t = 0; t < 3; ++t) brow[t] = m.blend + ((size_t)((vtile * 4 + wave) * 3 + t) * NG * 64 + lane) * 4;
-    f32x4 acc[FM][3];
-#pragma unroll
-    for (int i = 0; i < FM; ++i)
-#pragma unroll
-        for (int t = 0; t < 3; ++t) acc[i][t] = f32x4{0.f, 0.f, 0.f, 0.f};
     constexpr int PD = 3;
     float4 bq[PD + 1][3];
     auto ldg = [&](float4 (&dst)[3], int gi) {
@@ -158,13 +172,20 @@
         }
     };
 #pragma unroll
-    for (int g = 0; g < PD && g < NG; ++g) ldg(bq[g], g);
-#pragma unroll
-    for (int g = 0; g < NG; ++g) {
-        if (g + PD < NG) ldg(bq[(g + PD) % (PD + 1)], g + PD);
+    for (int g = G0; g < G0 + PD && g < G1; ++g) ldg(bq[g % (PD + 1)], g);
+#pragma unroll
+    for (int g = G0; g < G1; ++g) {
+        if (g + PD < G1) ldg(bq[(g + PD) % (PD + 1)], g + PD);
         __builtin_amdgcn_sched_barrier(0);
         mac(bq[g % (PD + 1)], g);
         __builtin_amdgcn_sched_barrier(0);
+    }
+    if constexpr (SNAP) {
+#pragma unroll
+        for (int i = 0; i < FM; ++i)
+#pragma unroll
+            for (int t = 0; t < 3; ++t) snap[(i * 3 + t) * 64] = acc[i][t];
+        return;
     }
     __syncthreads();
     IDF_SMPL_STAMP(2);
@@ -235,28 +256,101 @@
     return idf_align((size_t)N * m->KB * sizeof(float)) + idf_align(((size_t)N + SF) * m->J * 12 * sizeof(float));
 }
 
-extern "C" int interdiff_smpl_forward(const idf_smpl_model *m, const float *pose, const float *betas, const float *trans,
-                                      int64_t N, float *verts, float *jtr, float *v_posed, void *ws, size_t ws_bytes,
-                                      void *stream) {
-    if (!m || !pose || !betas || !trans || !verts || !jtr || !ws || N < 0) return IDF_E_INVAL;
-    if (m->J < 1 || m->J > MAXJ || m->KB % 16 != 0 || m->KB < 9 * (m->J - 1) + m->n_betas + 1 || m->S < 1) return IDF_E_INVAL;
+extern "C" size_t interdiff_smpl_base_bytes(const idf_smpl_model *m, int64_t N) {
+    if (!m || N < 0) return 0;
+    return (size_t)idf_cdiv(N, FT) * (size_t)idf_cdiv(m->V, VT) * FT * NTC * sizeof(float);
+}
+
+namespace {
+
+constexpr int NG_H = 30, K0_H = 18;
+
+int smpl_check(const idf_smpl_model *m) {
+    if (m->J < 1 || m->J > MAXJ || m->n_const_joints < 0 || m->n_const_joints > m->J - 1 || m->S < 1) return IDF_E_INVAL;
+    if (m->KB % 16 != 0 || m->KB < 9 * (m->J - 1) + m->n_betas + 1) return IDF_E_INVAL;
+    return IDF_OK;
+}
+
+int smpl_split_model(const idf_smpl_model *m, idf_smpl_model *ms) {
+    if (m->n_const_joints < 1 || m->KB != idf_smpl_kconst(*m) + idf_cdiv(9 * (m->J - 1 - m->n_const_joints) + 1, 16) * 16) return IDF_E_INVAL;
+    *ms = *m;
+    ms->blend = m->blend + (size_t)idf_cdiv(m->V, VT) * NTC * m->KB;
+    return IDF_OK;
+}
+
+template <bool SNAP>
+int launch_blend_skin(const idf_smpl_model *m, bool split, const float *feat, const float *A, const float *trans, int64_t N, float *verts,
+                      float *v_posed, float *base, hipStream_t s) {
+    const size_t lds = SNAP ? (size_t)FT * m->KB * sizeof(float)
+                            : std::max((size_t)FT * m->KB, (size_t)((FT * STS + 255) & ~255) + ((SF * m->J * 12 + 255) & ~255) + (size_t)SF * NTC + FT * 3) * sizeof(float);
+    if (lds > 150 * 1024 || m->KB % 32 != 0 || (m->V * 3) % 2 != 0 || m->S > 4) return IDF_E_INVAL;
+    if (m->KB != 16 * NG_H) return IDF_E_INVAL;
+    if (split && idf_smpl_kconst(*m) != 16 * K0_H) return IDF_E_INVAL;
+    const unsigned nwg_launch = (unsigned)(idf_cdiv(idf_cdiv(N, FT), TBF) * idf_cdiv(idf_cdiv(m->V, VT), TBV) * TBF * TBV);
+    auto go = [&](auto kern, std::atomic<uint64_t> &lds_ok) {
+        if (lds > 64 * 1024 && idf_opt_in_lds(reinterpret_cast<const void *>(kern), 150 * 1024, lds_ok) != IDF_OK) return IDF_E_LAUNCH;
+        idf_prof_mark(IDF_K_SMPL_BLEND_SKIN, s);
+        hipLaunchKernelGGL(kern, dim3(nwg_launch), dim3(BT), lds, s, *m, feat, A, trans, N, verts, v_posed, base);
+        return IDF_OK;
+    };
+    static std::atomic<uint64_t> ok_full{0}, ok_based{0}, ok_snap{0};
+    if (SNAP) return go(smpl_blend_skin_kernel<NG_H, K0_H, SMPL_SNAP>, ok_snap);
+    return base ? go(smpl_blend_skin_kernel<NG_H, K0_H, SMPL_BASED>, ok_based) : go(smpl_blend_skin_kernel<NG_H, K0_H, SMPL_FULL>, ok_full);
+}
+
+}
+
+extern "C" int interdiff_smpl_blend_base(const idf_smpl_model *m, const float *pose, const float *betas, int64_t N, float *base,
+                                         void *ws, size_t ws_bytes, void *stream) {
+    if (!m || !pose || !betas || !base || !ws || N < 0) return IDF_E_INVAL;
+    if (int rc = smpl_check(m)) return rc;
+    idf_smpl_model ms;
+    if (int rc = smpl_split_model(m, &ms)) return rc;
     if (ws_bytes < interdiff_smpl_workspace_bytes(m, N)) return IDF_E_NOMEM;
     if (N == 0) return IDF_OK;
     hipStream_t s = idf_stream(stream);
     float *feat = reinterpret_cast<float *>(ws);
     float *A = reinterpret_cast<float *>(reinterpret_cast<char *>(ws) + idf_align((size_t)N * m->KB * sizeof(float)));
     idf_prof_mark(IDF_K_SMPL_POSE, s);
-    hipLaunchKernelGGL(smpl_pose_kernel, dim3((unsigned)N), dim3(64), 0, s, *m, pose, betas, trans, feat, A, jtr);
-    const size_t lds = std::max((size_t)FT * m->KB, (size_t)((FT * STS + 255) & ~255) + ((SF * m->J * 12 + 255) & ~255) + (size_t)SF * NTC + FT * 3) * sizeof(float);
-    if (lds > 150 * 1024 || m->KB % 32 != 0 || (m->V * 3) % 2 != 0 || m->S > 4) return IDF_E_INVAL;
-    if (m->KB != 480) return IDF_E_INVAL;
-    static std::atomic<uint64_t> lds_ok{0};
-    if (lds > 64 * 1024 && idf_opt_in_lds(reinterpret_cast<const void *>(smpl_blend_skin_kernel<30>), 150 * 1024, lds_ok) != IDF_OK) return IDF_E_LAUNCH;
-    idf_prof_mark(IDF_K_SMPL_BLEND_SKIN, s);
-    const unsigned nwg_launch = (unsigned)(idf_cdiv(idf_cdiv(N, FT), TBF) * idf_cdiv(idf_cdiv(m->V, VT), TBV) * TBF * TBV);
-    hipLaunchKernelGGL(smpl_blend_skin_kernel<30>, dim3(nwg_launch), dim3(BT), lds, s, *m,
-                       feat, A, trans, N, verts, v_posed);
+    hipLaunchKernelGGL(smpl_pose_kernel, dim3((unsigned)N), dim3(64), 0, s, ms, pose, betas, nullptr, feat, A, nullptr, 1);
+    if (int rc = launch_blend_skin<true>(&ms, true, feat, nullptr, nullptr, N, nullptr, nullptr, base, s)) return rc;
     idf_prof_mark(-1, s);
     IDF_CHECK_LAUNCH();
     return IDF_OK;
 }
+
+namespace {
+
+int smpl_forward_impl(const idf_smpl_model *m, bool split, const float *pose, const float *betas, const float *trans, int64_t N,
+                      const float *base, float *verts, float *jtr, float *v_posed, void *ws, size_t ws_bytes, void *stream) {
+    if (!m || !pose || !betas || !trans || !verts || !jtr || !ws || N < 0) return IDF_E_INVAL;
+    if (int rc = smpl_check(m)) return rc;
+    idf_smpl_model mm = *m;
+    if (split)
+        if (int rc = smpl_split_model(m, &mm)) return rc;
+    if (ws_bytes < interdiff_smpl_workspace_bytes(m, N)) return IDF_E_NOMEM;
+    if (N == 0) return IDF_OK;
+    hipStream_t s = idf_stream(stream);
+    float *feat = reinterpret_cast<float *>(ws);
+    float *A = reinterpret_cast<float *>(reinterpret_cast<char *>(ws) + idf_align((size_t)N * m->KB * sizeof(float)));
+    idf_prof_mark(IDF_K_SMPL_POSE, s);
+    hipLaunchKernelGGL(smpl_pose_kernel, dim3((unsigned)N), dim3(64), 0, s, mm, pose, betas, trans, feat, A, jtr, split ? 1 : 0);
+    if (int rc = launch_blend_skin<false>(&mm, split, feat, A, trans, N, verts, v_posed, const_cast<float *>(base), s)) return rc;
+    idf_prof_mark(-1, s);
+    IDF_CHECK_LAUNCH();
+    return IDF_OK;
+}
+
+}
+
+extern "C" int interdiff_smpl_forward_based(const idf_smpl_model *m, const float *pose, const float *betas, const float *trans,
+                                            int64_t N, const float *base, float *verts, float *jtr, float *v_posed, void *ws,
+                                            size_t ws_bytes, void *stream) {
+    return smpl_forward_impl(m, true, pose, betas, trans, N, base, verts, jtr, v_posed, ws, ws_bytes, stream);
+}
+
+extern "C" int interdiff_smpl_forward(const idf_smpl_model *m, const float *pose, const float *betas, const float *trans,
+                                      int64_t N, float *verts, float *jtr, float *v_posed, void *ws, size_t ws_bytes,
+                                      void *stream) {
+    return smpl_forward_impl(m, false, pose, betas, trans, N, nullptr, verts, jtr, v_posed, ws, ws_bytes, stream);
+}
diff --git a/interdiff_amd/diffusion.py b/interdiff_amd/diffusion.py
--- a/interdiff_amd/diffusion.py
+++ b/interdiff_amd/diffusion.py
@@ -224,6 +224,8 @@
         cond = model_kwargs.get('y', {}).get('cond') if isinstance(model_kwargs.get('y', None), dict) else None
         if cond is not None and hasattr(model, 'prepare_memory'):
             model.prepare_memory(cond)
+        if any(map(graph_sampler.hook_gate(denoised_fn), range(t_first, t_first - todo, -1))):
+            graph_sampler.begin_hook_sample(denoised_fn, model_kwargs.get('y', {}))
         for it, i in enumerate(range(t_first, t_first - todo, -1)):
             t, th = ts[i], ts_hook[i]
             t.host_value = th.host_value = i
diff --git a/interdiff_amd/graph_sampler.py b/interdiff_amd/graph_sampler.py
--- a/interdiff_amd/graph_sampler.py
+++ b/interdiff_amd/graph_sampler.py
@@ -133,7 +133,7 @@
             start = c * (B // n) + min(c, B % n)
             self.chains.append(Chain(model, self, slice(start, start + B // n + (1 if c < B % n else 0)), own_state=c > 0))
 
-    def hook_buffers(self, hook, y, table):
+    def hook_buffers(self, hook, y, table, has_hook_step=True):
         shapes = tuple(tuple(y[k].shape) for k in HOOK_KEYS)
         hk = self.hooks.get(hook._uid)
         if hk is None or hk.shapes != shapes:
@@ -142,6 +142,11 @@
                 del self.graphs[stale]
         for k in HOOK_KEYS + (() if self.gt is not None else ('inpainted_motion',)):
             hk.y[k].copy_(y[k])
+        if getattr(hook, 'begin_sample', None) is not None:
+            if has_hook_step or hk.fresh:
+                hook.begin_sample(hk.y, ws=hk.ws)
+            else:
+                hook.end_sample(hk.ws)
         if hk.fresh:
             hook.apply_dev(hk.y['inpainted_motion'].clone(), table, torch.zeros(8, dtype=torch.int64, device=self.x.device), hk.y, hk.ws)
             torch.cuda.synchronize(self.x.device)
@@ -153,6 +158,12 @@
     return (hook is not None and getattr(hook, 'graph_capturable', False) and getattr(hook, 'debug', None) is None
             and getattr(hook, 'is_active', None) is not None and all(k in y for k in ('inpainted_motion',) + HOOK_KEYS)
             and os.environ.get('INTERDIFF_EAGER_HOOK') != '1')
+
+
+def begin_hook_sample(hook, y):
+    begin = getattr(hook, 'begin_sample', None)
+    if begin is not None and isinstance(y, dict) and all(k in y for k in HOOK_KEYS):
+        begin(y)
 
 
 def hook_gate(hook):
@@ -282,7 +293,11 @@
         st.graphs.clear()
         st.chain_steps = chain_steps
     fuse_hook = hook_capturable(hook, y)
-    run = Run(model, st, table, rows, fused, split, hook, st.hook_buffers(hook, y, table) if fuse_hook else None, tmap)
+    plan = plan_steps(t_start, todo, hook_gate(hook), dump_steps, fuse_hook)
+    has_hook_step = any(op[0] in ('hook', 'eager_hook') for op in plan)
+    run = Run(model, st, table, rows, fused, split, hook, st.hook_buffers(hook, y, table, has_hook_step) if fuse_hook else None, tmap)
+    if has_hook_step and not fuse_hook:
+        begin_hook_sample(hook, y)
 
     st.x.copy_(img)
     st.state.copy_(diffusion.seeded_state(t_start, seed, elem0))
@@ -290,5 +305,5 @@
         for ch in st.chains[1:]:
             ch.state.copy_(diffusion.seeded_state(t_start, seed, elem0 + ch.sl.start * per_clip))
     st.ts.fill_(diff.timestep_map[t_start])
-    dump = run.play(plan_steps(t_start, todo, hook_gate(hook), dump_steps, fuse_hook), t_start, diff._timesteps(B, dev, loop_side=True), model_kwargs)
+    dump = run.play(plan, t_start, diff._timesteps(B, dev, loop_side=True), model_kwargs)
     return dump if dump_steps is not None else st.x.clone()
diff --git a/interdiff_amd/smpl.py b/interdiff_amd/smpl.py
--- a/interdiff_amd/smpl.py
+++ b/interdiff_amd/smpl.py
@@ -8,7 +8,24 @@
     return a.detach().cpu().numpy() if isinstance(a, torch.Tensor) else np.asarray(a)
 
 
-def pack_smpl_model(model, device):
+N_BODY_JOINTS = 22
+
+
+def feature_columns(J, n_betas, n_const_joints):
+    if not 0 <= n_const_joints <= J - 1:
+        raise ValueError('n_const_joints outside 0..J-1')
+    kp, nvar = 9 * (J - 1), 9 * (J - 1 - n_const_joints)
+    const = list(range(nvar, kp)) + list(range(kp, kp + n_betas))
+    split = -(-len(const) // 16) * 16
+    KB = split + -(-(nvar + 1) // 16) * 16
+    cols = np.full(KB, -1, np.int64)
+    cols[:len(const)] = const
+    cols[split:split + nvar] = np.arange(nvar)
+    cols[split + nvar] = kp + n_betas
+    return cols, split, KB
+
+
+def pack_smpl_model(model, device, n_const_joints=None):
     vt = _np(model['v_template']).astype(np.float64).reshape(-1, 3)
     sdirs = _np(model['shapedirs']).astype(np.float64)
     pdirs = _np(model['posedirs']).astype(np.float64)
@@ -19,11 +36,19 @@
     kp = 9 * (J - 1)
     if pdirs.shape != (V, 3, kp) or jreg.shape != (J, V):
         raise ValueError('inconsistent SMPL buffers')
+    if n_const_joints is None:
+        n_const_joints = max(0, J - N_BODY_JOINTS)
     KB = (kp + nb + 1 + 15) // 16 * 16
     blend = np.zeros((3 * V, KB), np.float32)
     blend[:, :kp] = pdirs.reshape(3 * V, kp)
     blend[:, kp:kp + nb] = sdirs.reshape(3 * V, nb)
     blend[:, kp + nb] = vt.reshape(3 * V)
+    cols, _, KBs = feature_columns(J, nb, n_const_joints)
+    if n_const_joints and KBs != KB:
+        n_const_joints = 0
+    blend_split = np.zeros((3 * V, KB), np.float32)
+    if n_const_joints:
+        blend_split[:, cols >= 0] = blend[:, cols[cols >= 0]]
     jt = (jreg @ vt).astype(np.float32)
     js = np.einsum('jv,vck->jck', jreg, sdirs).astype(np.float32)
     nnz = (wts != 0)
@@ -37,14 +62,16 @@
     parents[0] = 0
     t = lambda a: torch.from_numpy(np.ascontiguousarray(a)).to(device)
     nvt = -(-V // 64)
-    rows = np.zeros((nvt * 192, KB), np.float32)
-    rows[:3 * V] = blend
-    frag = rows.reshape(nvt, 4, 3, 16, KB // 16, 4, 4).transpose(0, 1, 2, 4, 5, 3, 6)
-    bufs = dict(blend=t(frag), blend_rows=t(blend), jt=t(jt), js=t(js), parents=t(parents.astype(np.int32)), skin_idx=t(skin_idx), skin_w=t(skin_w))
+    rows = np.zeros((1 + bool(n_const_joints), nvt * 192, KB), np.float32)
+    rows[0, :3 * V] = blend
+    if n_const_joints:
+        rows[1, :3 * V] = blend_split
+    frag = rows.reshape(-1, nvt, 4, 3, 16, KB // 16, 4, 4).transpose(0, 1, 2, 3, 5, 6, 4, 7)
+    bufs = dict(blend=t(frag), blend_rows=t(blend), blend_rows_split=t(blend_split), jt=t(jt), js=t(js), parents=t(parents.astype(np.int32)), skin_idx=t(skin_idx), skin_w=t(skin_w))
     m = _lib.SmplModel()
-    m.V, m.J, m.n_betas, m.KB, m.S = V, J, nb, KB, S
+    m.V, m.J, m.n_betas, m.KB, m.S, m.n_const_joints = V, J, nb, KB, S, n_const_joints
     for k, v in bufs.items():
-        if k != 'blend_rows':
+        if not k.startswith('blend_rows'):
             setattr(m, k, v.data_ptr())
     return m, bufs
 
@@ -66,7 +93,16 @@
             self._ws = torch.empty(max(need, 256), dtype=torch.uint8, device=self.device)
         return self._ws
 
-    def forward(self, th_pose_axisang, th_betas=None, th_trans=None, th_offsets=None, scale=1., want_v_posed=True):
+    def blend_base(self, th_pose_axisang, th_betas):
+        N = th_pose_axisang.shape[0]
+        pose, betas = th_pose_axisang.contiguous().float(), th_betas.contiguous().float()
+        base = torch.empty(self.lib.interdiff_smpl_base_bytes(C.byref(self.cmodel), N) // 4, dtype=torch.float32, device=self.device)
+        ws = self._workspace(N)
+        _lib.check(self.lib.interdiff_smpl_blend_base(C.byref(self.cmodel), _lib.dptr(pose, torch.float32), _lib.dptr(betas, torch.float32), N,
+                                                      _lib.dptr(base), _lib.dptr(ws), ws.numel(), _lib.stream()), 'smpl_blend_base')
+        return base
+
+    def forward(self, th_pose_axisang, th_betas=None, th_trans=None, th_offsets=None, scale=1., want_v_posed=True, base=None, split=False):
         if th_offsets is not None or scale != 1.:
             raise NotImplementedError('th_offsets / scale are not used on the eval_smpl_short path')
         N = th_pose_axisang.shape[0]
@@ -82,10 +118,18 @@
         jtr = torch.empty(N, J, 3, dtype=torch.float32, device=self.device)
         v_posed = torch.empty(N, V, 3, dtype=torch.float32, device=self.device) if want_v_posed else None
         ws = self._workspace(N)
-        _lib.check(self.lib.interdiff_smpl_forward(C.byref(self.cmodel), _lib.dptr(pose, torch.float32), _lib.dptr(betas, torch.float32),
-                                                   _lib.dptr(trans, torch.float32), N, _lib.dptr(verts), _lib.dptr(jtr),
-                                                   _lib.dptr(v_posed, allow_none=True), _lib.dptr(ws), ws.numel(), _lib.stream()),
-                   'smpl_forward')
+        if base is None and not split:
+            _lib.check(self.lib.interdiff_smpl_forward(C.byref(self.cmodel), _lib.dptr(pose, torch.float32), _lib.dptr(betas, torch.float32),
+                                                       _lib.dptr(trans, torch.float32), N, _lib.dptr(verts), _lib.dptr(jtr),
+                                                       _lib.dptr(v_posed, allow_none=True), _lib.dptr(ws), ws.numel(), _lib.stream()),
+                       'smpl_forward')
+        else:
+            if base is not None and base.numel() * 4 != self.lib.interdiff_smpl_base_bytes(C.byref(self.cmodel), N):
+                raise ValueError('base was made for another number of frames')
+            _lib.check(self.lib.interdiff_smpl_forward_based(C.byref(self.cmodel), _lib.dptr(pose, torch.float32), _lib.dptr(betas, torch.float32),
+                                                             _lib.dptr(trans, torch.float32), N, _lib.dptr(base, torch.float32, allow_none=True), _lib.dptr(verts),
+                                                             _lib.dptr(jtr), _lib.dptr(v_posed, allow_none=True), _lib.dptr(ws), ws.numel(),
+                                                             _lib.stream()), 'smpl_forward_based')
         return verts, jtr, v_posed, v_posed
 
     __call__ = forward
```

Result: slower. 6.983 million (-2.0%).
